# skyepurchase/MeatModeler

Hardware: AMD Instinct MI355X
Metric: descriptor-match pairs/sec + BA residuals/sec, 500×1080p frames, 1/2/4/8 GPU (higher is better)
Workload: dtype u8/int32 (match), f64 (BA); 1 GPU; 500 frames 1920x1080, 4000 ORB kpts/frame, BF Hamming 2-NN + ratio, track linking, 2-view DLT, full BA (TRF, Schur, f64 MFMA Cholesky); frames=500, height=1080, width=1920, nfeatures=4000, parallelism=pairs/points x1

## Files before the change

meatmodeler_amd/_lib.py:

```python
import ctypes as C
import os

_HERE = os.path.dirname(os.path.abspath(__file__))
LIB_PATH = os.path.join(_HERE, "libmeatmodeler_hip.so")

c_i32p = C.POINTER(C.c_int32)
c_i64p = C.POINTER(C.c_int64)
c_f32p = C.POINTER(C.c_float)
c_f64p = C.POINTER(C.c_double)
c_u8p = C.POINTER(C.c_uint8)
c_i8p = C.POINTER(C.c_int8)
vp = C.c_void_p


class MMError(RuntimeError):
    pass


class OrbParams(C.Structure):
    _fields_ = [("nfeatures", C.c_int32), ("nlevels", C.c_int32), ("edge_threshold", C.c_int32),
                ("fast_threshold", C.c_int32), ("scale_factor", C.c_float), ("reserved", C.c_int32)]


class BAProblem(C.Structure):
    _fields_ = [("F", C.c_int32), ("P", C.c_int32), ("O", C.c_int64), ("K", vp), ("fi", vp), ("pi", vp),
                ("obs", vp), ("pt_ptr", vp), ("pt_obs", vp), ("cam_ptr", vp), ("cam_obs", vp),
                ("cam_span", C.c_int32), ("reserved", C.c_int32), ("n_seg", C.c_int64), ("seg_ids", vp),
                ("seg_chunk_ptr", vp), ("n_chunks", C.c_int64), ("chunk_seg", vp), ("chunk_begin", vp),
                ("chunk_end", vp), ("pair_o", vp), ("pair_o2", vp), ("pair_p", vp)]


class BAIndex(C.Structure):
    _fields_ = [("F", C.c_int32), ("P", C.c_int32), ("O", C.c_int64), ("fi", vp), ("pi", vp),
                ("pt_ptr", vp), ("pt_obs", vp), ("cam_ptr", vp), ("cam_obs", vp), ("head", vp),
                ("cam_span", C.c_int32), ("chunk", C.c_int32), ("n_pairs", C.c_int64),
                ("pair_o", vp), ("pair_o2", vp), ("pair_p", vp), ("seg_ids", vp), ("seg_chunk_ptr", vp),
                ("chunk_seg", vp), ("chunk_begin", vp), ("chunk_end", vp)]


class BAFixed(C.Structure):
    _fields_ = [("F_fixed", C.c_int32), ("reserved", C.c_int32), ("cams", vp)]


class TrfParams(C.Structure):
    _fields_ = [("ftol", C.c_double), ("xtol", C.c_double), ("gtol", C.c_double), ("min_damping", C.c_double),
                ("max_nfev", C.c_int64)]


class TrfRow(C.Structure):
    _fields_ = [("iteration", C.c_int32), ("nfev", C.c_int32), ("cost", C.c_double), ("reduction", C.c_double),
                ("step_norm", C.c_double), ("optimality", C.c_double)]


class TriParams(C.Structure):
    _fields_ = [("refine_iters", C.c_int32), ("reserved", C.c_int32), ("max_reproj_px", C.c_double),
                ("max_cos_parallax", C.c_double), ("min_depth", C.c_double)]


class VerifyParams(C.Structure):
    _fields_ = [("n_hyp", C.c_int32), ("min_matches", C.c_int32), ("min_inliers", C.c_int32), ("refit_iters", C.c_int32),
                ("seed", C.c_uint32), ("pair_base", C.c_uint32), ("on_fail", C.c_int32), ("reserved", C.c_int32),
                ("threshold_px", C.c_double)]


class PoseParams(C.Structure):
    _fields_ = [("min_matches", C.c_int32), ("reserved", C.c_int32), ("min_front_frac", C.c_double),
                ("ambiguous_frac", C.c_double)]


class HomographyParams(C.Structure):
    _fields_ = [("n_hyp", C.c_int32), ("min_matches", C.c_int32), ("min_inliers", C.c_int32), ("refit_iters", C.c_int32),
                ("seed", C.c_uint32), ("pair_base", C.c_uint32), ("threshold_px", C.c_double), ("collinear_tol", C.c_double),
                ("degenerate_frac", C.c_double)]


class HPoseParams(C.Structure):
    _fields_ = [("min_matches", C.c_int32), ("reserved", C.c_int32), ("min_front_frac", C.c_double),
                ("ambiguous_frac", C.c_double), ("rotation_tol", C.c_double)]


class GuidedParams(C.Structure):
    _fields_ = [("threshold_px", C.c_double), ("ratio", C.c_double), ("max_dist", C.c_int32), ("cross_check", C.c_int32)]


class ResectParams(C.Structure):
    _fields_ = [("n_hyp", C.c_int32), ("min_rows", C.c_int32), ("min_inliers", C.c_int32), ("refit_iters", C.c_int32),
                ("polish_iters", C.c_int32), ("reserved", C.c_int32), ("seed", C.c_uint32), ("cam_base", C.c_uint32),
                ("threshold_px", C.c_double)]


class ResectPlanarParams(C.Structure):
    _fields_ = ResectParams._fields_ + [("planar_tol", C.c_double), ("collinear_tol", C.c_double)]


class AlignParams(C.Structure):
    _fields_ = [("n_hyp", C.c_int32), ("min_points", C.c_int32), ("min_inliers", C.c_int32), ("refit_iters", C.c_int32),
                ("with_scale", C.c_int32), ("reserved", C.c_int32), ("seed", C.c_uint32), ("prob_base", C.c_uint32),
                ("tau", C.c_double), ("collinear_tol", C.c_double)]


ALLREDUCE_FN =C.CFUNCTYPE(C.c_int, vp, vp, C.c_int64)


class Dist(C.Structure):
    _fields_ = [("rank", C.c_int32), ("world", C.c_int32), ("half_bandwidth", C.c_int32), ("band_exchange", C.c_int32),
                ("allreduce", ALLREDUCE_FN), ("user", vp)]


class TrfReport(C.Structure):
    _fields_ = [("cost0", C.c_double), ("cost", C.c_double), ("optimality", C.c_double), ("min_damping", C.c_double),
                ("nfev", C.c_int32), ("njev", C.c_int32), ("status", C.c_int32), ("iterations", C.c_int32),
                ("log_rows", C.c_int32), ("chol_fallbacks", C.c_int32), ("collectives", C.c_int32), ("reserved", C.c_int32)]


SIGNATURES = {
    "mm_abi_version": (C.c_int, []),
    "mm_ctx_create": (C.c_int, [C.c_int, vp, C.POINTER(vp)]),
    "mm_ctx_destroy": (None, [vp]),
    "mm_ctx_control": (C.c_longlong, [vp, C.c_int, C.c_longlong]),
    "mm_last_error": (C.c_char_p, [vp]),
    "mm_ctx_sync": (C.c_int, [vp]),
    "mm_timer_create": (C.c_int, [vp, C.POINTER(vp)]),
    "mm_timer_start": (C.c_int, [vp, vp]),
    "mm_timer_stop": (C.c_int, [vp, vp]),
    "mm_timer_elapsed_ms": (C.c_int, [vp, vp, C.POINTER(C.c_float)]),
    "mm_timer_destroy": (None, [vp, vp]),
    "mm_profile_enable": (C.c_int, [vp, C.c_int]),
    "mm_profile_report": (C.c_int, [vp, C.c_char_p, C.c_size_t]),
    "mm_profile_select": (C.c_int, [vp, C.c_char_p]),
    "mm_bf_workspace_bytes": (C.c_size_t, [C.c_int, C.c_int, C.c_int]),
    "mm_bf_knn2_batched": (C.c_int, [vp, vp, vp, C.c_int, C.c_size_t, vp, vp, C.c_int, C.c_size_t, C.c_int, vp, vp,
                                     vp, C.c_size_t]),
    "mm_bf_knn2_hamming": (C.c_int, [vp, vp, C.c_int, vp, C.c_int, vp, vp, vp, C.c_size_t]),
    "mm_ratio_filter_batched": (C.c_int, [vp, vp, vp, vp, C.c_int, C.c_int, C.c_double, vp, vp]),
    "mm_bf_match_ratio_workspace_bytes": (C.c_size_t, [C.c_int, C.c_int, C.c_int]),
    "mm_bf_match_ratio_batched": (C.c_int, [vp, vp, vp, C.c_int, C.c_size_t, vp, vp, C.c_int, C.c_size_t, C.c_int,
                                            C.c_double, vp, vp, vp, C.c_size_t]),
    "mm_orb_workspace_bytes": (C.c_size_t, [C.c_int, C.c_int, C.c_int, C.POINTER(OrbParams)]),
    "mm_orb_detect_compute": (C.c_int, [vp, vp, C.c_int, C.c_int, C.c_int, C.c_int, C.POINTER(OrbParams), vp, vp,
                                        C.c_size_t, vp, vp, vp, vp, vp, vp]),
    "mm_orb_level_sizes": (C.c_int, [C.c_int, C.c_int, C.POINTER(OrbParams), c_i32p, c_i32p, c_i32p, c_f32p]),
    "mm_link_tracks_clip": (C.c_int64, [C.c_int, C.c_int, c_i32p, c_f32p, C.c_int, c_i32p, c_i32p, C.c_int64,
                                        C.c_int64, c_i64p, c_i32p, c_i32p, c_i64p]),
    "mm_link_workspace_bytes": (C.c_size_t, [C.c_int, C.c_int]),
    "mm_link_tracks_device": (C.c_int, [vp, C.c_int, C.c_int, vp, vp, vp, vp, vp, C.c_size_t, vp, vp, vp, vp]),
    "mm_flatten_offsets": (C.c_int, [vp, vp, vp, C.c_int64, vp]),
    "mm_flatten_tracks": (C.c_int, [vp, vp, vp, vp, vp, C.c_int, vp, C.c_int, C.c_int64, vp, C.c_int64, C.c_int, vp, vp, vp]),
    "mm_ba_build_pairs": (C.c_int64, [C.c_int, C.c_int, C.c_int64, c_i32p, c_i32p, c_i32p, c_i32p, c_i32p, c_i32p, C.c_int,
                                      c_i64p, c_i32p, c_i32p, C.c_int64]),
    "mm_ba_build_index": (C.c_int, [C.c_int, C.c_int, C.c_int64, c_i32p, c_i32p, c_i32p, c_i32p, c_i32p, c_i32p]),
    "mm_verify_workspace_bytes": (C.c_size_t, [C.c_int, C.c_int]),
    "mm_verify_matches": (C.c_int, [vp, vp, vp, vp, C.c_int, C.c_int, C.POINTER(VerifyParams), vp, vp, vp, vp, vp, vp, C.c_size_t]),
    "mm_recover_poses": (C.c_int, [vp, c_f64p, vp, vp, vp, vp, C.c_int, C.c_int, C.POINTER(PoseParams), vp, vp, vp, vp, vp]),
    "mm_chain_poses": (C.c_int, [vp, vp, vp, vp, vp, vp, vp, C.c_int, C.c_int, c_f64p, C.c_int, vp, vp, vp, vp]),
    "mm_homography_workspace_bytes": (C.c_size_t, [C.c_int, C.c_int]),
    "mm_verify_homography": (C.c_int, [vp, vp, vp, vp, C.c_int, C.c_int, C.POINTER(HomographyParams), vp, vp, vp, vp, vp, vp, vp,
                                       C.c_size_t]),
    "mm_recover_poses_homography": (C.c_int, [vp, c_f64p, vp, vp, vp, vp, vp, C.c_int, C.c_int, C.POINTER(HPoseParams), vp, vp, vp,
                                              vp, vp, vp]),
    "mm_guided_workspace_bytes": (C.c_size_t, [C.c_int, C.c_int]),
    "mm_guided_match": (C.c_int, [vp, vp, vp, vp, vp, vp, vp, vp, C.c_int, C.c_int, C.POINTER(GuidedParams), vp, vp, vp, vp, vp,
                                  C.c_size_t]),
    "mm_resect_workspace_bytes": (C.c_size_t, [C.c_int, C.c_int, C.c_int64]),
    "mm_resect_cameras": (C.c_int, [vp, c_f64p, vp, C.c_int64, vp, vp, C.c_int64, vp, vp, C.c_int64, C.c_int, vp, vp,
                                    C.POINTER(ResectParams), vp, vp, vp, vp, vp, C.c_size_t]),
    "mm_resect_planar_workspace_bytes": (C.c_size_t, [C.c_int, C.c_int, C.c_int64]),
    "mm_resect_planar": (C.c_int, [vp, c_f64p, vp, C.c_int64, vp, vp, C.c_int64, vp, vp, C.c_int64, C.c_int, vp, vp,
                                   C.POINTER(ResectPlanarParams), vp, vp, vp, vp, vp, vp, C.c_size_t]),
    "mm_align_workspace_bytes": (C.c_size_t, [C.c_int, C.c_int, C.c_int64]),
    "mm_align_similarity": (C.c_int, [vp, vp, vp, c_i64p, C.c_int, C.POINTER(AlignParams), vp, vp, vp, vp, vp, C.c_size_t]),
    "mm_apply_similarity": (C.c_int, [vp, vp, vp, C.c_int64, vp, C.c_int64]),
    "mm_camera_centres": (C.c_int, [vp, vp, C.c_int64, vp]),
    "mm_triangulate_dlt": (C.c_int, [vp, vp, vp, vp, vp, vp, C.c_int64, vp]),
    "mm_triangulate_tracks_workspace_bytes": (C.c_size_t, [C.c_int]),
    "mm_triangulate_tracks": (C.c_int, [vp, vp, C.c_int, vp, C.c_int64, vp, vp, C.POINTER(TriParams), vp, vp, vp, vp, C.c_size_t]),
    "mm_ba_residual": (C.c_int, [vp, C.POINTER(BAProblem), vp, vp, vp, vp, vp, C.c_size_t]),
    "mm_ba_jacobian": (C.c_int, [vp, C.POINTER(BAProblem), vp, vp, vp, vp]),
    "mm_ba_normal_eq": (C.c_int, [vp, C.POINTER(BAProblem), vp, vp, vp, vp, vp, vp]),
    "mm_ba_jvp": (C.c_int, [vp, C.POINTER(BAProblem), vp, vp, vp, vp, vp]),
    "mm_ba_schur": (C.c_int, [vp, C.POINTER(BAProblem), vp, vp, vp, vp, vp, vp, vp, vp, vp, vp, C.c_size_t]),
    "mm_ba_schur_workspace_bytes": (C.c_size_t, [C.POINTER(BAProblem)]),
    "mm_ba_pairs_count": (C.c_int, [vp, C.POINTER(BAProblem), vp, vp]),
    "mm_ba_pairs_emit": (C.c_int, [vp, C.POINTER(BAProblem), vp, C.c_int, vp, vp, vp]),
    "mm_ba_index_bounds": (C.c_int, [C.c_int, C.c_int, C.c_int64, C.c_int, c_i64p, c_i64p]),
    "mm_ba_index_workspace_bytes": (C.c_size_t, [vp, C.POINTER(BAIndex), C.c_int]),
    "mm_ba_index_build": (C.c_int, [vp, C.POINTER(BAIndex), C.c_int, vp, C.c_size_t, vp, C.c_size_t]),
    "mm_ba_schur_solve": (C.c_int, [vp, C.POINTER(BAProblem), vp, vp, vp, vp, vp, vp, vp, vp, vp, C.c_int, vp, vp,
                                    C.c_size_t, vp, C.c_size_t, C.c_int, C.c_int, c_i64p, c_i64p]),
    "mm_multi_dot_workspace_bytes": (C.c_size_t, []),
    "mm_multi_dot": (C.c_int, [vp, C.c_int, C.POINTER(vp), C.POINTER(vp), C.c_int64, C.c_int64, vp, vp, C.c_size_t]),
    "mm_trf_fused": (C.c_int, [vp, C.c_int, C.POINTER(vp), C.POINTER(vp), C.POINTER(vp), C.c_double, C.c_double, C.c_int64,
                               C.c_int64, vp, vp, C.c_size_t]),
    "mm_trf_damping": (C.c_int, [vp, vp, vp, C.c_double, C.c_double, vp]),
    "mm_ba_backsub": (C.c_int, [vp, C.POINTER(BAProblem), vp, vp, vp, vp, vp, vp, vp, C.c_size_t]),
    "mm_ba_backsub_workspace_bytes": (C.c_size_t, [C.POINTER(BAProblem)]),
    "mm_chol_workspace_bytes": (C.c_size_t, [C.c_int]),
    "mm_chol_solve": (C.c_int, [vp, vp, C.c_int, vp, C.c_int, C.c_int, vp, vp, C.c_size_t]),
    "mm_ba_jvp_dots_workspace_bytes": (C.c_size_t, [C.POINTER(BAProblem)]),
    "mm_ba_jvp_dots": (C.c_int, [vp, C.POINTER(BAProblem), vp, vp, vp, vp, vp, vp, vp, vp, C.c_size_t]),
    "mm_ba_scale_update": (C.c_int, [vp, C.c_int, C.c_int, vp, vp, vp, C.c_int]),
    "mm_ba_damp": (C.c_int, [vp, C.c_int, C.c_int, vp, vp, vp, vp, vp, vp]),
    "mm_trf_step2d": (C.c_int, [vp, vp, vp, vp, vp, vp, vp, vp, vp, C.c_double, vp]),
    "mm_pyr_down": (C.c_int, [vp, vp, C.c_int, C.c_int, C.c_int, vp, C.c_int]),
    "mm_lk_track": (C.c_int, [vp, vp, vp, vp, vp, vp, C.c_int, vp, C.c_int, C.c_int, C.c_int, C.c_int, C.c_double, vp, vp, vp]),
    "mm_min_eig": (C.c_int, [vp, vp, C.c_int, C.c_int, C.c_int, C.c_int, vp]),
    "mm_corner_candidates": (C.c_int, [vp, vp, C.c_int, C.c_int, C.c_double, vp, vp, vp, C.c_int, vp]),
    "mm_gftt_select": (C.c_int, [vp, C.c_int64, C.c_int, C.c_int, C.c_int, C.c_double, vp, C.c_int]),
    "mm_contrast_workspace_bytes": (C.c_size_t, [C.c_int, C.c_int, C.c_int, C.c_int, C.c_int]),
    "mm_increase_contrast": (C.c_int, [vp, vp, C.c_int, C.c_int, C.c_int, vp, vp, vp, C.c_double, C.c_int, C.c_int, vp, vp, vp,
                                       C.c_size_t]),
    "mm_bgr_to_grey": (C.c_int, [vp, vp, C.c_size_t, vp]),
    "mm_write_ply": (C.c_int, [C.c_char_p, vp, C.c_int64]),
    "mm_chol_solve_sym": (C.c_int, [vp, vp, C.c_int, vp, C.c_int, C.c_int, vp, vp, C.c_size_t]),
    "mm_ba_trf_workspace_bytes": (C.c_size_t, [C.POINTER(BAProblem)]),
    "mm_ba_trf": (C.c_int, [vp, C.POINTER(BAProblem), vp, vp, C.POINTER(TrfParams), C.POINTER(TrfReport),
                            C.POINTER(TrfRow), C.c_int, vp, C.c_size_t]),
    "mm_ba_trf_batched_workspace_bytes": (C.c_size_t, [C.POINTER(BAProblem)]),
    "mm_ba_trf_batched": (C.c_int, [vp, C.c_int, C.POINTER(C.POINTER(BAProblem)), C.POINTER(vp), C.POINTER(vp),
                                    C.POINTER(TrfParams), C.POINTER(TrfReport), C.POINTER(vp), C.POINTER(C.c_size_t), c_i32p]),
    "mm_ba_residual_fixed": (C.c_int, [vp, C.POINTER(BAProblem), C.POINTER(BAFixed), vp, vp, vp, vp, vp, C.c_size_t]),
    "mm_ba_normal_eq_fixed": (C.c_int, [vp, C.POINTER(BAProblem), C.POINTER(BAFixed), vp, vp, vp, vp, vp, vp]),
    "mm_ba_trf_fixed_workspace_bytes": (C.c_size_t, [C.POINTER(BAProblem), C.POINTER(BAFixed)]),
    "mm_ba_trf_fixed": (C.c_int, [vp, C.POINTER(BAProblem), C.POINTER(BAFixed), vp, vp, C.POINTER(TrfParams),
                                  C.POINTER(TrfReport), C.POINTER(TrfRow), C.c_int, vp, C.c_size_t]),
    "mm_ba_trf_dist_workspace_bytes": (C.c_size_t, [C.POINTER(BAProblem), C.c_int]),
    "mm_ba_trf_dist": (C.c_int, [vp, C.POINTER(BAProblem), vp, vp, C.POINTER(TrfParams), C.POINTER(TrfReport),
                                 C.POINTER(TrfRow), C.c_int, vp, C.c_size_t, C.POINTER(Dist)]),
}


def _load():
    if not os.path.exists(LIB_PATH):
        raise ImportError(
            f"{LIB_PATH} is missing: the HIP extension has not been built "
            "(make -C meatmodeler_amd/csrc).  meatmodeler_amd has no CPU fallback.")
    lib = C.CDLL(LIB_PATH)
    for name, (res, args) in SIGNATURES.items():
        fn = getattr(lib, name)
        fn.restype = res
        fn.argtypes = args
    return lib


lib = _load()


def ptr(t):
    if t is None:
        return None
    if hasattr(t, "data_ptr"):
        return t.data_ptr()
    return t.ctypes.data


class Context:

    def __init__(self, device=None, stream=None):
        import torch
        if not torch.cuda.is_available():
            raise MMError("meatmodeler_amd needs an AMD GPU (torch.cuda.is_available() is False); "
                          "there is no CPU path")
        if device is None:
            device = torch.cuda.current_device()
        self.device = torch.device("cuda", device if isinstance(device, int) else device.index or 0)
        self.stream = stream if stream is not None else torch.cuda.current_stream(self.device)
        h = vp()
        rc = lib.mm_ctx_create(self.device.index, vp(self.stream.cuda_stream), C.byref(h))
        if rc != 0:
            raise MMError(f"mm_ctx_create failed ({rc})")
        self.h = h

    def check(self, rc, what=""):
        if rc != 0:
            msg = lib.mm_last_error(self.h)
            raise MMError(f"{what} failed ({rc}): {msg.decode() if msg else ''}")

    def sync(self):
        self.check(lib.mm_ctx_sync(self.h), "mm_ctx_sync")

    CTL_CHOL_FORCE_ABANDON, CTL_CHOL_LAST_PATH, CTL_CHOL_RESERVED, CTL_CU_COUNT, CTL_CHOL_AVOID_FUSED = 1, 2, 3, 4, 5
    CTL_LINK_LAST_VARIANT = 6
    CTL_BATCH_LAST = 7

    def control(self, what, value=0):
        r = int(lib.mm_ctx_control(self.h, int(what), int(value)))
        if r < -1 or (r == -1 and what not in (self.CTL_CHOL_LAST_PATH, self.CTL_LINK_LAST_VARIANT, self.CTL_BATCH_LAST)):
            self.check(r, "mm_ctx_control")
        return r

    def profile(self, level, only=None):
        if only is not None:
            self.check(lib.mm_profile_select(self.h, only.encode()), "mm_profile_select")
        self.check(lib.mm_profile_enable(self.h, int(level)), "mm_profile_enable")

    def profile_report(self):
        buf = C.create_string_buffer(1 << 16)
        n = lib.mm_profile_report(self.h, buf, len(buf))
        if n < 0:
            self.check(n, "mm_profile_report")
        out = {}
        for line in buf.value.decode().splitlines():
            name, cnt, ms = line.split()
            out[name] = (int(cnt), float(ms))
        return out

    def __del__(self):
        try:
            if getattr(self, "h", None):
                lib.mm_ctx_destroy(self.h)
                self.h = None
        except Exception:
            pass


class Timer:

    def __init__(self, ctx):
        self.ctx = ctx
        self.t = vp()
        ctx.check(lib.mm_timer_create(ctx.h, C.byref(self.t)), "mm_timer_create")

    def start(self):
        self.ctx.check(lib.mm_timer_start(self.ctx.h, self.t), "mm_timer_start")

    def stop(self):
        self.ctx.check(lib.mm_timer_stop(self.ctx.h, self.t), "mm_timer_stop")

    def elapsed_ms(self):
        ms = C.c_float()
        self.ctx.check(lib.mm_timer_elapsed_ms(self.ctx.h, self.t, C.byref(ms)), "mm_timer_elapsed_ms")
        return ms.value

    def __del__(self):
        try:
            lib.mm_timer_destroy(self.ctx.h, self.t)
        except Exception:
            pass


_default_ctx = {}


def default_context():
    import torch
    key = (torch.cuda.current_device(), torch.cuda.current_stream().cuda_stream)
    c = _default_ctx.get(key)
    if c is None:
        c = _default_ctx[key] = Context()
    return c
```

meatmodeler_amd/csrc/mm_common.h:

```cpp
#pragma once
#include <hip/hip_runtime.h>
#include <cstdarg>
#include <cstdio>
#include <cstring>
#include <vector>
#include "../../include/meatmodeler.h"

struct mm_prof_rec {
    const char *name;
    hipEvent_t a, b;
};

struct mm_ctx {
    int device;
    hipStream_t stream;
    char err[512];
    int prof = 0;
    char prof_only[64] = {0};
    std::vector<mm_prof_rec> recs;
    std::vector<hipEvent_t> pool;
    hipStream_t aux = nullptr;
    hipEvent_t ev_fork = nullptr, ev_join = nullptr;
    bool attr_chol_fused = false, attr_chol_bwd = false, attr_chol_batch = false;
    int cu_count = 0, fused_wgs = 0, chol_last_path = -1, debug_abandon = 0;
    bool chol_avoid_fused = false;
    bool chol_strict_budget = false;
    hipEvent_t fused_ev = nullptr;
    bool fused_ev_pending = false;
    bool fused_no_event = false;
    int link_last_variant = -1;
    void *cam_tab = nullptr;
    int cam_tab_cap = 0, cam_tab_F = 0;
    const double *cam_tab_for = nullptr;
    bool cam_tab_hold = false;
    const double *fx_cams = nullptr;
    int fx_F = 0;
    bool fx_tab_ok = false;
    void *host_board = nullptr;
    unsigned long long host_board_seq = 0;
    void *batch_dev = nullptr, *batch_host = nullptr;
    size_t batch_dev_cap = 0, batch_host_cap = 0;
    bool jvp_rows_deferred = false;
    const double *jvp_partial = nullptr;
    unsigned jvp_n_wg = 0;
    const void *chol_init_done = nullptr;
    int chol_init_sides = 0;
    int batch_last = -1;
};

struct mm_stream_swap {
    mm_ctx *c;
    hipStream_t saved;
    mm_stream_swap(mm_ctx *ctx, hipStream_t s) : c(ctx), saved(ctx->stream) { ctx->stream = s; }
    ~mm_stream_swap() { c->stream = saved; }
};

struct mm_fixed_scope {
    mm_ctx *c;
    mm_fixed_scope(mm_ctx *ctx, const mm_ba_fixed *fx) : c(ctx) {
        ctx->fx_cams = fx->cams;
        ctx->fx_F = fx->F_fixed;
        ctx->fx_tab_ok = false;
    }
    ~mm_fixed_scope() {
        c->fx_cams = nullptr;
        c->fx_F = 0;
        c->fx_tab_ok = false;
    }
};

int mm_cam_coef_table(mm_ctx *ctx, const double *cams, int F, const void **tab_out);
void mm_cam_table_hold(mm_ctx *ctx, bool on);
void mm_cam_table_invalidate(mm_ctx *ctx);

int mm_ba_residual_publish(mm_ctx *ctx, const mm_ba_problem *pb, const double *cams, const double *pts, void *ws,
                           size_t ws_bytes, double *board, int cost_slot, int count, void *host_board, unsigned long long seq);

int mm_trf_fused0_scaled(mm_ctx *ctx, const double *g, double *si, const double *B, const double *C, double *gh, double *ghs, int64_t n,
                         int64_t split, double *out, void *ws, size_t ws_bytes);
int mm_trf_fused5_coef(mm_ctx *ctx, const double *x, const double *s1, const double *s2, double *x_new, const double *h01, int64_t n,
                       int64_t split, void *ctab, int F);
int mm_trf_rows_step2d(mm_ctx *ctx, const double *partial, unsigned n_wg, double *rows, const double *r0, const double *d11,
                       const double *r1, const double *r2, const double *r3, const double *reg, const int32_t *info, double Delta,
                       double *board);
int mm_cam_table_adopt(mm_ctx *ctx, const double *cams, int F, void **tab_out);
int mm_ba_damp_damping(mm_ctx *ctx, int F, int P, const double *B, const double *C, const double *scale_inv, const double *gh2,
                       const double *d11, double Delta, double min_damping, double *damp_out, double *Bd, double *Cd);
void mm_chol_release_budget(mm_ctx *ctx);
bool mm_chol_fused_eligible(int n, int half_bandwidth);
struct mm_chol_geom {
    int n, nblk, bwb;
    int a, m, b;
    int pad;
};
struct mm_chol_layout {
    double *Linv, *ytmp, *contrib, *contrib_bwd, *lpub, *spub;
    int32_t *flags;
    mm_chol_geom g;
    uint64_t nflags, nsent, nlpub;
};
struct mm_chol_plan {
    mm_chol_layout lay;
    bool fused;
    int sides;
    unsigned grid_fused, grid_bwd;
};
struct mm_chol_init_args {
    int32_t *info, *flags;
    size_t nflags;
    unsigned long long *sentinel_buf;
    size_t nsent;
    unsigned long long *lpub;
    size_t nlpub;
    unsigned long long *Linv;
    size_t nblk;
};
bool mm_chol_init_plan(mm_ctx *ctx, int n, int half_bandwidth, int32_t *info, void *ws, size_t ws_bytes, mm_chol_init_args *out, int *sides, int *bwb);
void mm_chol_init_done(mm_ctx *ctx, const void *ws, int sides);
struct mm_damp_spec {
    const double *B, *C, *si;
    const double *gh2, *d11;
    double Delta, min_damping;
    double *damp_out;
    const double *reg;
};
int mm_ba_schur_solve_damped(mm_ctx *ctx, const mm_ba_problem *pb, const double *cams, const double *pts, const mm_damp_spec *dmp,
                             double *Bd, double *Cd, const double *gc, const double *gp, double *S, double *v, double *Cinv,
                             int half_bandwidth, int32_t *info, void *ws_schur, size_t ws_schur_bytes, void *ws_chol,
                             size_t ws_chol_bytes);
int mm_chol_solve_gated(mm_ctx *ctx, double *A, int n, double *b, int nrhs, int half_bandwidth, int32_t *info, void *ws,
                        size_t ws_bytes, const int32_t *slab_ready, int cams_per_slab, int n_cams, int sym_mode);

struct mm_batch_prob {
    mm_ba_problem pb;
    int64_t n, nc;
    double *x, *x_new, *g, *si, *gh, *ghs, *gn, *q1, *w, *q2, *s1, *s2;
    double *B, *Bd, *C, *Cd, *Cinv, *u1, *Jq2, *dp, *v, *S;
    double *r0, *r1, *r2, *r3, *d11, *bs, *damp, *board;
    int32_t *info;
    void *ctab_x, *ctab_new;
    double *res_partial;
    unsigned *md_counter;
    double *md_partial;
    double *jvp_partial;
    double *backsub_T;
    double *schur_partial, *schur_camtab;
    int32_t *schur_seg_done, *schur_desc;
    mm_chol_layout chol;
    int32_t half_bw, chol_sym_mirror;
    uint32_t g_vec, g_res, g_jvp, g_pblk, g_obs, g_pts, g_scale, g_damp, g_prep, g_pairs, g_chol, g_bwd, g_coef, g_zero;
    void *mailbox;
};
struct mm_batch_dyn {
    double Delta;
    unsigned long long seq;
    double min_damping;
    double reg;
};

int mm_batch_fused(mm_ctx *ctx, int op, const mm_batch_prob *tab, const int32_t *list, int n_list, unsigned max_g);
unsigned mm_batch_fused_grid(int64_t n);
int mm_batch_scale_update(mm_ctx *ctx, const mm_batch_prob *tab, const int32_t *list, int n_list, unsigned max_g);
int mm_batch_damp(mm_ctx *ctx, const mm_batch_prob *tab, const int32_t *list, int n_list, unsigned max_g);
int mm_batch_accept(mm_ctx *ctx, const mm_batch_prob *tab, const int32_t *list, int n_list, unsigned max_g);
int mm_batch_step2d(mm_ctx *ctx, const mm_batch_prob *tab, const int32_t *list, int n_list, const mm_batch_dyn *dyn);
void mm_batch_ba_setup(mm_batch_prob *bp);
int mm_batch_cam_coef(mm_ctx *ctx, const mm_batch_prob *tab, const int32_t *list, int n_list, unsigned max_g, int which );
int mm_batch_jvp_dots(mm_ctx *ctx, const mm_batch_prob *tab, const int32_t *list, int n_list, unsigned max_g, int second);
int mm_batch_damping(mm_ctx *ctx, const mm_batch_prob *tab, const int32_t *list, int n_list, const mm_batch_dyn *dyn);
int mm_batch_set_reg(mm_ctx *ctx, const mm_batch_prob *tab, const int32_t *list, int n_list, const mm_batch_dyn *dyn);
int mm_batch_backsub(mm_ctx *ctx, const mm_batch_prob *tab, const int32_t *list, int n_list, unsigned max_g_obs, unsigned max_g_pts);
int mm_batch_residual_publish(mm_ctx *ctx, const mm_batch_prob *tab, const int32_t *list, int n_list, unsigned max_g,
                              const mm_batch_dyn *dyn);
int mm_batch_normal_eq(mm_ctx *ctx, const mm_batch_prob *tab, const int32_t *list, int n_list, unsigned max_g_pblk, unsigned max_F);
int mm_batch_publish_rows(mm_ctx *ctx, const mm_batch_prob *tab, const int32_t *list, int n_list, const mm_batch_dyn *dyn);
int mm_batch_schur_setup(mm_ctx *ctx, mm_batch_prob *bp, void *ws_schur, size_t ws_schur_bytes);
int mm_batch_schur(mm_ctx *ctx, const mm_batch_prob *tab, const int32_t *list, int n_list, unsigned max_g_zero, unsigned max_g_prep,
                   unsigned max_g_pairs);
int mm_batch_chol_setup(mm_ctx *ctx, mm_batch_prob *bp, void *ws_chol, size_t ws_chol_bytes);
int mm_batch_chol(mm_ctx *ctx, const mm_batch_prob *tab, const int32_t *list, int n_list, unsigned max_g_chol, unsigned max_g_bwd);

static inline hipEvent_t mm_prof_event(mm_ctx *c) {
    hipEvent_t e = nullptr;
    if (!c->pool.empty()) {
        e = c->pool.back();
        c->pool.pop_back();
    } else {
        (void)hipEventCreate(&e);
    }
    return e;
}

#define MM_LAUNCH(ctx, name, kernel, grid, block, shmem, ...)                                          \
    do {                                                                                               \
        hipEvent_t ea_ = nullptr, eb_ = nullptr;                                                       \
        const dim3 g_ = (grid);                                                                        \
        const bool p_ = (ctx)->prof == 1 || ((ctx)->prof == 2 && (size_t)g_.x * g_.y * g_.z >= 64) || \
                        ((ctx)->prof == 3 && strcmp(name, (ctx)->prof_only) == 0);                      \
        if (p_) {                                                                                      \
            ea_ = mm_prof_event(ctx);                                                                  \
            eb_ = mm_prof_event(ctx);                                                                  \
            (void)hipEventRecord(ea_, (ctx)->stream);                                                  \
        }                                                                                              \
        hipLaunchKernelGGL(kernel, g_, block, shmem, (ctx)->stream, __VA_ARGS__);                      \
        if (p_) {                                                                                      \
            (void)hipEventRecord(eb_, (ctx)->stream);                                                  \
            (ctx)->recs.push_back(mm_prof_rec{name, ea_, eb_});                                        \
        }                                                                                              \
        MM_LAUNCH_CHECK(ctx, name);                                                                    \
    } while (0)

static inline int mm_fail(mm_ctx *ctx, int code, const char *fmt, ...) {
    if (ctx) {
        va_list ap;
        va_start(ap, fmt);
        vsnprintf(ctx->err, sizeof(ctx->err), fmt, ap);
        va_end(ap);
    }
    return code;
}

#define MM_HIP(ctx, call)                                                                              \
    do {                                                                                               \
        hipError_t e_ = (call);                                                                        \
        if (e_ != hipSuccess)                                                                          \
            return mm_fail(ctx, MM_ERR_HIP, "%s failed: %s (%s:%d)", #call, hipGetErrorString(e_),    \
                           __FILE__, __LINE__);                                                        \
    } while (0)

#define MM_LAUNCH_CHECK(ctx, name)                                                                     \
    do {                                                                                               \
        hipError_t e_ = hipGetLastError();                                                             \
        if (e_ != hipSuccess)                                                                          \
            return mm_fail(ctx, MM_ERR_HIP, "launch of %s failed: %s", name, hipGetErrorString(e_));   \
    } while (0)

static inline size_t mm_align_up(size_t x, size_t a) { return (x + a - 1) / a * a; }
```

meatmodeler_amd/csrc/schur.hip:

```cpp
#include <type_traits>
#include "ba_eval.h"
#include "chol_init.h"

namespace {

__device__ __forceinline__ void sym3_inverse(double a, double b, double d, double e, double f, double g, double *__restrict__ o) {
    const double m00 = e * g - f * f, m01 = d * f - b * g, m02 = b * f - d * e;
    const double det = a * m00 + b * m01 + d * m02;
    const double id = 1.0 / det;
    o[0] = m00 * id;
    o[1] = m01 * id;
    o[2] = m02 * id;
    o[3] = (a * g - d * d) * id;
    o[4] = (b * d - a * f) * id;
    o[5] = (a * e - b * b) * id;
}

constexpr int SR_WIN = 256;

__global__ __launch_bounds__(256) void point_inverse_kernel(int P, const double *__restrict__ Cd,
                                                            double *__restrict__ Cinv) {
    int p = blockIdx.x * 256 + threadIdx.x;
    if (p >= P) return;
    const double *c = Cd + (size_t)p * 6;
    sym3_inverse(c[0], c[1], c[2], c[3], c[4], c[5], Cinv + (size_t)p * 6);
}

__global__ __launch_bounds__(256) void schur_rows_kernel(mm_ba_problem pb, const double *__restrict__ cams,
                                                         const double *__restrict__ pts, const double *__restrict__ Bd,
                                                         const double *__restrict__ Cinv, const double *__restrict__ gc,
                                                         const double *__restrict__ gp, double *__restrict__ S,
                                                         double *__restrict__ v) {
    __shared__ double acc[6][SR_WIN * 6];
    __shared__ double Ks[9];
    __shared__ double cs[6];
    __shared__ double sm[4];
    const int i = blockIdx.x;
    const int w0 = blockIdx.y * SR_WIN;
    const int wn = min(SR_WIN, pb.F - w0);
    const size_t n = (size_t)pb.F * 6;
    for (int e = threadIdx.x; e < 6 * SR_WIN * 6; e += 256) (&acc[0][0])[e] = 0.0;
    if (threadIdx.x < 9) Ks[threadIdx.x] = pb.K[threadIdx.x];
    if (threadIdx.x < 6) cs[threadIdx.x] = cams[(size_t)i * 6 + threadIdx.x];
    __syncthreads();
    double vg[6] = {0, 0, 0, 0, 0, 0};
    for (int e = pb.cam_ptr[i] + threadIdx.x; e < pb.cam_ptr[i + 1]; e += 256) {
        const int o = pb.cam_obs[e];
        const int p = pb.pi[o];
        const double *Xp = pts + (size_t)p * 3;
        Proj pr;
        ba_eval<true, true>(cs, Xp, Ks, pb.obs[2 * (size_t)o], pb.obs[2 * (size_t)o + 1], pr);
        const double *ci = Cinv + (size_t)p * 6;
        const double q00 = ci[0], q01 = ci[1], q02 = ci[2], q11 = ci[3], q12 = ci[4], q22 = ci[5];
        double Y[6][3];
#pragma unroll
        for (int a = 0; a < 6; ++a) {
            const double e0 = pr.Jc[0][a] * pr.Jp[0][0] + pr.Jc[1][a] * pr.Jp[1][0];
            const double e1 = pr.Jc[0][a] * pr.Jp[0][1] + pr.Jc[1][a] * pr.Jp[1][1];
            const double e2 = pr.Jc[0][a] * pr.Jp[0][2] + pr.Jc[1][a] * pr.Jp[1][2];
            Y[a][0] = e0 * q00 + e1 * q01 + e2 * q02;
            Y[a][1] = e0 * q01 + e1 * q11 + e2 * q12;
            Y[a][2] = e0 * q02 + e1 * q12 + e2 * q22;
        }
        if (blockIdx.y == 0) {
            const double g0 = gp[(size_t)p * 3], g1 = gp[(size_t)p * 3 + 1], g2 = gp[(size_t)p * 3 + 2];
#pragma unroll
            for (int a = 0; a < 6; ++a) vg[a] += Y[a][0] * g0 + Y[a][1] * g1 + Y[a][2] * g2;
        }
        for (int e2i = pb.pt_ptr[p]; e2i < pb.pt_ptr[p + 1]; ++e2i) {
            const int o2 = pb.pt_obs[e2i];
            const int f2 = pb.fi[o2];
            if (f2 < w0 || f2 >= w0 + wn) continue;
            Proj p2;
            ba_eval<true, true>(cams + (size_t)f2 * 6, Xp, Ks, pb.obs[2 * (size_t)o2], pb.obs[2 * (size_t)o2 + 1], p2);
            double *dst = &acc[0][(f2 - w0) * 6];
#pragma unroll
            for (int b = 0; b < 6; ++b) {
                const double e0 = p2.Jc[0][b] * p2.Jp[0][0] + p2.Jc[1][b] * p2.Jp[1][0];
                const double e1 = p2.Jc[0][b] * p2.Jp[0][1] + p2.Jc[1][b] * p2.Jp[1][1];
                const double e2 = p2.Jc[0][b] * p2.Jp[0][2] + p2.Jc[1][b] * p2.Jp[1][2];
#pragma unroll
                for (int a = 0; a < 6; ++a)
                    atomicAdd(dst + a * (SR_WIN * 6) + b, Y[a][0] * e0 + Y[a][1] * e1 + Y[a][2] * e2);
            }
        }
    }
    __syncthreads();
    for (int e = threadIdx.x; e < 6 * wn * 6; e += 256) {
        const int a = e / (wn * 6), c = e % (wn * 6);
        const int col = w0 * 6 + c;
        double val = -acc[a][c];
        if (col / 6 == i) val += Bd[(size_t)i * 36 + a * 6 + (col % 6)];
        S[((size_t)i * 6 + a) * n + col] = val;
    }
    if (blockIdx.y == 0) {
#pragma unroll
        for (int a = 0; a < 6; ++a) {
            const double s = block_sum<256>(vg[a], sm);
            if (threadIdx.x == 0) v[(size_t)i * 6 + a] = gc[(size_t)i * 6 + a] - s;
        }
    }
}

#ifndef MM_SP_WAVES
#define MM_SP_WAVES 1
#endif
constexpr int SP_WAVES = MM_SP_WAVES;
constexpr int MAX_SLABS = 64;
struct SlabSync {
    int32_t *ready;
    int32_t *done;
    int32_t seg_count[MAX_SLABS];
    int cams_per_slab;
};

constexpr int RED_LD = 65;
__device__ __forceinline__ void wave_lds_barrier() {
    __builtin_amdgcn_fence(__ATOMIC_RELEASE, "wavefront");
    __builtin_amdgcn_wave_barrier();
    __builtin_amdgcn_fence(__ATOMIC_ACQUIRE, "wavefront");
}
__device__ __forceinline__ void wave_reduce_42(const double (&acc)[42], double *slab , int lane, double &out0,
                                               double &out1) {
#pragma unroll
    for (int h = 0; h < 2; ++h) {
#pragma unroll
        for (int q = 0; q < 21; ++q) slab[q * RED_LD + lane] = acc[21 * h + q];
        wave_lds_barrier();
        double s = 0.0;
        if (lane < 21) {
            const double *row = slab + lane * RED_LD;
            double s0 = 0.0, s1 = 0.0, s2 = 0.0, s3 = 0.0;
#pragma unroll
            for (int j = 0; j < 64; j += 4) {
                s0 += row[j];
                s1 += row[j + 1];
                s2 += row[j + 2];
                s3 += row[j + 3];
            }
            s = (s0 + s1) + (s2 + s3);
        }
        if (h == 0)
            out0 = s;
        else
            out1 = s;
        wave_lds_barrier();
    }
}

struct CamPQ {
    double P[9], q[3];
};
__device__ __forceinline__ double fast_rcp(double x) {
    double y = __builtin_amdgcn_rcp(x);
    double e = fma(-x, y, 1.0);
    y = fma(y, e, y);
    e = fma(-x, y, 1.0);
    return fma(y, e, y);
}

struct LeanJ {
    double Jc[2][6];
    double Jp[2][3];
};
__device__ __forceinline__ void lean_eval(const CamPQ &c, const double *__restrict__ Ks, const double *__restrict__ Jr,
                                          double X0, double X1, double X2, LeanJ &o) {
    const double u0 = fma(c.P[0], X0, fma(c.P[1], X1, fma(c.P[2], X2, c.q[0])));
    const double u1 = fma(c.P[3], X0, fma(c.P[4], X1, fma(c.P[5], X2, c.q[1])));
    const double u2 = fma(c.P[6], X0, fma(c.P[7], X1, fma(c.P[8], X2, c.q[2])));
    const double iz = fast_rcp(u2);
    const double p[2] = {u0 * iz, u1 * iz};
#pragma unroll
    for (int m = 0; m < 2; ++m) {
#pragma unroll
        for (int k = 0; k < 3; ++k) {
            o.Jp[m][k] = fma(-p[m], c.P[6 + k], c.P[3 * m + k]) * iz;
            o.Jc[m][3 + k] = fma(-p[m], Ks[6 + k], Ks[3 * m + k]) * iz;
        }
        const double g0 = X1 * o.Jp[m][2] - X2 * o.Jp[m][1];
        const double g1 = X2 * o.Jp[m][0] - X0 * o.Jp[m][2];
        const double g2 = X0 * o.Jp[m][1] - X1 * o.Jp[m][0];
#pragma unroll
        for (int k = 0; k < 3; ++k) o.Jc[m][k] = fma(g0, Jr[k], fma(g1, Jr[3 + k], g2 * Jr[6 + k]));
    }
}

constexpr int SLAB2 = 32;
struct ChunkDesc {
    int32_t i, f2, e_begin, e_end, sidx, c_first, n_ch, pad;
};
template <bool FORCE>
__device__ __forceinline__ CamPQ cam_pq_scalar(const double *__restrict__ t) {
    CamPQ v;
#pragma unroll
    for (int k = 0; k < 9; ++k) v.P[k] = FORCE ? uniform_f64(t[k]) : t[k];
#pragma unroll
    for (int k = 0; k < 3; ++k) v.q[k] = FORCE ? uniform_f64(t[9 + k]) : t[9 + k];
    return v;
}
template <bool FORCE_UNIFORM>
__device__ __forceinline__ void schur_pairs_body(const mm_ba_problem pb, const double *__restrict__ camtab,
                                                                    const ChunkDesc *__restrict__ desc,
                                                                    const double *__restrict__ pts,
                                                                    const double *__restrict__ Cinv,
                                                                    const double *__restrict__ gp,
                                                                    double *partial, const double *__restrict__ Bd,
                                                                    const double *__restrict__ gc, double *S, double *v,
                                                                    int32_t *seg_done, SlabSync slabs, unsigned wg_begin,
                                                                    unsigned wg_total, const unsigned bx) {
    __shared__ double Ks[9];
    __shared__ double red[SP_WAVES][21 * RED_LD];
    __shared__ double jrs[SP_WAVES][SLAB2];
    if (threadIdx.x < 9) Ks[threadIdx.x] = pb.K[threadIdx.x];
    const int lane = threadIdx.x & 63;
    const int wv = __builtin_amdgcn_readfirstlane((int)(threadIdx.x >> 6));
    const unsigned gpos = bx + wg_begin;
    const unsigned wg = (gpos & 1) ? wg_total - 1 - (gpos >> 1) : (gpos >> 1);
    const int64_t c = (int64_t)wg * SP_WAVES + wv;
    const bool live = c < pb.n_chunks;
    ChunkDesc cd = {};
    if (live) cd = desc[c];
    if (FORCE_UNIFORM) {
        cd.i = __builtin_amdgcn_readfirstlane(cd.i);
        cd.f2 = __builtin_amdgcn_readfirstlane(cd.f2);
        cd.e_begin = __builtin_amdgcn_readfirstlane(cd.e_begin);
        cd.e_end = __builtin_amdgcn_readfirstlane(cd.e_end);
        cd.sidx = __builtin_amdgcn_readfirstlane(cd.sidx);
        cd.c_first = __builtin_amdgcn_readfirstlane(cd.c_first);
        cd.n_ch = __builtin_amdgcn_readfirstlane(cd.n_ch);
    }
    const int i = cd.i, f2 = cd.f2, d = cd.i - cd.f2, sidx = cd.sidx;
    const int e_begin = cd.e_begin, e_end = cd.e_end;
    auto point_of = [&](int e) { return pb.pair_p ? pb.pair_p[e] : pb.pi[pb.pair_o[e]]; };
    auto self_of = [&](int e) { return d == 0 && pb.pair_o[e] == pb.pair_o2[e]; };
    int e = e_begin + lane;
    int p_next = -1;
    bool self_next = false;
    if (live) {
        if (e < e_end) {
            p_next = point_of(e);
            self_next = self_of(e);
        }
        if (lane < 9) jrs[wv][lane] = camtab[(size_t)i * CAMTAB2 + 12 + lane];
        else if (lane >= 16 && lane < 25) jrs[wv][lane] = camtab[(size_t)f2 * CAMTAB2 + 12 + lane - 16];
    }
    __syncthreads();
    if (!live) return;
    const CamPQ cp_i = cam_pq_scalar<FORCE_UNIFORM>(camtab + (size_t)i * CAMTAB2), cp_2 = cam_pq_scalar<FORCE_UNIFORM>(camtab + (size_t)f2 * CAMTAB2);
    const double *Jr_i = jrs[wv], *Jr_2 = jrs[wv] + 16;
    double acc[42];
#pragma unroll
    for (int q = 0; q < 42; ++q) acc[q] = 0.0;
    auto load_xc = [&](int p, double (&x)[12]) {
        if (p >= 0) {
            const double *Xp = pts + (size_t)p * 3, *ci = Cinv + (size_t)p * 6;
            x[0] = Xp[0];
            x[1] = Xp[1];
            x[2] = Xp[2];
#pragma unroll
            for (int q = 0; q < 6; ++q) x[3 + q] = ci[q];
            if (d == 0) {
                x[9] = gp[(size_t)p * 3];
                x[10] = gp[(size_t)p * 3 + 1];
                x[11] = gp[(size_t)p * 3 + 2];
            }
        }
    };
    auto pair_body = [&](int p, bool self, const double (&x)[12]) {
        const double X0 = x[0], X1 = x[1], X2 = x[2];
        const double q00 = x[3], q01 = x[4], q02 = x[5], q11 = x[6], q12 = x[7], q22 = x[8];
        LeanJ a;
        lean_eval(cp_i, Ks, Jr_i, X0, X1, X2, a);
        double Z[2][3];
#pragma unroll
        for (int m = 0; m < 2; ++m) {
            Z[m][0] = a.Jp[m][0] * q00 + a.Jp[m][1] * q01 + a.Jp[m][2] * q02;
            Z[m][1] = a.Jp[m][0] * q01 + a.Jp[m][1] * q11 + a.Jp[m][2] * q12;
            Z[m][2] = a.Jp[m][0] * q02 + a.Jp[m][1] * q12 + a.Jp[m][2] * q22;
        }
        double M[2][2], T[2][6];
        if (d == 0) {
            if (self) {
                const double g0 = x[9], g1 = x[10], g2 = x[11];
                const double z0 = Z[0][0] * g0 + Z[0][1] * g1 + Z[0][2] * g2, z1 = Z[1][0] * g0 + Z[1][1] * g1 + Z[1][2] * g2;
#pragma unroll
                for (int q = 0; q < 6; ++q) acc[36 + q] += a.Jc[0][q] * z0 + a.Jc[1][q] * z1;
            }
#pragma unroll
            for (int m = 0; m < 2; ++m)
#pragma unroll
                for (int n_ = 0; n_ < 2; ++n_) M[m][n_] = Z[m][0] * a.Jp[n_][0] + Z[m][1] * a.Jp[n_][1] + Z[m][2] * a.Jp[n_][2];
#pragma unroll
            for (int b = 0; b < 6; ++b) {
                T[0][b] = M[0][0] * a.Jc[0][b] + M[0][1] * a.Jc[1][b];
                T[1][b] = M[1][0] * a.Jc[0][b] + M[1][1] * a.Jc[1][b];
            }
        } else {
            LeanJ b2;
            lean_eval(cp_2, Ks, Jr_2, X0, X1, X2, b2);
#pragma unroll
            for (int m = 0; m < 2; ++m)
#pragma unroll
                for (int n_ = 0; n_ < 2; ++n_) M[m][n_] = Z[m][0] * b2.Jp[n_][0] + Z[m][1] * b2.Jp[n_][1] + Z[m][2] * b2.Jp[n_][2];
#pragma unroll
            for (int b = 0; b < 6; ++b) {
                T[0][b] = M[0][0] * b2.Jc[0][b] + M[0][1] * b2.Jc[1][b];
                T[1][b] = M[1][0] * b2.Jc[0][b] + M[1][1] * b2.Jc[1][b];
            }
        }
#pragma unroll
        for (int q = 0; q < 6; ++q)
#pragma unroll
            for (int b = 0; b < 6; ++b) acc[q * 6 + b] += a.Jc[0][q] * T[0][b] + a.Jc[1][q] * T[1][b];
    };
    double xc[12];
    load_xc(p_next, xc);
    int p_cur = p_next;
    bool self_cur = self_next;
    {
        const int en = e + 64;
        p_next = en < e_end ? point_of(en) : -1;
        self_next = en < e_end && self_of(en);
    }
#pragma clang loop unroll(disable)
    for (; e - lane < e_end; e += 64) {
        double xn[12];
        load_xc(p_next, xn);
        const int p_nn_e = e + 128;
        const int p_nn = p_nn_e < e_end ? point_of(p_nn_e) : -1;
        const bool self_nn = p_nn_e < e_end && self_of(p_nn_e);
        if (p_cur >= 0) pair_body(p_cur, self_cur, xc);
#pragma unroll
        for (int q = 0; q < 12; ++q) xc[q] = xn[q];
        p_cur = p_next;
        self_cur = self_next;
        p_next = p_nn;
        self_next = self_nn;
    }
    double tot0, tot1;
    wave_reduce_42(acc, red[wv], lane, tot0, tot1);
    const int c_first = cd.c_first, n_ch = cd.n_ch;
    const size_t n = (size_t)pb.F * 6;
    bool writer = true;
    if (n_ch > 1) {
        if (lane < 21) {
            __hip_atomic_store(partial + (size_t)c * 42 + lane, tot0, __ATOMIC_RELAXED, __HIP_MEMORY_SCOPE_AGENT);
            __hip_atomic_store(partial + (size_t)c * 42 + 21 + lane, tot1, __ATOMIC_RELAXED, __HIP_MEMORY_SCOPE_AGENT);
        }
        asm volatile("s_waitcnt vmcnt(0)" ::: "memory");
        __builtin_amdgcn_wave_barrier();
        int last = 0;
        if (lane == 0) last = atomicAdd(seg_done + sidx, 1) == n_ch - 1;
        writer = __shfl(last, 0, 64) != 0;
        if (writer && lane < 21) {
            tot0 = 0.0;
            tot1 = 0.0;
            for (int cc = 0; cc < n_ch; ++cc) {
                tot0 += __hip_atomic_load(partial + (size_t)(c_first + cc) * 42 + lane, __ATOMIC_RELAXED, __HIP_MEMORY_SCOPE_AGENT);
                tot1 += __hip_atomic_load(partial + (size_t)(c_first + cc) * 42 + 21 + lane, __ATOMIC_RELAXED, __HIP_MEMORY_SCOPE_AGENT);
            }
        }
    }
    if (!writer) return;
    const bool through = slabs.ready != nullptr;
    if (lane < 21) {
#pragma unroll
        for (int h = 0; h < 2; ++h) {
            const int q = 21 * h + lane;
            const double sum = h == 0 ? tot0 : tot1;
            if (q < 36) {
                double val = -sum;
                if (d == 0) val += Bd[(size_t)i * 36 + q];
                double *dst = S + ((size_t)i * 6 + q / 6) * n + (size_t)f2 * 6 + q % 6;
                double *mir = S + ((size_t)f2 * 6 + q % 6) * n + (size_t)i * 6 + q / 6;
                if (through) {
                    __hip_atomic_store(dst, val, __ATOMIC_RELAXED, __HIP_MEMORY_SCOPE_AGENT);
                    if (d != 0) __hip_atomic_store(mir, val, __ATOMIC_RELAXED, __HIP_MEMORY_SCOPE_AGENT);
                } else {
                    *dst = val;
                    if (d != 0) *mir = val;
                }
            } else if (d == 0) {
                double *dst = v + (size_t)i * 6 + (q - 36);
                const double val = gc[(size_t)i * 6 + (q - 36)] - sum;
                if (through) __hip_atomic_store(dst, val, __ATOMIC_RELAXED, __HIP_MEMORY_SCOPE_AGENT);
                else *dst = val;
            }
        }
    }
    if (slabs.ready) {
        asm volatile("s_waitcnt vmcnt(0)" ::: "memory");
        __builtin_amdgcn_wave_barrier();
        if (lane == 0) {
            const int sl = i / slabs.cams_per_slab;
            if (atomicAdd(slabs.done + sl, 1) == slabs.seg_count[sl] - 1)
                __hip_atomic_store(slabs.ready + sl, 1, __ATOMIC_RELEASE, __HIP_MEMORY_SCOPE_AGENT);
        }
    }
}
__global__ __launch_bounds__(64 * SP_WAVES, 2) void schur_pairs_kernel(mm_ba_problem pb, const double *__restrict__ camtab,
                                                                    const ChunkDesc *__restrict__ desc,
                                                                    const double *__restrict__ pts,
                                                                    const double *__restrict__ Cinv,
                                                                    const double *__restrict__ gp,
                                                                    double *partial, const double *__restrict__ Bd,
                                                                    const double *__restrict__ gc, double *S, double *v,
                                                                    int32_t *seg_done, SlabSync slabs, unsigned wg_begin,
                                                                    unsigned wg_total) {
    schur_pairs_body<false>(pb, camtab, desc, pts, Cinv, gp, partial, Bd, gc, S, v, seg_done, slabs, wg_begin, wg_total, blockIdx.x);
}
__global__ __launch_bounds__(64 * SP_WAVES, 2) void schur_pairs_batch_kernel(const mm_batch_prob *__restrict__ tab, const int32_t *__restrict__ list) {
    const mm_batch_prob &bp = tab[list[blockIdx.y]];
    if (blockIdx.x >= bp.g_pairs) return;
    SlabSync none = {};
    schur_pairs_body<true>(bp.pb, bp.schur_camtab, (const ChunkDesc *)bp.schur_desc, bp.x + bp.nc, bp.Cinv, bp.g + bp.nc, bp.schur_partial, bp.Bd,
                     bp.g, bp.S, bp.v, bp.schur_seg_done, none, 0u, bp.g_pairs, blockIdx.x);
}


__device__ __forceinline__ void write_chunk_desc(const mm_ba_problem &pb, int32_t *__restrict__ desc, int64_t first, int64_t stride) {
    for (int64_t k = first; k < pb.n_chunks; k += stride) {
        const int sidx = pb.chunk_seg[k], seg = pb.seg_ids[sidx];
        const int ci = seg / (pb.cam_span + 1), cdd = seg % (pb.cam_span + 1);
        const int c_first = pb.seg_chunk_ptr[sidx];
        int32_t *o = desc + 8 * k;
        o[0] = ci;
        o[1] = ci - cdd;
        o[2] = pb.chunk_begin[k];
        o[3] = pb.chunk_end[k];
        o[4] = sidx;
        o[5] = c_first;
        o[6] = pb.seg_chunk_ptr[sidx + 1] - c_first;
        o[7] = 0;
    }
}
struct PrepExtra {
    mm_damp_spec dmp;
    int zero_bwb;
    int chol_init;
    mm_chol_init_args init;
};
__device__ __forceinline__ void schur_prepare_body(mm_ba_problem pb, const double *__restrict__ cams,
                                                            double *__restrict__ Bd, const double *__restrict__ Cd,
                                                            const double *__restrict__ gc, double *__restrict__ Cinv,
                                                            double *__restrict__ S, double *__restrict__ v,
                                                            double *__restrict__ tab, int32_t *__restrict__ seg_done,
                                                            int32_t *__restrict__ desc , const unsigned bx, const unsigned gx,
                                                            const PrepExtra *ex = nullptr) {
    const int b = (int)bx, tid = threadIdx.x;
    for (int64_t k = (int64_t)b * 256 + tid; k < pb.n_seg; k += (int64_t)gx * 256) seg_done[k] = 0;
    if (desc) write_chunk_desc(pb, desc, (int64_t)b * 256 + tid, (int64_t)gx * 256);
    const bool fold = ex && ex->dmp.B;
    double reg = 0.0;
    if (fold) {
        if (ex->dmp.gh2) {
            const double r = trf_damping_value(ex->dmp.gh2[0], ex->dmp.d11[0], ex->dmp.Delta);
            reg = fmax(r, ex->dmp.min_damping);
            if (b == 0 && tid == 0) {
                ex->dmp.damp_out[0] = r;
                ex->dmp.damp_out[1] = reg;
            }
        } else {
            reg = ex->dmp.reg[0];
        }
    }
    if (ex && ex->chol_init) mm_chol_init_body(ex->init, bx, gx);
    const size_t n = (size_t)pb.F * 6;
    if (ex && ex->zero_bwb >= 0) {
        const int nblk = (int)((n + 63) / 64);
        for (size_t r = bx; r < n; r += gx) {
            const int bi = (int)(r >> 6);
            const int lo = bi - ex->zero_bwb < 0 ? 0 : bi - ex->zero_bwb, hi = bi + ex->zero_bwb >= nblk ? nblk - 1 : bi + ex->zero_bwb;
            const size_t c0 = (size_t)lo * 64, c1 = (size_t)(hi + 1) * 64 < n ? (size_t)(hi + 1) * 64 : n;
            const size_t d0 = r / 6 * 6;
            for (size_t c = c0 + 2 * (size_t)tid; c < c1; c += 512)
                if (c < d0 || c >= d0 + 6) *reinterpret_cast<double2 *>(S + r * n + c) = double2{0.0, 0.0};
        }
    }
    const int f = b * 256 + tid;
    if (f < pb.F) cam_table2_row(cams + (size_t)f * 6, pb.K, tab + (size_t)f * CAMTAB2);
    if (b < pb.F) {
        const bool empty = pb.cam_ptr[b + 1] == pb.cam_ptr[b];
        if (tid < 36) {
            double bd;
            if (fold) {
                bd = ex->dmp.B[(size_t)b * 36 + tid];
                if (tid % 7 == 0) {
                    const double s = ex->dmp.si[(size_t)b * 6 + tid / 7];
                    bd = fma(s * s, reg, bd);
                }
                Bd[(size_t)b * 36 + tid] = bd;
            } else {
                bd = Bd[(size_t)b * 36 + tid];
            }
            if (empty)
                S[((size_t)b * 6 + tid / 6) * n + (size_t)b * 6 + tid % 6] = bd;
            else if (ex && ex->zero_bwb >= 0)
                S[((size_t)b * 6 + tid / 6) * n + (size_t)b * 6 + tid % 6] = 0.0;
        }
        if (empty && tid < 6) v[(size_t)b * 6 + tid] = gc[(size_t)b * 6 + tid];
    }
    const int p = b * 256 + tid;
    if (p < pb.P) {
        double a, bq, d, e, ff, g;
        if (fold) {
            const double *c = ex->dmp.C + (size_t)p * 6;
            const double *sp = ex->dmp.si + n + (size_t)p * 3;
            a = fma(sp[0] * sp[0], reg, c[0]);
            bq = c[1];
            d = c[2];
            e = fma(sp[1] * sp[1], reg, c[3]);
            ff = c[4];
            g = fma(sp[2] * sp[2], reg, c[5]);
        } else {
            const double *c = Cd + (size_t)p * 6;
            a = c[0], bq = c[1], d = c[2], e = c[3], ff = c[4], g = c[5];
        }
        sym3_inverse(a, bq, d, e, ff, g, Cinv + (size_t)p * 6);
    }
}
__global__ __launch_bounds__(256) void schur_prepare_kernel(mm_ba_problem pb, const double *__restrict__ cams,
                                                            double *__restrict__ Bd, const double *__restrict__ Cd,
                                                            const double *__restrict__ gc, double *__restrict__ Cinv,
                                                            double *__restrict__ S, double *__restrict__ v,
                                                            double *__restrict__ tab, int32_t *__restrict__ seg_done,
                                                            int32_t *__restrict__ desc) {
    schur_prepare_body(pb, cams, Bd, Cd, gc, Cinv, S, v, tab, seg_done, desc, blockIdx.x, gridDim.x);
}
__global__ __launch_bounds__(256) void schur_prepare_damped_kernel(mm_ba_problem pb, const double *__restrict__ cams,
                                                                   double *__restrict__ Bd, const double *__restrict__ gc,
                                                                   double *__restrict__ Cinv, double *__restrict__ S,
                                                                   double *__restrict__ v, double *__restrict__ tab,
                                                                   int32_t *__restrict__ seg_done, int32_t *__restrict__ desc,
                                                                   PrepExtra ex) {
    schur_prepare_body(pb, cams, Bd, nullptr, gc, Cinv, S, v, tab, seg_done, desc, blockIdx.x, gridDim.x, &ex);
}
__global__ __launch_bounds__(256) void zero_batch_kernel(const mm_batch_prob *__restrict__ tab, const int32_t *__restrict__ list) {
    const mm_batch_prob &bp = tab[list[blockIdx.y]];
    if (blockIdx.x >= bp.g_zero) return;
    double2 *S2 = reinterpret_cast<double2 *>(bp.S);
    const int64_t n2 = bp.nc * bp.nc / 2;
    for (int64_t i = (int64_t)blockIdx.x * 256 + threadIdx.x; i < n2; i += (int64_t)bp.g_zero * 256) S2[i] = make_double2(0.0, 0.0);
}
__global__ __launch_bounds__(256) void schur_prepare_batch_kernel(const mm_batch_prob *__restrict__ tab, const int32_t *__restrict__ list) {
    const mm_batch_prob &bp = tab[list[blockIdx.y]];
    if (blockIdx.x >= bp.g_prep) return;
    schur_prepare_body(bp.pb, bp.x, bp.Bd, bp.Cd, bp.g, bp.Cinv, bp.S, bp.v, bp.schur_camtab, bp.schur_seg_done, bp.schur_desc,
                       blockIdx.x, bp.g_prep);
}

__global__ void slab_flag_kernel(int32_t *flags, int s) {
    __hip_atomic_store(flags + s, 1, __ATOMIC_RELEASE, __HIP_MEMORY_SCOPE_AGENT);
}

__global__ __launch_bounds__(256) void pairs_count_kernel(mm_ba_problem pb, int32_t *__restrict__ cnt,
                                                          int32_t *__restrict__ span_out) {
    const int64_t o = (int64_t)blockIdx.x * 256 + threadIdx.x;
    int dmax = 0;
    if (o < pb.O) {
        const int f = pb.fi[o], p = pb.pi[o];
        int c = 0;
        for (int e = pb.pt_ptr[p]; e < pb.pt_ptr[p + 1]; ++e) {
            const int d = f - pb.fi[pb.pt_obs[e]];
            c += d >= 0;
            dmax = max(dmax, d);
        }
        cnt[o] = c;
    }
    for (int off = 32; off > 0; off >>= 1) dmax = max(dmax, __shfl_down(dmax, off, 64));
    if ((threadIdx.x & 63) == 0 && dmax > __hip_atomic_load(span_out, __ATOMIC_RELAXED, __HIP_MEMORY_SCOPE_AGENT)) atomicMax(span_out, dmax);
}

__global__ __launch_bounds__(256) void pairs_emit_kernel(mm_ba_problem pb, const int64_t *__restrict__ offsets, int span,
                                                         int32_t *__restrict__ key, int32_t *__restrict__ po,
                                                         int32_t *__restrict__ po2) {
    const int64_t o = (int64_t)blockIdx.x * 256 + threadIdx.x;
    if (o >= pb.O) return;
    const int f = pb.fi[o], p = pb.pi[o];
    int64_t w = offsets[o];
    for (int e = pb.pt_ptr[p]; e < pb.pt_ptr[p + 1]; ++e) {
        const int o2 = pb.pt_obs[e];
        const int d = f - pb.fi[o2];
        if (d < 0) continue;
        key[w] = f * (span + 1) + d;
        po[w] = (int32_t)o;
        po2[w] = o2;
        ++w;
    }
}

}

extern "C" int mm_ba_pairs_count(mm_ctx *ctx, const mm_ba_problem *pb, int32_t *cnt, int32_t *span_out) {
    if (!ctx) return MM_ERR_ARG;
    if (!pb || !cnt || !span_out || (pb->O > 0 && (!pb->fi || !pb->pi || !pb->pt_ptr || !pb->pt_obs)))
        return mm_fail(ctx, MM_ERR_ARG, "mm_ba_pairs_count: bad argument");
    MM_HIP(ctx, hipMemsetAsync(span_out, 0, sizeof(int32_t), ctx->stream));
    if (pb->O == 0) return MM_OK;
    MM_LAUNCH(ctx, "pairs_count_kernel", pairs_count_kernel, dim3((unsigned)((pb->O + 255) / 256)), dim3(256), 0, *pb, cnt,
              span_out);
    return MM_OK;
}

extern "C" int mm_ba_pairs_emit(mm_ctx *ctx, const mm_ba_problem *pb, const int64_t *offsets, int span, int32_t *key,
                                int32_t *pair_o, int32_t *pair_o2) {
    if (!ctx) return MM_ERR_ARG;
    if (!pb || !offsets || !key || !pair_o || !pair_o2 || span < 0) return mm_fail(ctx, MM_ERR_ARG, "mm_ba_pairs_emit: bad argument");
    if (pb->O == 0) return MM_OK;
    if ((int64_t)pb->F * (span + 1) > 0x7fffffffLL) return mm_fail(ctx, MM_ERR_ARG, "mm_ba_pairs_emit: F * (span + 1) overflows the key");
    MM_LAUNCH(ctx, "pairs_emit_kernel", pairs_emit_kernel, dim3((unsigned)((pb->O + 255) / 256)), dim3(256), 0, *pb, offsets,
              span, key, pair_o, pair_o2);
    return MM_OK;
}

namespace {
struct SchurWs {
    double *partial;
    int32_t *seg_done;
    int32_t *slab_ready;
    int32_t *slab_done;
    double *camtab;
    int32_t *desc;
};
size_t carve_schur_ws(SchurWs &w, char *base, const mm_ba_problem *pb) {
    size_t off = 0;
    auto take = [&](auto *&p, size_t n) {
        using T = std::remove_reference_t<decltype(*p)>;
        p = reinterpret_cast<T *>(base + off);
        off += mm_align_up(n * sizeof(T), 256);
    };
    take(w.partial, (size_t)pb->n_chunks * 42);
    take(w.seg_done, (size_t)pb->n_seg);
    take(w.slab_ready, 2 * MAX_SLABS);
    w.slab_done = w.slab_ready + MAX_SLABS;
    take(w.camtab, (size_t)pb->F * CAMTAB2);
    take(w.desc, (size_t)pb->n_chunks * 8);
    return off;
}
struct SchurPlan {
    bool pairs;
    unsigned g_prep;
    unsigned g_pairs;
    size_t ws_bytes;
    SchurWs ws;
};
SchurPlan schur_plan(const mm_ba_problem *pb, void *ws) {
    SchurPlan pl;
    pl.pairs = pb->n_seg > 0 && pb->n_chunks > 0 && pb->seg_ids && pb->seg_chunk_ptr && pb->chunk_seg && pb->chunk_begin &&
               pb->chunk_end && pb->pair_o && pb->pair_o2;
    pl.g_prep = (unsigned)((pb->P + 255) / 256 > pb->F ? (pb->P + 255) / 256 : pb->F);
    pl.g_pairs = (unsigned)((pb->n_chunks + SP_WAVES - 1) / SP_WAVES);
    pl.ws_bytes = carve_schur_ws(pl.ws, (char *)ws, pb);
    return pl;
}
int launch_prepare(mm_ctx *ctx, const mm_ba_problem *pb, const SchurPlan &pl, const double *cams, const double *Bd, const double *Cd,
                   const double *gc, double *Cinv, double *S, double *v) {
    MM_LAUNCH(ctx, "schur_prepare_kernel", schur_prepare_kernel, dim3(pl.g_prep), dim3(256), 0, *pb, cams, const_cast<double *>(Bd), Cd, gc,
              Cinv, S, v, pl.ws.camtab, pl.ws.seg_done, pl.ws.desc);
    return MM_OK;
}
int launch_pairs(mm_ctx *ctx, const mm_ba_problem *pb, const SchurPlan &pl, const double *pts, const double *Cinv, const double *gp,
                 const double *Bd, const double *gc, double *S, double *v, const SlabSync &slabs, unsigned wg_begin, unsigned wg_count) {
    MM_LAUNCH(ctx, "schur_pairs_kernel", schur_pairs_kernel, dim3(wg_count), dim3(64 * SP_WAVES), 0, *pb, (const double *)pl.ws.camtab,
              (const ChunkDesc *)pl.ws.desc, pts, Cinv, gp, pl.ws.partial, Bd, gc, S, v, pl.ws.seg_done, slabs, wg_begin, pl.g_pairs);
    return MM_OK;
}
}

extern "C" size_t mm_ba_schur_workspace_bytes(const mm_ba_problem *pb) {
    if (!pb || pb->n_chunks <= 0) return 0;
    return schur_plan(pb, nullptr).ws_bytes;
}

extern "C" int mm_ba_schur(mm_ctx *ctx, const mm_ba_problem *pb, const double *cams, const double *pts,
                           const double *Bd, const double *Cd, const double *gc, const double *gp, double *S, double *v,
                           double *Cinv, void *ws, size_t ws_bytes) {
    if (!ctx) return MM_ERR_ARG;
    if (!pb || pb->F < 0 || pb->P < 0 || pb->O < 0 || !pb->K) return mm_fail(ctx, MM_ERR_ARG, "mm_ba_schur: bad problem");
    if (!cams || !pts || !Bd || !Cd || !gc || !gp || !S || !v || !Cinv || !pb->pt_ptr || !pb->cam_ptr ||
        (pb->O > 0 && (!pb->pt_obs || !pb->cam_obs || !pb->fi || !pb->pi || !pb->obs)))
        return mm_fail(ctx, MM_ERR_ARG, "mm_ba_schur: null pointer");
    if (pb->F == 0) return MM_OK;
    const SchurPlan pl = schur_plan(pb, ws);
    if (pl.pairs) {
        if (!ws || ws_bytes < pl.ws_bytes) return mm_fail(ctx, MM_ERR_WORKSPACE, "mm_ba_schur: workspace too small");
        MM_HIP(ctx, hipMemsetAsync(S, 0, (size_t)pb->F * 6 * pb->F * 6 * sizeof(double), ctx->stream));
        if (int rc = launch_prepare(ctx, pb, pl, cams, Bd, Cd, gc, Cinv, S, v)) return rc;
        return launch_pairs(ctx, pb, pl, pts, Cinv, gp, Bd, gc, S, v, SlabSync{}, 0u, pl.g_pairs);
    }
    if (pb->P > 0)
        MM_LAUNCH(ctx, "point_inverse_kernel", point_inverse_kernel, dim3((pb->P + 255) / 256), dim3(256), 0, pb->P, Cd,
                  Cinv);
    const int nwin = (pb->F + SR_WIN - 1) / SR_WIN;
    MM_LAUNCH(ctx, "schur_rows_kernel", schur_rows_kernel, dim3(pb->F, nwin), dim3(256), 0, *pb, cams, pts, Bd, Cinv, gc,
              gp, S, v);
    return MM_OK;
}

extern "C" int mm_ba_schur_solve(mm_ctx *ctx, const mm_ba_problem *pb, const double *cams, const double *pts,
                                 const double *Bd, const double *Cd, const double *gc, const double *gp, double *S,
                                 double *v, double *Cinv, int half_bandwidth, int32_t *info, void *ws_schur,
                                 size_t ws_schur_bytes, void *ws_chol, size_t ws_chol_bytes, int n_slabs,
                                 int cams_per_slab, const int64_t *slab_seg_ptr, const int64_t *slab_chunk_ptr) {
    if (!ctx) return MM_ERR_ARG;
    if (!pb || !info) return mm_fail(ctx, MM_ERR_ARG, "mm_ba_schur_solve: bad argument");
    const int n = pb->F * 6;
    const SchurPlan pl = schur_plan(pb, ws_schur);
    const bool overlap = pl.pairs && n_slabs >= 2 && n_slabs <= MAX_SLABS && cams_per_slab >= 16 && slab_seg_ptr &&
                         slab_chunk_ptr && mm_chol_fused_eligible(n, half_bandwidth) && pb->P > 0;
    if (!overlap) {
        int rc = mm_ba_schur(ctx, pb, cams, pts, Bd, Cd, gc, gp, S, v, Cinv, ws_schur, ws_schur_bytes);
        if (rc) return rc;
        return mm_chol_solve_sym(ctx, S, n, v, half_bandwidth, 1, info, ws_chol, ws_chol_bytes);
    }
    if (!cams || !pts || !Bd || !Cd || !gc || !gp || !S || !v || !Cinv) return mm_fail(ctx, MM_ERR_ARG, "mm_ba_schur_solve: null pointer");
    if (!ws_schur || ws_schur_bytes < pl.ws_bytes) return mm_fail(ctx, MM_ERR_WORKSPACE, "mm_ba_schur_solve: workspace too small");
    if (slab_seg_ptr[0] != 0 || slab_seg_ptr[n_slabs] != pb->n_seg || slab_chunk_ptr[0] != 0 || slab_chunk_ptr[n_slabs] != pb->n_chunks ||
        (int64_t)n_slabs * cams_per_slab < pb->F)
        return mm_fail(ctx, MM_ERR_ARG, "mm_ba_schur_solve: slab tables do not cover the problem");
    if (!ctx->aux) {
        int lo = 0, hi = 0;
        (void)hipDeviceGetStreamPriorityRange(&lo, &hi);
        MM_HIP(ctx, hipStreamCreateWithPriority(&ctx->aux, hipStreamNonBlocking, hi));
        MM_HIP(ctx, hipEventCreateWithFlags(&ctx->ev_fork, hipEventDisableTiming));
        MM_HIP(ctx, hipEventCreateWithFlags(&ctx->ev_join, hipEventDisableTiming));
    }
    SlabSync slabs = {};
    slabs.ready = pl.ws.slab_ready;
    slabs.done = pl.ws.slab_done;
    slabs.cams_per_slab = cams_per_slab;
    for (int sl = 0; sl < n_slabs; ++sl) slabs.seg_count[sl] = (int32_t)(slab_seg_ptr[sl + 1] - slab_seg_ptr[sl]);
    MM_HIP(ctx, hipMemsetAsync(S, 0, (size_t)n * n * sizeof(double), ctx->stream));
    MM_HIP(ctx, hipMemsetAsync(pl.ws.slab_ready, 0, 2 * MAX_SLABS * sizeof(int32_t), ctx->stream));
    if (int rc = launch_prepare(ctx, pb, pl, cams, Bd, Cd, gc, Cinv, S, v)) return rc;
    for (int sl = 0; sl < n_slabs; ++sl)
        if (slabs.seg_count[sl] == 0) MM_LAUNCH(ctx, "slab_flag_kernel", slab_flag_kernel, dim3(1), dim3(1), 0, pl.ws.slab_ready, sl);
    const unsigned wg_first = pl.g_pairs / 2;
    if (wg_first > 0)
        if (int rc = launch_pairs(ctx, pb, pl, pts, Cinv, gp, Bd, gc, S, v, slabs, 0u, wg_first)) return rc;
    MM_HIP(ctx, hipEventRecord(ctx->ev_fork, ctx->stream));
    MM_HIP(ctx, hipStreamWaitEvent(ctx->aux, ctx->ev_fork, 0));
    {
        mm_stream_swap sw(ctx, ctx->aux);
        int rc = mm_chol_solve_gated(ctx, S, n, v, 1, half_bandwidth, info, ws_chol, ws_chol_bytes, pl.ws.slab_ready, cams_per_slab, pb->F, 2);
        if (rc) {
            (void)hipEventRecord(ctx->ev_join, ctx->aux);
            (void)hipStreamWaitEvent(sw.saved, ctx->ev_join, 0);
            return rc;
        }
        MM_HIP(ctx, hipEventRecord(ctx->ev_join, ctx->aux));
    }
    if (int rc = launch_pairs(ctx, pb, pl, pts, Cinv, gp, Bd, gc, S, v, slabs, wg_first, pl.g_pairs - wg_first)) return rc;
    MM_HIP(ctx, hipStreamWaitEvent(ctx->stream, ctx->ev_join, 0));
    return MM_OK;
}

int mm_ba_schur_solve_damped(mm_ctx *ctx, const mm_ba_problem *pb, const double *cams, const double *pts, const mm_damp_spec *dmp,
                             double *Bd, double *Cd, const double *gc, const double *gp, double *S, double *v, double *Cinv,
                             int half_bandwidth, int32_t *info, void *ws_schur, size_t ws_schur_bytes, void *ws_chol,
                             size_t ws_chol_bytes) {
    if (!ctx) return MM_ERR_ARG;
    if (!pb || !dmp || !info || !cams || !pts || !Bd || !gc || !gp || !S || !v || !Cinv || !dmp->B || !dmp->C || !dmp->si ||
        (!dmp->gh2 && !dmp->reg) || (dmp->gh2 && (!dmp->d11 || !dmp->damp_out)))
        return mm_fail(ctx, MM_ERR_ARG, "mm_ba_schur_solve_damped: bad argument");
    const int n = pb->F * 6;
    static const bool off = [] { const char *e = getenv("MM_SCHUR_FOLD"); return e && atoi(e) == 0; }();
    mm_chol_init_args ia = {};
    int sides = 0, bwb = 0;
    const SchurPlan pl = schur_plan(pb, ws_schur);
    const bool fold = !off && pl.pairs && pb->P > 0 && ws_schur && ws_schur_bytes >= pl.ws_bytes &&
                      mm_chol_init_plan(ctx, n, half_bandwidth, info, ws_chol, ws_chol_bytes, &ia, &sides, &bwb);
    if (!fold) {
        if (!Cd) return mm_fail(ctx, MM_ERR_ARG, "mm_ba_schur_solve_damped: the separate calls need Cd");
        int rc = dmp->gh2 ? mm_ba_damp_damping(ctx, pb->F, pb->P, dmp->B, dmp->C, dmp->si, dmp->gh2, dmp->d11, dmp->Delta, dmp->min_damping,
                                                dmp->damp_out, Bd, Cd)
                          : mm_ba_damp(ctx, pb->F, pb->P, dmp->B, dmp->C, dmp->si, dmp->reg, Bd, Cd);
        if (rc) return rc;
        return mm_ba_schur_solve(ctx, pb, cams, pts, Bd, Cd, gc, gp, S, v, Cinv, half_bandwidth, info, ws_schur, ws_schur_bytes, ws_chol,
                                 ws_chol_bytes, 0, 0, nullptr, nullptr);
    }
    PrepExtra ex = {};
    ex.dmp = *dmp;
    ex.zero_bwb = bwb;
    ex.chol_init = 1;
    ex.init = ia;
    MM_LAUNCH(ctx, "schur_prepare_kernel", schur_prepare_damped_kernel, dim3(pl.g_prep), dim3(256), 0, *pb, cams, Bd, gc, Cinv, S, v,
              pl.ws.camtab, pl.ws.seg_done, pl.ws.desc, ex);
    if (int rc = launch_pairs(ctx, pb, pl, pts, Cinv, gp, Bd, gc, S, v, SlabSync{}, 0u, pl.g_pairs)) return rc;
    mm_chol_init_done(ctx, ws_chol, sides);
    const int rc = mm_chol_solve_sym(ctx, S, n, v, half_bandwidth, 1, info, ws_chol, ws_chol_bytes);
    mm_chol_init_done(ctx, nullptr, 0);
    return rc;
}

int mm_batch_schur_setup(mm_ctx *ctx, mm_batch_prob *bp, void *ws_schur, size_t ws_schur_bytes) {
    const mm_ba_problem *pb = &bp->pb;
    const SchurPlan pl = schur_plan(pb, ws_schur);
    if (!(pl.pairs && pb->pair_p) || pb->P <= 0)
        return mm_fail(ctx, MM_ERR_ARG, "mm_ba_trf_batched: a problem without a co-observation pair list");
    if (!ws_schur || ws_schur_bytes < pl.ws_bytes) return mm_fail(ctx, MM_ERR_WORKSPACE, "mm_ba_trf_batched: Schur workspace");
    bp->schur_partial = pl.ws.partial;
    bp->schur_camtab = pl.ws.camtab;
    bp->schur_seg_done = pl.ws.seg_done;
    bp->schur_desc = pl.ws.desc;
    bp->g_prep = pl.g_prep;
    bp->g_pairs = pl.g_pairs;
    const int64_t n2 = bp->nc * bp->nc / 2;
    const int64_t gz = (n2 + 2047) / 2048;
    bp->g_zero = (uint32_t)(gz < 1 ? 1 : (gz > 1024 ? 1024 : gz));
    return MM_OK;
}
int mm_batch_schur(mm_ctx *ctx, const mm_batch_prob *tab, const int32_t *list, int n_list, unsigned max_g_zero, unsigned max_g_prep,
                   unsigned max_g_pairs) {
    if (n_list <= 0) return MM_OK;
    MM_LAUNCH(ctx, "schur_zero_kernel", zero_batch_kernel, dim3(max_g_zero, (unsigned)n_list), dim3(256), 0, tab, list);
    MM_LAUNCH(ctx, "schur_prepare_kernel", schur_prepare_batch_kernel, dim3(max_g_prep, (unsigned)n_list), dim3(256), 0, tab, list);
    MM_LAUNCH(ctx, "schur_pairs_kernel", schur_pairs_batch_kernel, dim3(max_g_pairs, (unsigned)n_list), dim3(64 * SP_WAVES), 0, tab, list);
    return MM_OK;
}
```

meatmodeler_amd/csrc/trf.hip:

```cpp
#include "mm_common.h"
#include "trf_decide.h"
#include <chrono>
#include <vector>
#include <algorithm>
#include <initializer_list>
#include <utility>
#include <cmath>
#include <cstdlib>

namespace {

__global__ __launch_bounds__(256) void vec_mul_kernel(const double *__restrict__ a, const double *__restrict__ b,
                                                      double *__restrict__ out, int64_t n) {
    const int64_t i = (int64_t)blockIdx.x * 256 + threadIdx.x;
    if (i < n) out[i] = a[i] * b[i];
}

struct HostBoard {
    double v[16];
    unsigned long long seq;
    unsigned long long pad[7];
};

__global__ __launch_bounds__(64) void board_publish_kernel(const double *__restrict__ dev, int count, HostBoard *hb,
                                                          unsigned long long seq) {
    if ((int)threadIdx.x < count) hb->v[threadIdx.x] = dev[threadIdx.x];
    __threadfence_system();
    __builtin_amdgcn_wave_barrier();
    if (threadIdx.x == 0) __hip_atomic_store(&hb->seq, seq, __ATOMIC_RELEASE, __HIP_MEMORY_SCOPE_SYSTEM);
}

constexpr int EX_MAX_ITEMS = 12, EX_SCALARS = 64, EX_MAX_WORLD = 16;
struct ExItems {
    double *p[EX_MAX_ITEMS];
    int kind[EX_MAX_ITEMS];
    int n, rank, world;
    const int32_t *info;
};
__global__ __launch_bounds__(64) void ex_pack_kernel(ExItems it, double *__restrict__ ex) {
    const int t = threadIdx.x;
    double v = 0.0;
    if (t < it.n) {
        const double *r = it.p[t];
        const int k = it.kind[t];
        if (k == 0) v = it.rank == 0 ? r[0] + r[1] : r[1];
        else if (k == 1) v = r[2];
        else if (k == 3) v = r[0];
    }
    ex[t] = v;
    __syncthreads();
    if (t == 0) {
        int slot = 16;
        for (int i = 0; i < it.n; ++i) {
            if (it.kind[i] == 2) { ex[slot + it.rank] = it.p[i][1]; slot += EX_MAX_WORLD; }
            if (it.kind[i] == 4) { ex[slot + it.rank] = it.info[0] < 0 ? 1.0 : 0.0; slot += EX_MAX_WORLD; }
        }
    }
}
__global__ __launch_bounds__(64) void ex_unpack_kernel(ExItems it, const double *__restrict__ ex) {
    const int t = threadIdx.x;
    if (t < it.n) {
        double *r = it.p[t];
        const int k = it.kind[t];
        if (k == 0 || k == 1) r[2] = ex[t];
        else if (k == 3) r[0] = ex[t];
    }
    if (t == 0) {
        int slot = 16;
        for (int i = 0; i < it.n; ++i) {
            if (it.kind[i] == 2) {
                double m = it.p[i][0];
                for (int q = 0; q < it.world; ++q) m = fmax(m, ex[slot + q]);
                it.p[i][2] = m;
                slot += EX_MAX_WORLD;
            }
            if (it.kind[i] == 4) {
                double sum = 0.0;
                for (int q = 0; q < it.world; ++q) sum += ex[slot + q];
                it.p[i][0] = sum;
                slot += EX_MAX_WORLD;
            }
        }
    }
}
__global__ __launch_bounds__(256) void band_pack_kernel(const double *__restrict__ S, int64_t n, int hb, double *__restrict__ band) {
    const int64_t i = (int64_t)blockIdx.x * 256 + threadIdx.x, total = n * (hb + 1);
    if (i >= total) return;
    const int64_t j = i / (hb + 1), k = i % (hb + 1);
    band[i] = j + k < n ? S[(j + k) * n + j] : 0.0;
}
__global__ __launch_bounds__(256) void band_unpack_kernel(double *__restrict__ S, int64_t n, int hb, const double *__restrict__ band,
                                                          const double *__restrict__ Bd, double dup) {
    const int64_t i = (int64_t)blockIdx.x * 256 + threadIdx.x, total = n * (hb + 1);
    if (i >= total) return;
    const int64_t j = i / (hb + 1), k = i % (hb + 1), row = j + k;
    if (row >= n) return;
    double v = band[i];
    if (row / 6 == j / 6) v -= dup * Bd[(j / 6) * 36 + (row % 6) * 6 + j % 6];
    S[row * n + j] = v;
}
__global__ __launch_bounds__(256) void dedup_dense_kernel(double *__restrict__ S, int64_t n, const double *__restrict__ Bd, double dup) {
    const int64_t i = (int64_t)blockIdx.x * 256 + threadIdx.x;
    if (i >= n * 6) return;
    const int64_t f = i / 36, a = (i % 36) / 6, b = i % 6;
    S[(6 * f + a) * n + 6 * f + b] -= dup * Bd[i];
}
__global__ __launch_bounds__(256) void axpy_kernel(double *__restrict__ y, const double *__restrict__ x, double a, int64_t n) {
    const int64_t i = (int64_t)blockIdx.x * 256 + threadIdx.x;
    if (i < n) y[i] += a * x[i];
}

struct Carve {
    char *p;
    size_t used = 0;
    explicit Carve(void *base) : p((char *)base) {}
    template <class T>
    T *take(size_t count) {
        T *r = p ? (T *)(p + used) : nullptr;
        used += mm_align_up(count * sizeof(T), 256);
        return r;
    }
};

struct TrfWs {
    double *x, *x_new, *g, *si, *gh, *ghs, *gn, *q1, *w, *q2, *s1, *s2;
    double *B, *Bd, *C, *Cd, *Cinv, *u1, *Jq2, *dp, *v, *S;
    double *r0, *r1, *r2, *r3, *d11, *bs, *damp, *board, *cost2, *rowsx;
    int32_t *info;
    void *ws_res, *ws_md, *ws_jvp, *ws_schur, *ws_chol, *ws_back;
    size_t ws_res_b, ws_md_b, ws_jvp_b, ws_schur_b, ws_chol_b, ws_back_b;
    double *exs, *ex;
    size_t ex_count;
    size_t total;
};

TrfWs carve_trf(const mm_ba_problem *pb, void *base, int64_t ex_half_bw = -1) {
    TrfWs t;
    Carve c(base);
    const size_t F = pb->F, P = pb->P, O = (size_t)pb->O, n = 6 * F + 3 * P, nc = 6 * F;
    double **vecs[12] = {&t.x, &t.x_new, &t.g, &t.si, &t.gh, &t.ghs, &t.gn, &t.q1, &t.w, &t.q2, &t.s1, &t.s2};
    for (auto v : vecs) *v = c.take<double>(n + 2);
    t.B = c.take<double>(F * 36);
    t.Bd = c.take<double>(F * 36);
    t.C = c.take<double>(P * 6 + 2);
    t.Cd = c.take<double>(P * 6 + 2);
    t.Cinv = c.take<double>(P * 6 + 2);
    t.u1 = c.take<double>(O * 2 + 2);
    t.Jq2 = c.take<double>(O * 2 + 2);
    t.dp = c.take<double>(P * 3 + 2);
    t.v = c.take<double>(nc + 2);
    t.S = c.take<double>(2 * nc * nc + 2);
    t.r0 = c.take<double>(6);
    t.r1 = c.take<double>(9);
    t.r2 = c.take<double>(6);
    t.r3 = c.take<double>(18);
    t.d11 = c.take<double>(6);
    t.bs = c.take<double>(6);
    t.damp = c.take<double>(2);
    t.board = c.take<double>(16);
    t.cost2 = c.take<double>(1);
    t.rowsx = c.take<double>(3);
    t.info = c.take<int32_t>(1);
    t.ws_res_b = 2048 * 8;
    t.ws_res = c.take<char>(t.ws_res_b);
    t.ws_md_b = mm_multi_dot_workspace_bytes();
    t.ws_md = c.take<char>(t.ws_md_b);
    t.ws_jvp_b = mm_ba_jvp_dots_workspace_bytes(pb);
    t.ws_jvp = c.take<char>(t.ws_jvp_b);
    t.ws_schur_b = mm_ba_schur_workspace_bytes(pb);
    if (t.ws_schur_b < 256) t.ws_schur_b = 256;
    t.ws_schur = c.take<char>(t.ws_schur_b);
    t.ws_chol_b = mm_chol_workspace_bytes((int)nc);
    t.ws_chol = c.take<char>(t.ws_chol_b);
    t.ws_back_b = mm_ba_backsub_workspace_bytes(pb);
    t.ws_back = c.take<char>(t.ws_back_b);
    t.exs = nullptr;
    t.ex = nullptr;
    t.ex_count = 0;
    if (ex_half_bw >= 0) {
        const size_t hb = (size_t)(ex_half_bw < (int64_t)nc - 1 ? ex_half_bw : (nc ? nc - 1 : 0));
        t.ex_count = nc * (hb + 1) + nc;
        if (t.ex_count < F * 42) t.ex_count = F * 42;
        t.exs = c.take<double>(EX_SCALARS);
        t.ex = c.take<double>(t.ex_count + 2);
    }
    t.total = c.used;
    return t;
}

int wait_seq(mm_ctx *ctx, const unsigned long long *word, unsigned long long seq, const char *what, int problem = -1) {
    const auto t0 = std::chrono::steady_clock::now();
    unsigned long spins = 0;
    while (__atomic_load_n(word, __ATOMIC_ACQUIRE) != seq) {
        __builtin_ia32_pause();
        if ((++spins & 0xFFFFF) == 0 && std::chrono::steady_clock::now() - t0 > std::chrono::seconds(20)) {
            MM_HIP(ctx, hipStreamSynchronize(ctx->stream));
            if (__atomic_load_n(word, __ATOMIC_ACQUIRE) == seq) break;
            if (problem < 0) return mm_fail(ctx, MM_ERR_HIP, "%s never arrived", what);
            return mm_fail(ctx, MM_ERR_HIP, "%s %d never arrived", what, problem);
        }
    }
    return MM_OK;
}

using namespace mm_trf;

}

extern "C" size_t mm_ba_trf_workspace_bytes(const mm_ba_problem *pb) {
    if (!pb || pb->F < 0 || pb->P < 0 || pb->O < 0) return 0;
    return carve_trf(pb, nullptr).total;
}

#define TRF_CALL(expr)        \
    do {                      \
        int rc_ = (expr);     \
        if (rc_) return rc_;  \
    } while (0)

extern "C" size_t mm_ba_trf_dist_workspace_bytes(const mm_ba_problem *pb, int half_bandwidth) {
    if (!pb || pb->F < 0 || pb->P < 0 || pb->O < 0 || half_bandwidth < 0) return 0;
    return carve_trf(pb, nullptr, half_bandwidth).total;
}

static int trf_run(mm_ctx *ctx, const mm_ba_problem *pb, double *cams, double *pts, const mm_trf_params *prm, mm_trf_report *rep,
                   mm_trf_row *log, int log_cap, void *ws, size_t ws_bytes, const mm_dist *dist) {
    const auto t_enter = std::chrono::steady_clock::now();
    if (!ctx) return MM_ERR_ARG;
    if (!pb || !cams || !pts || !prm || !rep || pb->F <= 0 || pb->P < 0 || pb->O < 0 || !pb->K || log_cap < 0 || (log_cap > 0 && !log))
        return mm_fail(ctx, MM_ERR_ARG, "mm_ba_trf: bad argument");
    if (dist && (dist->world < 1 || dist->world > EX_MAX_WORLD || dist->rank < 0 || dist->rank >= dist->world || !dist->allreduce ||
                 dist->half_bandwidth < 0))
        return mm_fail(ctx, MM_ERR_ARG, "mm_ba_trf_dist: bad communicator description (1 <= world <= %d)", EX_MAX_WORLD);
    const size_t need = dist ? mm_ba_trf_dist_workspace_bytes(pb, dist->half_bandwidth) : mm_ba_trf_workspace_bytes(pb);
    if (!ws || ws_bytes < need || ((uintptr_t)ws & 255))
        return mm_fail(ctx, MM_ERR_WORKSPACE, "mm_ba_trf: workspace too small or misaligned");
    const TrfWs t = carve_trf(pb, ws, dist ? dist->half_bandwidth : -1);
    struct TableHold {
        mm_ctx *c;
        explicit TableHold(mm_ctx *ctx) : c(ctx) { mm_cam_table_hold(c, true); }
        ~TableHold() { mm_cam_table_hold(c, false); }
    } table_hold(ctx);
    struct FusedGuard {
        mm_ctx *c;
        bool saved, saved_strict, saved_no_event;
        FusedGuard(mm_ctx *ctx, bool sharded)
            : c(ctx), saved(ctx->chol_avoid_fused), saved_strict(ctx->chol_strict_budget), saved_no_event(ctx->fused_no_event) {
            c->fused_no_event = true;
            if (sharded) c->chol_strict_budget = true;
        }
        ~FusedGuard() {
            c->chol_avoid_fused = saved;
            c->chol_strict_budget = saved_strict;
            c->fused_no_event = saved_no_event;
            mm_chol_release_budget(c);
        }
    } fused_guard(ctx, dist != nullptr);
    const int F = pb->F, P = pb->P;
    const int64_t nc = 6 * (int64_t)F, n = nc + 3 * (int64_t)P;
    hipStream_t st = ctx->stream;
    auto pts_of = [&](double *v) { return v + nc; };
    MM_HIP(ctx, hipMemsetAsync(t.ws_md, 0, t.ws_md_b, st));
    MM_HIP(ctx, hipMemsetAsync(t.ws_jvp, 0, t.ws_jvp_b, st));
    MM_HIP(ctx, hipMemsetAsync(t.S, 0, (size_t)(2 * nc * nc) * sizeof(double), st));
    double *x = t.x, *x_new = t.x_new;
    MM_HIP(ctx, hipMemcpyAsync(x, cams, (size_t)nc * sizeof(double), hipMemcpyDeviceToDevice, st));
    if (P) MM_HIP(ctx, hipMemcpyAsync(x + nc, pts, (size_t)3 * P * sizeof(double), hipMemcpyDeviceToDevice, st));
    double host[16];
    rep->chol_fallbacks = 0;
    rep->collectives = 0;
    auto ar = [&](double *buf, int64_t count) -> int {
        ++rep->collectives;
        const int rc = dist->allreduce(dist->user, buf, count);
        return rc ? mm_fail(ctx, MM_ERR_HIP, "mm_ba_trf_dist: the all-reduce callback failed (%d)", rc) : MM_OK;
    };
    auto exchange = [&](std::initializer_list<std::pair<double *, int>> items) -> int {
        if (!dist) return MM_OK;
        ExItems it = {};
        it.rank = dist->rank;
        it.world = dist->world;
        it.info = t.info;
        for (auto &pr : items) {
            it.p[it.n] = pr.first;
            it.kind[it.n] = pr.second;
            ++it.n;
        }
        hipLaunchKernelGGL(ex_pack_kernel, dim3(1), dim3(64), 0, st, it, t.exs);
        TRF_CALL(ar(t.exs, EX_SCALARS));
        hipLaunchKernelGGL(ex_unpack_kernel, dim3(1), dim3(64), 0, st, it, (const double *)t.exs);
        MM_LAUNCH_CHECK(ctx, "ex_unpack_kernel");
        return MM_OK;
    };
    auto normal_eq = [&](double *v) -> int {
        TRF_CALL(mm_ba_normal_eq(ctx, pb, v, pts_of(v), t.B, t.g, t.C, pts_of(t.g)));
        if (!dist) return MM_OK;
        MM_HIP(ctx, hipMemcpyAsync(t.ex, t.B, (size_t)F * 36 * sizeof(double), hipMemcpyDeviceToDevice, st));
        MM_HIP(ctx, hipMemcpyAsync(t.ex + (size_t)F * 36, t.g, (size_t)nc * sizeof(double), hipMemcpyDeviceToDevice, st));
        TRF_CALL(ar(t.ex, (int64_t)F * 42));
        MM_HIP(ctx, hipMemcpyAsync(t.B, t.ex, (size_t)F * 36 * sizeof(double), hipMemcpyDeviceToDevice, st));
        MM_HIP(ctx, hipMemcpyAsync(t.g, t.ex + (size_t)F * 36, (size_t)nc * sizeof(double), hipMemcpyDeviceToDevice, st));
        return MM_OK;
    };
    if (!ctx->host_board) {
        MM_HIP(ctx, hipHostMalloc(&ctx->host_board, sizeof(HostBoard), hipHostMallocDefault));
        memset(ctx->host_board, 0, sizeof(HostBoard));
        ctx->host_board_seq = 0;
    }
    HostBoard *hb = (HostBoard *)ctx->host_board;
    auto take_board = [&](unsigned long long seq, int count) -> int {
        TRF_CALL(wait_seq(ctx, &hb->seq, seq, "mm_ba_trf: the trial-step scalars"));
        for (int i = 0; i < count; ++i) host[i] = ((volatile double *)hb->v)[i];
        mm_chol_release_budget(ctx);
        return MM_OK;
    };
    auto read_board = [&](const double *dev, int count) -> int {
        const unsigned long long seq = ++ctx->host_board_seq;
        hipLaunchKernelGGL(board_publish_kernel, dim3(1), dim3(64), 0, st, dev, count, hb, seq);
        MM_LAUNCH_CHECK(ctx, "board_publish_kernel");
        return take_board(seq, count);
    };
    TRF_CALL(mm_ba_residual(ctx, pb, x, pts_of(x), nullptr, t.cost2, t.ws_res, t.ws_res_b));
    if (dist) {
        const double av = ctx->chol_avoid_fused ? 1.0 : 0.0;
        MM_HIP(ctx, hipMemcpyAsync(t.board + 15, &av, sizeof(double), hipMemcpyHostToDevice, st));
        MM_HIP(ctx, hipStreamSynchronize(st));
        TRF_CALL(exchange({{t.cost2, 3}, {t.board + 15, 3}}));
        TRF_CALL(read_board(t.board + 15, 1));
        if (host[0] > 0) ctx->chol_avoid_fused = true;
    }
    TRF_CALL(read_board(t.cost2, 1));
    const double cost0 = 0.5 * host[0];
    rep->cost0 = cost0;
    if (!std::isfinite(cost0)) {
        rep->status = -2;
        return mm_fail(ctx, MM_ERR_NUMERIC, "mm_ba_trf: residuals are not finite in the initial point");
    }
    const int half_bw = dist ? dist->half_bandwidth : 6 * pb->cam_span + 5;
    TRF_CALL(normal_eq(x));
    TRF_CALL(mm_ba_scale_update(ctx, F, P, t.B, t.C, t.si, 1));
    {
        hipLaunchKernelGGL(vec_mul_kernel, dim3((unsigned)((n + 255) / 256)), dim3(256), 0, st, (const double *)x, (const double *)t.si, t.w, n);
        const double *pa[1] = {t.w}, *pbv[1] = {t.w};
        TRF_CALL(mm_multi_dot(ctx, 1, pa, pbv, n, nc, t.rowsx, t.ws_md, t.ws_md_b));
        TRF_CALL(exchange({{t.rowsx, 0}}));
        TRF_CALL(read_board(t.rowsx, 3));
    }
    TrfDecide d(cost0, host[2], n, *prm, log, log_cap);
    Outcome next = d.begin();
    static const bool timing = getenv("MM_TRF_TIMING") && atoi(getenv("MM_TRF_TIMING")) > 0;
    const auto t_loop = std::chrono::steady_clock::now();
    auto t_iter = t_loop;
    if (timing) fprintf(stderr, "mm_ba_trf timing: prologue %.1f us\n", std::chrono::duration<double, std::micro>(t_loop - t_enter).count());
    for (;;) {
        if (timing && d.iteration > 0) {
            const auto now = std::chrono::steady_clock::now();
            fprintf(stderr, "mm_ba_trf timing: iteration %d %.1f us (nfev %d)\n", d.iteration - 1,
                    std::chrono::duration<double, std::micro>(now - t_iter).count(), d.nfev);
            t_iter = now;
        }
        if (!dist && d.iteration > 0) {
            TRF_CALL(mm_trf_fused0_scaled(ctx, t.g, t.si, t.B, t.C, t.gh, t.ghs, n, nc, t.r0, t.ws_md, t.ws_md_b));
        } else {
            const double *in[2] = {t.g, t.si};
            double *outv[2] = {t.gh, t.ghs};
            TRF_CALL(mm_trf_fused(ctx, 0, in, outv, nullptr, 0, 0, n, nc, t.r0, t.ws_md, t.ws_md_b));
        }
        TRF_CALL(mm_ba_jvp_dots(ctx, pb, x, pts_of(x), t.ghs, pts_of(t.ghs), t.u1, nullptr, t.d11, t.ws_jvp, t.ws_jvp_b));
        TRF_CALL(exchange({{t.r0, 0}, {t.r0 + 3, 2}, {t.d11, 1}, {t.d11 + 3, 1}}));
        if (next == FINAL) {
            TRF_CALL(read_board(t.r0, 6));
            d.on_final(host[5]);
            break;
        }
        double *reg_eff = t.damp + 1;
        bool rows_pending = false;
        auto trial = [&](double Delta_) -> int {
            if (rows_pending) {
                rows_pending = false;
                TRF_CALL(mm_trf_rows_step2d(ctx, ctx->jvp_partial, ctx->jvp_n_wg, t.bs, t.r0, t.d11, t.r1, t.r2, t.r3, reg_eff, t.info, Delta_,
                                            t.board));
            } else {
                TRF_CALL(mm_trf_step2d(ctx, t.r0, t.d11, t.r1, t.r2, t.r3, t.bs, reg_eff, t.info, Delta_, t.board));
            }
            if (F > 0 && !dist) {
                void *ctab = nullptr;
                TRF_CALL(mm_cam_table_adopt(ctx, x_new, (int)F, &ctab));
                TRF_CALL(mm_trf_fused5_coef(ctx, x, t.s1, t.s2, x_new, t.board, n, nc, ctab, (int)F));
            } else {
                const double *in[3] = {x, t.s1, t.s2};
                double *outv[1] = {x_new};
                const double *sc[1] = {t.board};
                TRF_CALL(mm_trf_fused(ctx, 5, in, outv, sc, 0, 0, n, nc, nullptr, t.ws_md, t.ws_md_b));
                mm_cam_table_invalidate(ctx);
            }
            if (!dist) {
                const unsigned long long seq = ++ctx->host_board_seq;
                TRF_CALL(mm_ba_residual_publish(ctx, pb, x_new, pts_of(x_new), t.ws_res, t.ws_res_b, t.board, 14, 16,
                                                ctx->host_board, seq));
                return take_board(seq, 16);
            }
            TRF_CALL(mm_ba_residual(ctx, pb, x_new, pts_of(x_new), nullptr, t.board + 14, t.ws_res, t.ws_res_b));
            TRF_CALL(exchange({{t.board + 14, 3}, {t.board + 15, 4}}));
            return read_board(t.board, 16);
        };
        bool damping_known = false;
        Outcome solve;
        do {
            if (!dist) {
                mm_damp_spec dmp = {t.B, t.C, t.si, nullptr, nullptr, d.Delta, d.min_damping, t.damp, reg_eff};
                if (!damping_known) {
                    dmp.gh2 = t.r0 + 2;
                    dmp.d11 = t.d11 + 2;
                    damping_known = true;
                }
                TRF_CALL(mm_ba_schur_solve_damped(ctx, pb, x, pts_of(x), &dmp, t.Bd, t.Cd, t.g, pts_of(t.g), t.S, t.v, t.Cinv,
                                                  half_bw, t.info, t.ws_schur, t.ws_schur_b, t.ws_chol, t.ws_chol_b));
            } else {
                if (!damping_known) {
                    TRF_CALL(mm_ba_damp_damping(ctx, F, P, t.B, t.C, t.si, t.r0 + 2, t.d11 + 2, d.Delta, d.min_damping, t.damp, t.Bd, t.Cd));
                    damping_known = true;
                } else {
                    TRF_CALL(mm_ba_damp(ctx, F, P, t.B, t.C, t.si, reg_eff, t.Bd, t.Cd));
                }
                TRF_CALL(mm_ba_schur(ctx, pb, x, pts_of(x), t.Bd, t.Cd, t.g, pts_of(t.g), t.S, t.v, t.Cinv, t.ws_schur,
                                     t.ws_schur_b));
                const double dup = (double)(dist->world - 1);
                if (dist->band_exchange) {
                    const int hb = (int)(half_bw < nc - 1 ? half_bw : nc - 1);
                    const int64_t cnt = nc * (hb + 1);
                    hipLaunchKernelGGL(band_pack_kernel, dim3((unsigned)((cnt + 255) / 256)), dim3(256), 0, st, (const double *)t.S, nc, hb, t.ex);
                    MM_HIP(ctx, hipMemcpyAsync(t.ex + cnt, t.v, (size_t)nc * sizeof(double), hipMemcpyDeviceToDevice, st));
                    TRF_CALL(ar(t.ex, cnt + nc));
                    hipLaunchKernelGGL(band_unpack_kernel, dim3((unsigned)((cnt + 255) / 256)), dim3(256), 0, st, t.S, nc, hb,
                                       (const double *)t.ex, (const double *)t.Bd, dup);
                    MM_HIP(ctx, hipMemcpyAsync(t.v, t.ex + cnt, (size_t)nc * sizeof(double), hipMemcpyDeviceToDevice, st));
                } else {
                    MM_HIP(ctx, hipMemcpyAsync(t.S + nc * nc, t.v, (size_t)nc * sizeof(double), hipMemcpyDeviceToDevice, st));
                    TRF_CALL(ar(t.S, nc * nc + nc));
                    MM_HIP(ctx, hipMemcpyAsync(t.v, t.S + nc * nc, (size_t)nc * sizeof(double), hipMemcpyDeviceToDevice, st));
                    hipLaunchKernelGGL(dedup_dense_kernel, dim3((unsigned)((nc * 6 + 255) / 256)), dim3(256), 0, st, t.S, nc,
                                       (const double *)t.Bd, dup);
                }
                hipLaunchKernelGGL(axpy_kernel, dim3((unsigned)((nc + 255) / 256)), dim3(256), 0, st, t.v, (const double *)t.g, -dup, nc);
                MM_LAUNCH_CHECK(ctx, "axpy_kernel");
                TRF_CALL(mm_chol_solve_sym(ctx, t.S, (int)nc, t.v, half_bw, dist->band_exchange ? 0 : 1, t.info, t.ws_chol, t.ws_chol_b));
            }
            TRF_CALL(mm_ba_backsub(ctx, pb, x, pts_of(x), t.Cinv, pts_of(t.g), t.v, t.dp, t.ws_back, t.ws_back_b));
            {
                const double *in[4] = {t.v, t.dp, t.si, t.gh};
                double *outv[2] = {t.gn, t.q1};
                const double *sc[1] = {t.r0 + 2};
                TRF_CALL(mm_trf_fused(ctx, 1, in, outv, sc, 0, 0, n, nc, t.r1, t.ws_md, t.ws_md_b));
                TRF_CALL(exchange({{t.r1, 0}, {t.r1 + 3, 0}}));
            }
            {
                const double *in[2] = {t.gn, t.q1};
                double *outv[1] = {t.w};
                const double *sc[1] = {t.r1 + 2};
                TRF_CALL(mm_trf_fused(ctx, 2, in, outv, sc, 0, 0, n, nc, t.r2, t.ws_md, t.ws_md_b));
                TRF_CALL(exchange({{t.r2, 0}}));
            }
            {
                const double *in[5] = {t.w, t.q1, t.si, t.gh, x};
                double *outv[3] = {t.q2, t.s1, t.s2};
                const double *sc[1] = {t.r2 + 2};
                TRF_CALL(mm_trf_fused(ctx, 3, in, outv, sc, 0, 0, n, nc, t.r3, t.ws_md, t.ws_md_b));
            }
            ctx->jvp_rows_deferred = !dist && P > 0 && pb->O > 0;
            {
                const int rc_ = mm_ba_jvp_dots(ctx, pb, x, pts_of(x), t.s2, pts_of(t.s2), t.Jq2, t.u1, t.bs, t.ws_jvp, t.ws_jvp_b);
                rows_pending = ctx->jvp_rows_deferred;
                ctx->jvp_rows_deferred = false;
                if (rc_) return rc_;
            }
            TRF_CALL(exchange({{t.r3, 0}, {t.r3 + 3, 0}, {t.r3 + 6, 0}, {t.r3 + 9, 0}, {t.r3 + 12, 0}, {t.bs, 1}, {t.bs + 3, 1}}));
            TRF_CALL(trial(d.Delta));
            solve = d.on_solve(dist && host[15] > 0 ? -1 : (int)host[6], host[13], host[10], host[9]);
            if (solve == ABANDONED) {
                if (ctx->chol_avoid_fused) return mm_fail(ctx, MM_ERR_HIP, "mm_ba_trf: the banded factorisation reported info = -1");
                ctx->chol_avoid_fused = true;
                ++rep->chol_fallbacks;
            } else if (solve == RETRY) {
                MM_HIP(ctx, hipMemcpyAsync(t.damp + 1, &d.reg, sizeof(double), hipMemcpyHostToDevice, st));
                MM_HIP(ctx, hipStreamSynchronize(st));
            }
        } while (solve == ABANDONED || solve == RETRY);
        if (solve == INDEFINITE)
            return mm_fail(ctx, MM_ERR_NUMERIC, "mm_ba_trf: reduced camera system is not positive definite (pivot %d)", (int)host[6]);
        if (solve == DONE) break;
        while ((next = d.on_trial(host[2], host[3], host[4], host[14])) == TRIAL) TRF_CALL(trial(d.Delta));
        if (d.accepted) {
            std::swap(x, x_new);
            TRF_CALL(normal_eq(x));
            if (dist) TRF_CALL(mm_ba_scale_update(ctx, F, P, t.B, t.C, t.si, 0));
        }
    }
    MM_HIP(ctx, hipMemcpyAsync(cams, x, (size_t)nc * sizeof(double), hipMemcpyDeviceToDevice, st));
    if (P) MM_HIP(ctx, hipMemcpyAsync(pts, x + nc, (size_t)3 * P * sizeof(double), hipMemcpyDeviceToDevice, st));
    MM_HIP(ctx, hipStreamSynchronize(st));
    if (timing) fprintf(stderr, "mm_ba_trf timing: total %.1f us, %d iterations\n",
                        std::chrono::duration<double, std::micro>(std::chrono::steady_clock::now() - t_enter).count(), d.iteration);
    d.fill(*rep);
    return MM_OK;
}

extern "C" int mm_ba_trf(mm_ctx *ctx, const mm_ba_problem *pb, double *cams, double *pts, const mm_trf_params *prm,
                         mm_trf_report *rep, mm_trf_row *log, int log_cap, void *ws, size_t ws_bytes) {
    return trf_run(ctx, pb, cams, pts, prm, rep, log, log_cap, ws, ws_bytes, nullptr);
}

extern "C" int mm_ba_trf_dist(mm_ctx *ctx, const mm_ba_problem *pb, double *cams, double *pts, const mm_trf_params *prm,
                              mm_trf_report *rep, mm_trf_row *log, int log_cap, void *ws, size_t ws_bytes, const mm_dist *dist) {
    if (!dist) return mm_fail(ctx, MM_ERR_ARG, "mm_ba_trf_dist: null communicator description");
    return trf_run(ctx, pb, cams, pts, prm, rep, log, log_cap, ws, ws_bytes, dist);
}

extern "C" size_t mm_ba_trf_fixed_workspace_bytes(const mm_ba_problem *pb, const mm_ba_fixed *fx) {
    (void)fx;
    return mm_ba_trf_workspace_bytes(pb);
}

extern "C" int mm_ba_trf_fixed(mm_ctx *ctx, const mm_ba_problem *pb, const mm_ba_fixed *fx, double *cams, double *pts,
                               const mm_trf_params *prm, mm_trf_report *rep, mm_trf_row *log, int log_cap, void *ws, size_t ws_bytes) {
    if (!ctx) return MM_ERR_ARG;
    if (!fx || fx->F_fixed == 0) return trf_run(ctx, pb, cams, pts, prm, rep, log, log_cap, ws, ws_bytes, nullptr);
    if (fx->F_fixed < 0 || !fx->cams) return mm_fail(ctx, MM_ERR_ARG, "mm_ba_trf_fixed: bad fixed-camera descriptor");
    if (pb && pb->O > 0 && pb->n_chunks <= 0) return mm_fail(ctx, MM_ERR_ARG, "mm_ba_trf_fixed: the problem needs its co-observation pair list");
    mm_fixed_scope scope(ctx, fx);
    return trf_run(ctx, pb, cams, pts, prm, rep, log, log_cap, ws, ws_bytes, nullptr);
}

namespace {
size_t batch_tables_bytes(const mm_ba_problem *pb) { return 2 * mm_align_up((size_t)pb->F * 5 * sizeof(double), 256); }
}

extern "C" size_t mm_ba_trf_batched_workspace_bytes(const mm_ba_problem *pb) {
    if (!pb || pb->F < 0 || pb->P < 0 || pb->O < 0) return 0;
    return carve_trf(pb, nullptr).total + batch_tables_bytes(pb);
}

extern "C" int mm_ba_trf_batched(mm_ctx *ctx, int n_prob, const mm_ba_problem *const *pbs, double *const *cams, double *const *pts,
                                 const mm_trf_params *prm, mm_trf_report *reports, void *const *ws, const size_t *ws_bytes,
                                 int32_t *solved_alone) {
    if (!ctx) return MM_ERR_ARG;
    if (n_prob < 0 || (n_prob > 0 && (!pbs || !cams || !pts || !prm || !reports || !ws || !ws_bytes)))
        return mm_fail(ctx, MM_ERR_ARG, "mm_ba_trf_batched: bad argument");
    if (n_prob == 0) return MM_OK;
    hipStream_t st = ctx->stream;
    for (int p = 0; p < n_prob; ++p) {
        const mm_ba_problem *pb = pbs[p];
        if (!pb || !cams[p] || !pts[p] || pb->F <= 0 || pb->P < 0 || pb->O < 0 || !pb->K)
            return mm_fail(ctx, MM_ERR_ARG, "mm_ba_trf_batched: bad problem %d", p);
        if (!ws[p] || ws_bytes[p] < mm_ba_trf_batched_workspace_bytes(pb) || ((uintptr_t)ws[p] & 255))
            return mm_fail(ctx, MM_ERR_WORKSPACE, "mm_ba_trf_batched: workspace of problem %d too small or misaligned", p);
        if (solved_alone) solved_alone[p] = 0;
    }
    auto solve_alone = [&](int p) -> int {
        if (solved_alone) solved_alone[p] = 1;
        return trf_run(ctx, pbs[p], cams[p], pts[p], prm, &reports[p], nullptr, 0, ws[p], ws_bytes[p], nullptr);
    };
    std::vector<mm_batch_prob> tab((size_t)n_prob);
    std::vector<TrfWs> tws((size_t)n_prob);
    bool batchable = n_prob > 1;
    for (int p = 0; p < n_prob && batchable; ++p) {
        const mm_ba_problem *pb = pbs[p];
        const TrfWs t = carve_trf(pb, ws[p]);
        tws[p] = t;
        mm_batch_prob &b = tab[p];
        memset(&b, 0, sizeof(b));
        b.pb = *pb;
        b.nc = 6 * (int64_t)pb->F;
        b.n = b.nc + 3 * (int64_t)pb->P;
        b.x = t.x; b.x_new = t.x_new; b.g = t.g; b.si = t.si; b.gh = t.gh; b.ghs = t.ghs; b.gn = t.gn; b.q1 = t.q1; b.w = t.w;
        b.q2 = t.q2; b.s1 = t.s1; b.s2 = t.s2;
        b.B = t.B; b.Bd = t.Bd; b.C = t.C; b.Cd = t.Cd; b.Cinv = t.Cinv; b.u1 = t.u1; b.Jq2 = t.Jq2; b.dp = t.dp; b.v = t.v; b.S = t.S;
        b.r0 = t.r0; b.r1 = t.r1; b.r2 = t.r2; b.r3 = t.r3; b.d11 = t.d11; b.bs = t.bs; b.damp = t.damp; b.board = t.board;
        b.info = t.info;
        char *extra = (char *)ws[p] + t.total;
        b.ctab_x = extra;
        b.ctab_new = extra + mm_align_up((size_t)pb->F * 5 * sizeof(double), 256);
        b.res_partial = (double *)t.ws_res;
        b.md_counter = (unsigned *)t.ws_md;
        b.md_partial = (double *)((char *)t.ws_md + 256);
        b.jvp_partial = (double *)((char *)t.ws_jvp + 256);
        b.backsub_T = (double *)t.ws_back;
        b.half_bw = 6 * pb->cam_span + 5;
        b.g_vec = mm_batch_fused_grid(b.n);
        b.g_scale = (uint32_t)((b.n + 255) / 256);
        b.g_damp = (uint32_t)(((int64_t)pb->F * 36 + (int64_t)pb->P * 6 + 255) / 256);
        mm_batch_ba_setup(&b);
        if (pb->O <= 0 || pb->P <= 0 || mm_batch_schur_setup(ctx, &b, t.ws_schur, t.ws_schur_b) != MM_OK ||
            mm_batch_chol_setup(ctx, &b, t.ws_chol, t.ws_chol_b) != MM_OK)
            batchable = false;
    }
    ctx->batch_last = batchable ? n_prob : 0;
    if (!batchable) {
        if (getenv("MM_BATCH_DEBUG")) fprintf(stderr, "mm_ba_trf_batched: %d problems one by one (%s)\n", n_prob, n_prob > 1 ? ctx->err : "a single problem");
        for (int p = 0; p < n_prob; ++p) TRF_CALL(solve_alone(p));
        return MM_OK;
    }
    const size_t tab_b = mm_align_up((size_t)n_prob * sizeof(mm_batch_prob), 256), dyn_b = mm_align_up((size_t)n_prob * sizeof(mm_batch_dyn), 256);
    const size_t list_b = mm_align_up((size_t)n_prob * sizeof(int32_t), 256);
    constexpr int N_LISTS = 7;
    const size_t dev_need = tab_b + dyn_b + N_LISTS * list_b;
    const size_t host_need = dyn_b + N_LISTS * list_b + (size_t)n_prob * sizeof(HostBoard) + (size_t)n_prob * 4 * sizeof(double);
    if (ctx->batch_dev_cap < dev_need) {
        if (ctx->batch_dev) (void)hipFree(ctx->batch_dev);
        ctx->batch_dev = nullptr;
        ctx->batch_dev_cap = 0;
        MM_HIP(ctx, hipMalloc(&ctx->batch_dev, dev_need));
        ctx->batch_dev_cap = dev_need;
    }
    if (ctx->batch_host_cap < host_need) {
        if (ctx->batch_host) (void)hipHostFree(ctx->batch_host);
        ctx->batch_host = nullptr;
        ctx->batch_host_cap = 0;
        MM_HIP(ctx, hipHostMalloc(&ctx->batch_host, host_need, hipHostMallocDefault));
        ctx->batch_host_cap = host_need;
    }
    char *dbase = (char *)ctx->batch_dev, *hbase = (char *)ctx->batch_host;
    mm_batch_prob *d_tab = (mm_batch_prob *)dbase;
    mm_batch_dyn *d_dyn = (mm_batch_dyn *)(dbase + tab_b);
    int32_t *d_list[N_LISTS];
    for (int q = 0; q < N_LISTS; ++q) d_list[q] = (int32_t *)(dbase + tab_b + dyn_b + q * list_b);
    mm_batch_dyn *h_dyn = (mm_batch_dyn *)hbase;
    int32_t *h_list[N_LISTS];
    for (int q = 0; q < N_LISTS; ++q) h_list[q] = (int32_t *)(hbase + dyn_b + q * list_b);
    HostBoard *mail = (HostBoard *)(hbase + dyn_b + N_LISTS * list_b);
    double *h_init = (double *)(mail + n_prob);
    memset(mail, 0, (size_t)n_prob * sizeof(HostBoard));
    for (int p = 0; p < n_prob; ++p) tab[p].mailbox = &mail[p];
    MM_HIP(ctx, hipMemcpyAsync(d_tab, tab.data(), (size_t)n_prob * sizeof(mm_batch_prob), hipMemcpyHostToDevice, st));
    for (int p = 0; p < n_prob; ++p) {
        const mm_ba_problem *pb = pbs[p];
        const TrfWs &t = tws[p];
        const int64_t nc = tab[p].nc, n = tab[p].n;
        MM_HIP(ctx, hipMemsetAsync(t.ws_md, 0, t.ws_md_b, st));
        MM_HIP(ctx, hipMemsetAsync(t.ws_jvp, 0, t.ws_jvp_b, st));
// ... 133 lines not shown
```

meatmodeler_amd/ops.py:

```python
import ctypes as C
import math
import os

import numpy as np
import torch

from . import _lib
from ._lib import lib, ptr, vp, OrbParams, BAProblem, default_context

ptr_ = ptr


def _i32(t):
    assert t.dtype == torch.int32 and t.is_contiguous()
    return t



def bf_knn2_batched(q, t, nq=None, nt=None, ctx=None):
    ctx = ctx or default_context()
    assert q.dtype == torch.uint8 and t.dtype == torch.uint8 and q.shape[-1] == 32 and t.shape[-1] == 32
    assert q.stride(-1) == 1 and q.stride(-2) == 32 and t.stride(-1) == 1 and t.stride(-2) == 32
    n_pairs, nq_cap, nt_cap = q.shape[0], q.shape[1], t.shape[1]
    assert t.shape[0] == n_pairs
# ... 605 lines not shown
                                        ptr(sel_t) if sel_t is not None else None, int(t_lo), n_sel,
                                        ptr(out_ptr) if out_ptr is not None else None, n_obs, int(frame_offset), ptr(coords),
                                        ptr(fi), ptr(pi)), "mm_flatten_tracks")
    return coords, fi, pi



def ba_build_index(F, P, fi, pi):
    fi = np.ascontiguousarray(fi, np.int32)
    pi = np.ascontiguousarray(pi, np.int32)
    O = fi.size
    pt_ptr = np.zeros(P + 1, np.int32)
    cam_ptr = np.zeros(F + 1, np.int32)
    pt_obs = np.zeros(max(O, 1), np.int32)
    cam_obs = np.zeros(max(O, 1), np.int32)
    i32p = _lib.c_i32p
    rc = lib.mm_ba_build_index(F, P, O, fi.ctypes.data_as(i32p), pi.ctypes.data_as(i32p), pt_ptr.ctypes.data_as(i32p),
                               pt_obs.ctypes.data_as(i32p), cam_ptr.ctypes.data_as(i32p), cam_obs.ctypes.data_as(i32p))
    if rc != 0:
        raise ValueError(f"mm_ba_build_index failed ({rc}): frame/point index out of range")
    return pt_ptr, pt_obs[:O], cam_ptr, cam_obs[:O]


class BADevice:

    def __init__(self, K, fi, pi, obs, F, P, device, ctx=None, pairs=True, max_band_span=192, fixed_cams=None,
                 native_index=True):
        self.ctx = ctx or default_context()
        self._mdot = None
        dev = device
        self.device = dev
        self.F, self.P, self.O = int(F), int(P), int(len(fi))
        F, P, O = self.F, self.P, self.O

        def to_dev(a, dtype):
            if isinstance(a, torch.Tensor):
                return a.to(device=dev, dtype=dtype).contiguous()
            return torch.as_tensor(np.ascontiguousarray(a)).to(device=dev, dtype=dtype).contiguous()

        self.K = to_dev(np.asarray(K, np.float64).reshape(9), torch.float64)
        self.fi = to_dev(fi, torch.int32).reshape(-1)
        self.pi = to_dev(pi, torch.int32).reshape(-1)
        self.obs = to_dev(obs, torch.float64).reshape(-1, 2)
        self.fixed_cams, self.F_fixed, self.fx = None, 0, None
        if fixed_cams is not None:
            assert (isinstance(fixed_cams, torch.Tensor) and fixed_cams.dtype == torch.float64 and fixed_cams.device == dev
                    and fixed_cams.dim() == 2 and fixed_cams.shape[1] == 6), "fixed_cams: [F_fixed, 6] f64 device tensor"
            self.F_fixed = int(fixed_cams.shape[0])
            if self.F_fixed:
                self.fixed_cams = fixed_cams.contiguous()
                self.fx = _lib.BAFixed(self.F_fixed, 0, ptr(self.fixed_cams))
        F_all = F + self.F_fixed
        self.cam_span = 0
        self.max_band_span = int(max_band_span)
        self._slabs, self._slab_src = None, None
        self.n_pairs = 0
        self.overlap = os.environ.get("MM_SCHUR_OVERLAP", "0") != "0"
        self.index_build = "torch"
        if native_index and O and F > 0 and P > 0 and not self.F_fixed and self._build_index_native(pairs):
            self.index_build = "native"
        else:
            self._build_index_torch(pairs, F_all)
        self._ws = torch.empty(2048 * 8, dtype=torch.uint8, device=dev)
        self._cost2 = torch.zeros(1, dtype=torch.float64, device=dev)
        self._S = None
        self._schur_ws = None
        self._chol_ws = None

    @staticmethod
    def _chunk_pairs():
        return max(64, int(os.environ.get("MM_SCHUR_CHUNK", "512")) // 64 * 64)

    @property
    def slabs(self):
        if self._slabs is None and self._slab_src is not None:
            seg_ids, seg_chunk_ptr = self._slab_src
            self._slab_src = None
            self._set_slabs(seg_ids.to(torch.int64), seg_chunk_ptr.to(torch.int64))
        return self._slabs

    def _set_slabs(self, seg_ids, seg_chunk_ptr):
        n_slabs = 8
        cps = -(-self.F // n_slabs)
        if cps >= 16:
            seg_cam = seg_ids // (self.cam_span + 1)
            bounds = torch.arange(n_slabs + 1, dtype=torch.int64, device=self.device) * cps
            sseg = torch.searchsorted(seg_cam, bounds)
            schunk = seg_chunk_ptr[sseg]
            self._slabs = (n_slabs, cps, np.ascontiguousarray(sseg.cpu().numpy(), np.int64),
                           np.ascontiguousarray(schunk.cpu().numpy(), np.int64))

    def _set_pair_list(self, pair_o, pair_o2, pair_p, seg_ids, seg_chunk_ptr, chunk_seg, chunk_begin, chunk_end):
        self.pair_o, self.pair_o2, self.pair_p = pair_o, pair_o2, pair_p
        self.seg_ids, self.seg_chunk_ptr = seg_ids, seg_chunk_ptr
        self.chunk_seg, self.chunk_begin, self.chunk_end = chunk_seg, chunk_begin, chunk_end
        self.n_pairs = int(pair_o.numel())
        self.pb.n_seg = int(seg_ids.numel())
        self.pb.n_chunks = int(chunk_seg.numel())
        self.pb.seg_ids, self.pb.seg_chunk_ptr = ptr(seg_ids), ptr(seg_chunk_ptr)
        self.pb.chunk_seg, self.pb.chunk_begin, self.pb.chunk_end = ptr(chunk_seg), ptr(chunk_begin), ptr(chunk_end)
        self.pb.pair_o, self.pb.pair_o2, self.pb.pair_p = ptr(pair_o), ptr(pair_o2), ptr(pair_p)

    def _build_index_native(self, pairs):
        F, P, O, dev = self.F, self.P, self.O, self.device
        i32 = dict(dtype=torch.int32, device=dev)
        pt_ptr, pt_obs = torch.empty(P + 1, **i32), torch.empty(O, **i32)
        cam_ptr, cam_obs = torch.empty(F + 1, **i32), torch.empty(O, **i32)
        head = torch.empty(8, dtype=torch.int64, device=dev)
        ix = _lib.BAIndex(F, P, O, ptr(self.fi), ptr(self.pi), ptr(pt_ptr), ptr(pt_obs), ptr(cam_ptr), ptr(cam_obs), ptr(head),
                          0, self._chunk_pairs(), 0, None, None, None, None, None, None, None, None)
        ws0b = lib.mm_ba_index_workspace_bytes(self.ctx.h, C.byref(ix), 0)
        if not ws0b:
            raise _lib.MMError("mm_ba_index_workspace_bytes: no workspace size for stage 0")
        ws0 = torch.empty(ws0b, dtype=torch.uint8, device=dev)
        self.ctx.check(lib.mm_ba_index_build(self.ctx.h, C.byref(ix), 0, ptr(ws0), ws0b, None, 0), "mm_ba_index_build")
        span, n, bad_range, not_point_major = head[:4].tolist()
        if bad_range:
            raise ValueError("frame / point index out of range")
        if not_point_major:
            return False
        self.pt_ptr, self.pt_obs, self.cam_ptr, self.cam_obs = pt_ptr, pt_obs, cam_ptr, cam_obs
        self.cam_span = int(span)
        self.pb = BAProblem(F, P, O, ptr(self.K), ptr(self.fi), ptr(self.pi), ptr(self.obs),
                            ptr(self.pt_ptr), ptr(self.pt_obs), ptr(self.cam_ptr), ptr(self.cam_obs),
                            self.cam_span, 0, 0, None, None, 0, None, None, None, None, None, None)
        if pairs and self.cam_span <= self.max_band_span and self.cam_span < F and F * (self.cam_span + 1) < 2 ** 31:
            n = int(n)
            seg_cap, chunk_cap = C.c_int64(0), C.c_int64(0)
            lib.mm_ba_index_bounds(F, self.cam_span, n, ix.chunk, C.byref(seg_cap), C.byref(chunk_cap))
            seg_cap, chunk_cap = seg_cap.value, chunk_cap.value
            pair_o, pair_o2, pair_p = torch.empty(n, **i32), torch.empty(n, **i32), torch.empty(n, **i32)
            seg_ids, seg_chunk_ptr = torch.empty(seg_cap, **i32), torch.empty(seg_cap + 1, **i32)
            chunk_seg, chunk_begin, chunk_end = (torch.empty(chunk_cap, **i32) for _ in range(3))
            ix.cam_span, ix.n_pairs = self.cam_span, n
            ix.pair_o, ix.pair_o2, ix.pair_p = ptr(pair_o), ptr(pair_o2), ptr(pair_p)
            ix.seg_ids, ix.seg_chunk_ptr = ptr(seg_ids), ptr(seg_chunk_ptr)
            ix.chunk_seg, ix.chunk_begin, ix.chunk_end = ptr(chunk_seg), ptr(chunk_begin), ptr(chunk_end)
            ws1b = lib.mm_ba_index_workspace_bytes(self.ctx.h, C.byref(ix), 1)
            if not ws1b:
                raise _lib.MMError("mm_ba_index_workspace_bytes: no workspace size for stage 1")
            ws1 = torch.empty(ws1b, dtype=torch.uint8, device=dev)
            self.ctx.check(lib.mm_ba_index_build(self.ctx.h, C.byref(ix), 1, ptr(ws0), ws0b, ptr(ws1), ws1b), "mm_ba_index_build")
            n_seg, n_chunks = head[4:6].tolist()
            self._set_pair_list(pair_o, pair_o2, pair_p, seg_ids[:n_seg], seg_chunk_ptr[:n_seg + 1], chunk_seg[:n_chunks],
                                chunk_begin[:n_chunks], chunk_end[:n_chunks])
            self._slab_src = (self.seg_ids, self.seg_chunk_ptr)
        return True

    def _build_index_torch(self, pairs, F_all):
        F, P, O, dev = self.F, self.P, self.O, self.device
        max_band_span = self.max_band_span
        i64 = dict(dtype=torch.int64, device=dev)
        if O:
            lim = torch.stack([self.fi.min(), self.fi.max(), self.pi.min(), self.pi.max(),
                               (self.pi[1:] >= self.pi[:-1]).all().to(torch.int32)]).tolist()
            if lim[0] < 0 or lim[1] >= F_all or lim[2] < 0 or lim[3] >= P:
                raise ValueError("frame / point index out of range")
            point_major = bool(lim[4])
        else:
            point_major = True
        if point_major:
            self.pt_obs = torch.arange(O, dtype=torch.int32, device=dev)
        else:
            self.pt_obs = torch.sort(self.pi, stable=True)[1].to(torch.int32)
        self.pt_ptr = torch.zeros(P + 1, dtype=torch.int32, device=dev)
        self.cam_ptr = torch.zeros(F + 1, dtype=torch.int32, device=dev)
        if O and self.F_fixed:
            self.pt_ptr[1:] = torch.cumsum(torch.bincount(self.pi, minlength=P), 0).to(torch.int32)
            self.cam_ptr[1:] = torch.cumsum(torch.bincount(self.fi, minlength=F_all)[:F], 0).to(torch.int32)
            n_free = int(self.cam_ptr[-1].item())
            self.cam_obs = torch.sort(self.fi, stable=True)[1][:n_free].to(torch.int32).contiguous()
        elif O:
            self.pt_ptr[1:] = torch.cumsum(torch.bincount(self.pi, minlength=P), 0).to(torch.int32)
            self.cam_ptr[1:] = torch.cumsum(torch.bincount(self.fi, minlength=F), 0).to(torch.int32)
            self.cam_obs = torch.sort(self.fi, stable=True)[1].to(torch.int32)
        else:
            self.cam_obs = torch.zeros(0, dtype=torch.int32, device=dev)
        self.pb = BAProblem(F, P, O, ptr(self.K), ptr(self.fi), ptr(self.pi), ptr(self.obs),
                            ptr(self.pt_ptr), ptr(self.pt_obs), ptr(self.cam_ptr), ptr(self.cam_obs),
                            0, 0, 0, None, None, 0, None, None, None, None, None, None)
        pair_pb, free_idx, O_pairs = self.pb, None, O
        if O and self.F_fixed:
            free_idx = torch.nonzero(self.fi < F).reshape(-1)
            O_pairs = int(free_idx.numel())
            fi_f, pi_f = self.fi[free_idx].contiguous(), self.pi[free_idx].contiguous()
            pt_ptr_f = torch.zeros(P + 1, dtype=torch.int32, device=dev)
            pt_ptr_f[1:] = torch.cumsum(torch.bincount(pi_f, minlength=P), 0).to(torch.int32)
            pt_obs_f = (torch.arange(O_pairs, dtype=torch.int32, device=dev) if point_major
                        else torch.sort(pi_f, stable=True)[1].to(torch.int32))
            self._pair_src = (fi_f, pi_f, pt_ptr_f, pt_obs_f)
            pair_pb = BAProblem(F, P, O_pairs, ptr(self.K), ptr(fi_f), ptr(pi_f), ptr(self.obs), ptr(pt_ptr_f),
                                ptr(pt_obs_f), ptr(self.cam_ptr), ptr(self.cam_obs),
                                0, 0, 0, None, None, 0, None, None, None, None, None, None)
        if O_pairs:
            cnt = torch.empty(O_pairs, dtype=torch.int32, device=dev)
            span_t = torch.zeros(1, dtype=torch.int32, device=dev)
            self.ctx.check(lib.mm_ba_pairs_count(self.ctx.h, C.byref(pair_pb), ptr(cnt), ptr(span_t)),
                           "mm_ba_pairs_count")
            offs = torch.cumsum(cnt, 0, dtype=torch.int64)
            span, n = torch.stack([span_t[0].to(torch.int64), offs[-1]]).tolist()
            self.cam_span = int(span)
            self.pb.cam_span = self.cam_span
            if pairs and self.cam_span <= max_band_span and self.cam_span < F and F * (self.cam_span + 1) < 2 ** 31:
                key = torch.empty(n, dtype=torch.int32, device=dev)
                po = torch.empty(n, dtype=torch.int32, device=dev)
                po2 = torch.empty(n, dtype=torch.int32, device=dev)
                offs_ex = (offs - cnt).contiguous()
                self.ctx.check(lib.mm_ba_pairs_emit(self.ctx.h, C.byref(pair_pb), ptr(offs_ex), self.cam_span, ptr(key),
                                                    ptr(po), ptr(po2)), "mm_ba_pairs_emit")
                key_s, perm = torch.sort(key, stable=True)
                pair_o, pair_o2 = po[perm].contiguous(), po2[perm].contiguous()
                if free_idx is not None:
                    pair_o = free_idx[pair_o.long()].to(torch.int32).contiguous()
                    pair_o2 = free_idx[pair_o2.long()].to(torch.int32).contiguous()
                seg_ids, counts = torch.unique_consecutive(key_s, return_counts=True)
                seg_hi = torch.cumsum(counts, 0)
                seg_lo = seg_hi - counts
                CH = self._chunk_pairs()
                cntc = (counts + (CH - 1)) // CH
                first_hi = torch.cumsum(cntc, 0)
                first = first_hi - cntc
                nchunks = int(first_hi[-1].item())
                chunk_seg = torch.repeat_interleave(torch.arange(len(seg_ids), **i64), cntc, output_size=nchunks)
                chunk_begin = seg_lo[chunk_seg] + CH * (torch.arange(nchunks, **i64) - first[chunk_seg])
                chunk_end = torch.minimum(chunk_begin + CH, seg_hi[chunk_seg])
                i32 = lambda t: t.to(torch.int32).contiguous()
                pair_p = self.pi[pair_o.long()].contiguous()
                self._set_pair_list(pair_o, pair_o2, pair_p, i32(seg_ids), i32(torch.cat([first, first_hi[-1:]])), i32(chunk_seg),
                                    i32(chunk_begin), i32(chunk_end))
                self._set_slabs(seg_ids.to(torch.int64), torch.cat([first, first_hi[-1:]]))

    def residual(self, cams, pts, want_res=False, cost_out=None):
        res = torch.empty((self.O, 2), dtype=torch.float64, device=self.device) if want_res else None
        cost2 = cost_out if cost_out is not None else torch.empty(1, dtype=torch.float64, device=self.device)
        if self.fx is not None:
            self.ctx.check(lib.mm_ba_residual_fixed(self.ctx.h, C.byref(self.pb), C.byref(self.fx), ptr(cams), ptr(pts),
                                                    ptr(res), ptr(cost2), ptr(self._ws), self._ws.numel()),
                           "mm_ba_residual_fixed")
            return cost2, res
        self.ctx.check(lib.mm_ba_residual(self.ctx.h, C.byref(self.pb), ptr(cams), ptr(pts), ptr(res), ptr(cost2),
                                          ptr(self._ws), self._ws.numel()), "mm_ba_residual")
        return cost2, res

    def _no_fixed(self, what):
        if self.fx is not None:
            raise NotImplementedError(f"BADevice.{what}: no fixed-camera form (residual, normal_eq and trf_solve have one)")

    def jacobian(self, cams, pts):
        self._no_fixed("jacobian")
        Jc = torch.empty((self.O, 2, 6), dtype=torch.float64, device=self.device)
        Jp = torch.empty((self.O, 2, 3), dtype=torch.float64, device=self.device)
        self.ctx.check(lib.mm_ba_jacobian(self.ctx.h, C.byref(self.pb), ptr(cams), ptr(pts), ptr(Jc), ptr(Jp)),
                       "mm_ba_jacobian")
        return Jc, Jp

    def normal_eq(self, cams, pts, want_cams=True, want_pts=True, out=None):
        d = self.device
        if out is not None:
            B, gc, Cb, gp = out
            for t_ in out:
                assert t_ is None or (t_.dtype == torch.float64 and t_.is_contiguous())
        else:
            B = torch.empty((self.F, 6, 6), dtype=torch.float64, device=d) if want_cams else None
            gc = torch.empty((self.F, 6), dtype=torch.float64, device=d) if want_cams else None
            Cb = torch.empty((self.P, 6), dtype=torch.float64, device=d) if want_pts else None
            gp = torch.empty((self.P, 3), dtype=torch.float64, device=d) if want_pts else None
        if self.fx is not None:
            self.ctx.check(lib.mm_ba_normal_eq_fixed(self.ctx.h, C.byref(self.pb), C.byref(self.fx), ptr(cams), ptr(pts),
                                                     ptr(B), ptr(gc), ptr(Cb), ptr(gp)), "mm_ba_normal_eq_fixed")
            return B, gc, Cb, gp
        self.ctx.check(lib.mm_ba_normal_eq(self.ctx.h, C.byref(self.pb), ptr(cams), ptr(pts), ptr(B), ptr(gc), ptr(Cb),
                                           ptr(gp)), "mm_ba_normal_eq")
        return B, gc, Cb, gp

    def jvp(self, cams, pts, wc, wp):
        self._no_fixed("jvp")
        out = torch.empty((self.O, 2), dtype=torch.float64, device=self.device)
        self.ctx.check(lib.mm_ba_jvp(self.ctx.h, C.byref(self.pb), ptr(cams), ptr(pts), ptr(wc), ptr(wp), ptr(out)),
                       "mm_ba_jvp")
        return out

    def jvp_dots(self, cams, pts, wc, wp, other=None):
        self._no_fixed("jvp_dots")
        out = torch.empty((self.O, 2), dtype=torch.float64, device=self.device)
        rows = torch.empty((2, 3), dtype=torch.float64, device=self.device)
        if getattr(self, "_jvp_ws", None) is None:
            self._jvp_ws = torch.zeros(lib.mm_ba_jvp_dots_workspace_bytes(C.byref(self.pb)), dtype=torch.uint8,
                                       device=self.device)
        self.ctx.check(lib.mm_ba_jvp_dots(self.ctx.h, C.byref(self.pb), ptr(cams), ptr(pts), ptr(wc), ptr(wp), ptr(out),
                                          ptr(other), ptr(rows), ptr(self._jvp_ws), self._jvp_ws.numel()), "mm_ba_jvp_dots")
        return out, rows

    def schur(self, cams, pts, Bd, Cd, gc, gp):
        self._no_fixed("schur")
        n = 6 * self.F
        S = self._schur_buffers(n)
        v = torch.empty(n, dtype=torch.float64, device=self.device)
        Cinv = torch.empty((self.P, 6), dtype=torch.float64, device=self.device)
        self.ctx.check(lib.mm_ba_schur(self.ctx.h, C.byref(self.pb), ptr(cams), ptr(pts), ptr(Bd), ptr(Cd), ptr(gc),
                                       ptr(gp), ptr(S), ptr(v), ptr(Cinv), ptr(self._schur_ws),
                                       self._schur_ws.numel()), "mm_ba_schur")
        return S, v, Cinv

    def _alloc_S(self, n):
        self._S_storage = torch.zeros(2 * n * n, dtype=torch.float64, device=self.device)
        self._S = self._S_storage[:n * n].view(n, n)

    def _schur_buffers(self, n):
        if self._S is None:
            self._alloc_S(n)
        if self._schur_ws is None:
            nb = lib.mm_ba_schur_workspace_bytes(C.byref(self.pb))
            self._schur_ws = torch.empty(max(nb, 256), dtype=torch.uint8, device=self.device)
        return self._S

    def band_view(self, half_bandwidth):
        n = 6 * self.F
        hb = int(min(half_bandwidth, n - 1))
        return torch.as_strided(self._S_storage, (n, hb + 1), (n + 1, n))

    def schur_solve(self, cams, pts, Bd, Cd, gc, gp, half_bandwidth):
        self._no_fixed("schur_solve")
        n = 6 * self.F
        self._schur_buffers(n)
        v = torch.empty(n, dtype=torch.float64, device=self.device)
        Cinv = torch.empty((self.P, 6), dtype=torch.float64, device=self.device)
        info = torch.zeros(1, dtype=torch.int32, device=self.device)
        if self._chol_ws is None:
            self._chol_ws = torch.empty(lib.mm_chol_workspace_bytes(n), dtype=torch.uint8, device=self.device)
        hb = int(min(half_bandwidth, n))
        if self.overlap and self.slabs is not None:
            ns, cps, sseg, schunk = self.slabs
            a_seg, a_chunk = sseg.ctypes.data_as(_lib.c_i64p), schunk.ctypes.data_as(_lib.c_i64p)
        else:
            ns, cps, a_seg, a_chunk = 0, 0, None, None
        self.ctx.check(lib.mm_ba_schur_solve(self.ctx.h, C.byref(self.pb), ptr(cams), ptr(pts), ptr(Bd), ptr(Cd), ptr(gc),
                                             ptr(gp), ptr(self._S), ptr(v), ptr(Cinv), hb, ptr(info), ptr(self._schur_ws),
                                             self._schur_ws.numel(), ptr(self._chol_ws), self._chol_ws.numel(), ns, cps,
                                             a_seg, a_chunk), "mm_ba_schur_solve")
        return info, v, Cinv

    def multi_dot(self, pairs, split=0):
        if self._mdot is None:
            self._mdot = MultiDot(self.device, self.ctx)
        return self._mdot(pairs, split)

    _FUSED_ROWS = (2, 3, 2, 6, 0, 0)

    def trf_fused(self, op, ins, outs, scalars=(), h0=0.0, h1=0.0, split=0):
        if self._mdot is None:
            self._mdot = MultiDot(self.device, self.ctx)
        ws = self._mdot.ws
        n = outs[0].numel()
        for t in list(ins) + list(outs) + list(scalars):
            assert t.dtype == torch.float64 and t.is_contiguous()
        pin = (C.c_void_p * len(ins))(*[t.data_ptr() for t in ins])
        pout = (C.c_void_p * len(outs))(*[t.data_ptr() for t in outs])
        psc = (C.c_void_p * max(len(scalars), 1))(*[t.data_ptr() for t in scalars]) if scalars else None
        rows = self._FUSED_ROWS[op]
        if n == 0:
            return torch.zeros((max(rows, 1), 3), dtype=torch.float64, device=self.device)
        res = torch.empty((max(rows, 1), 3), dtype=torch.float64, device=self.device)
        self.ctx.check(lib.mm_trf_fused(self.ctx.h, op, pin, pout, psc, float(h0), float(h1), n, int(split), ptr(res), ptr(ws),
                                        ws.numel()), "mm_trf_fused")
        return res

    def trf_step2d(self, r0, d11, r1, r2, r3, bs, reg, info, Delta, board):
        self.ctx.check(lib.mm_trf_step2d(self.ctx.h, ptr(r0), ptr(d11), ptr(r1), ptr(r2), ptr(r3), ptr(bs), ptr(reg),
                                         ptr(info), float(Delta), ptr(board)), "mm_trf_step2d")

    def trf_damping(self, gh2, d11, Delta, min_damping):
        return trf_damping(gh2, d11, Delta, min_damping, self.ctx)

    def chol_solve(self, S, v, half_bandwidth=None):
        return chol_solve(S, v, self.ctx, half_bandwidth=half_bandwidth)

    def scale_update(self, B, Cb, si, first):
        self.ctx.check(lib.mm_ba_scale_update(self.ctx.h, self.F, self.P, ptr(B), ptr(Cb), ptr(si), 1 if first else 0),
                       "mm_ba_scale_update")
        return si

    def damp(self, B, Cb, si, reg, Bd, Cd):
        assert reg.dtype == torch.float64 and reg.numel() == 1
        self.ctx.check(lib.mm_ba_damp(self.ctx.h, self.F, self.P, ptr(B), ptr(Cb), ptr(si), ptr(reg), ptr(Bd), ptr(Cd)),
                       "mm_ba_damp")
        return Bd, Cd

    def chol_solve_sym(self, S, v, half_bandwidth, both_triangles):
        return chol_solve_sym(S, v, self.ctx, half_bandwidth, both_triangles)

    def trf_solve(self, cams, pts, ftol, xtol, gtol, max_nfev=None, min_damping=1e-9, log_cap=0):
        for t in (cams, pts):
            assert t.dtype == torch.float64 and t.is_contiguous() and t.device == self.device
        if getattr(self, "_trf_ws", None) is None:
            nb = (lib.mm_ba_trf_fixed_workspace_bytes(C.byref(self.pb), C.byref(self.fx)) if self.fx is not None
                  else lib.mm_ba_trf_workspace_bytes(C.byref(self.pb)))
            self._trf_ws = torch.empty(nb, dtype=torch.uint8, device=self.device)
        prm = _lib.TrfParams(ftol, xtol, gtol, min_damping, int(max_nfev) if max_nfev else 0)
        rep = _lib.TrfReport()
        log = (_lib.TrfRow * max(log_cap, 1))()
        if self.fx is not None:
            name = "mm_ba_trf_fixed"
            rc = lib.mm_ba_trf_fixed(self.ctx.h, C.byref(self.pb), C.byref(self.fx), ptr(cams), ptr(pts), C.byref(prm),
                                     C.byref(rep), log, int(log_cap), ptr(self._trf_ws), self._trf_ws.numel())
        else:
            name = "mm_ba_trf"
            rc = lib.mm_ba_trf(self.ctx.h, C.byref(self.pb), ptr(cams), ptr(pts), C.byref(prm), C.byref(rep), log,
                               int(log_cap), ptr(self._trf_ws), self._trf_ws.numel())
        if rc and rep.status == -2:
            raise ValueError("Residuals are not finite in the initial point.")
        self.ctx.check(rc, name)
        rows = [(r.iteration, r.nfev, r.cost, r.reduction, r.step_norm, r.optimality)
                for r in log[:min(rep.log_rows, log_cap)]]
        return rep, rows

    def trf_solve_dist(self, cams, pts, ftol, xtol, gtol, allreduce, half_bandwidth, band_exchange, max_nfev=None,
                       min_damping=1e-9, log_cap=0):
        self._no_fixed("trf_solve_dist")
        for t in (cams, pts):
            assert t.dtype == torch.float64 and t.is_contiguous() and t.device == self.device
        need = lib.mm_ba_trf_dist_workspace_bytes(C.byref(self.pb), int(half_bandwidth))
        if getattr(self, "_trf_ws_dist", None) is None or self._trf_ws_dist.numel() < need:
            self._trf_ws_dist = torch.empty(need, dtype=torch.uint8, device=self.device)
        ws = self._trf_ws_dist
        base = ws.data_ptr()
        err = []

        def _cb(user, buf, count):
            try:
                off = int(buf) - base
                with torch.cuda.stream(self.ctx.stream):
                    allreduce(ws[off:off + 8 * int(count)].view(torch.float64))
                return 0
            except BaseException as e:
                err.append(e)
                return 1
        cb = _lib.ALLREDUCE_FN(_cb)
        d = _lib.Dist(int(getattr(allreduce, "rank", 0)), int(getattr(allreduce, "world_size", 1)), int(half_bandwidth),
                      1 if band_exchange else 0, cb, None)
        prm = _lib.TrfParams(ftol, xtol, gtol, min_damping, int(max_nfev) if max_nfev else 0)
        rep = _lib.TrfReport()
        log = (_lib.TrfRow * max(log_cap, 1))()
        rc = lib.mm_ba_trf_dist(self.ctx.h, C.byref(self.pb), ptr(cams), ptr(pts), C.byref(prm), C.byref(rep), log,
                                int(log_cap), ptr(ws), ws.numel(), C.byref(d))
        if err:
            raise err[0]
        if rc and rep.status == -2:
            raise ValueError("Residuals are not finite in the initial point.")
        self.ctx.check(rc, "mm_ba_trf_dist")
        rows = [(r.iteration, r.nfev, r.cost, r.reduction, r.step_norm, r.optimality)
                for r in log[:min(rep.log_rows, log_cap)]]
        return rep, rows

    def backsub(self, cams, pts, Cinv, gp, dc):
        self._no_fixed("backsub")
        dp = torch.empty((self.P, 3), dtype=torch.float64, device=self.device)
        if getattr(self, "_backsub_ws", None) is None:
            self._backsub_ws = torch.empty(lib.mm_ba_backsub_workspace_bytes(C.byref(self.pb)), dtype=torch.uint8,
                                           device=self.device)
        self.ctx.check(lib.mm_ba_backsub(self.ctx.h, C.byref(self.pb), ptr(cams), ptr(pts), ptr(Cinv), ptr(gp), ptr(dc),
                                         ptr(dp), ptr(self._backsub_ws), self._backsub_ws.numel()), "mm_ba_backsub")
        return dp


def trf_solve_batched(problems, cams_list, pts_list, ftol, xtol, gtol, max_nfev=None, min_damping=1e-9, ctx=None):
    n = len(problems)
    if n == 0:
        return [], []
    ctx = ctx or problems[0].ctx
    dev = problems[0].device
    pbs = (C.POINTER(_lib.BAProblem) * n)()
    cams_p, pts_p, ws_p = (C.c_void_p * n)(), (C.c_void_p * n)(), (C.c_void_p * n)()
    ws_b = (C.c_size_t * n)()
    keep = []
    for k, (pb, cm, pt) in enumerate(zip(problems, cams_list, pts_list)):
        for t in (cm, pt):
            assert t.dtype == torch.float64 and t.is_contiguous() and t.device == dev
        assert pb.device == dev
        need = lib.mm_ba_trf_batched_workspace_bytes(C.byref(pb.pb))
        if getattr(pb, "_trf_ws", None) is None or pb._trf_ws.numel() < need:
            pb._trf_ws = torch.empty(need, dtype=torch.uint8, device=dev)
        pbs[k] = C.pointer(pb.pb)
        cams_p[k], pts_p[k], ws_p[k], ws_b[k] = cm.data_ptr(), pt.data_ptr(), pb._trf_ws.data_ptr(), pb._trf_ws.numel()
        keep.append(pb._trf_ws)
    prm = _lib.TrfParams(ftol, xtol, gtol, min_damping, int(max_nfev) if max_nfev else 0)
    reps = (_lib.TrfReport * n)()
    alone = (C.c_int32 * n)()
    rc = lib.mm_ba_trf_batched(ctx.h, n, pbs, cams_p, pts_p, C.byref(prm), reps, ws_p, ws_b, alone)
    if rc and any(r.status == -2 for r in reps):
        raise ValueError("Residuals are not finite in the initial point.")
    ctx.check(rc, "mm_ba_trf_batched")
    return list(reps), [bool(a) for a in alone]


class MultiDot:

    def __init__(self, device, ctx=None):
        self.ctx = ctx or default_context()
        self.ws = torch.zeros(lib.mm_multi_dot_workspace_bytes(), dtype=torch.uint8, device=device)

    def __call__(self, pairs, split=0):
        out_all = []
        for i0 in range(0, len(pairs), 8):
            chunk = pairs[i0:i0 + 8]
            k = len(chunk)
            n = chunk[0][0].numel()
            if n == 0:
                out_all.append(torch.zeros((k, 3), dtype=torch.float64, device=self.ws.device))
                continue
            for a, b in chunk:
                assert a.dtype == torch.float64 and b.dtype == torch.float64 and a.is_contiguous() and b.is_contiguous()
                assert a.numel() == n and b.numel() == n
            pa = (C.c_void_p * k)(*[a.data_ptr() for a, _ in chunk])
            pb_ = (C.c_void_p * k)(*[b.data_ptr() for _, b in chunk])
            out = torch.empty((k, 3), dtype=torch.float64, device=self.ws.device)
            self.ctx.check(lib.mm_multi_dot(self.ctx.h, k, pa, pb_, n, int(split), ptr(out), ptr(self.ws), self.ws.numel()),
                           "mm_multi_dot")
            out_all.append(out)
        return out_all[0] if len(out_all) == 1 else torch.cat(out_all)


def trf_damping(gh2, d11, Delta, min_damping, ctx=None):
    ctx = ctx or default_context()
    out = torch.empty(2, dtype=torch.float64, device=gh2.device)
    ctx.check(lib.mm_trf_damping(ctx.h, ptr(gh2), ptr(d11), float(Delta), float(min_damping), ptr(out)), "mm_trf_damping")
    return out


def chol_solve(A, b, ctx=None, half_bandwidth=None):
    ctx = ctx or default_context()
    n = A.shape[0]
    assert A.dtype == torch.float64 and A.is_contiguous() and b.is_contiguous() and b.shape[-1] == n
    nrhs = 1 if b.dim() == 1 else b.shape[0]
    info = torch.zeros(1, dtype=torch.int32, device=A.device)
    wsb = lib.mm_chol_workspace_bytes(n)
    ws = torch.empty(wsb, dtype=torch.uint8, device=A.device)
    hb = n if half_bandwidth is None else int(min(half_bandwidth, n))
    ctx.check(lib.mm_chol_solve(ctx.h, ptr(A), n, ptr(b), nrhs, hb, ptr(info), ptr(ws), wsb), "mm_chol_solve")
    return info


def chol_solve_sym(A, b, ctx=None, half_bandwidth=None, both_triangles=True):
    ctx = ctx or default_context()
    n = A.shape[0]
    assert A.dtype == torch.float64 and A.is_contiguous() and b.is_contiguous() and b.dim() == 1 and b.shape[0] == n
    info = torch.zeros(1, dtype=torch.int32, device=A.device)
    wsb = lib.mm_chol_workspace_bytes(n)
    ws = torch.empty(wsb, dtype=torch.uint8, device=A.device)
    hb = n if half_bandwidth is None else int(min(half_bandwidth, n))
    ctx.check(lib.mm_chol_solve_sym(ctx.h, ptr(A), n, ptr(b), hb, 1 if both_triangles else 0, ptr(info), ptr(ws), wsb),
              "mm_chol_solve_sym")
    return info



def pyramid(img, max_level, ctx=None):
    ctx = ctx or default_context()
    assert img.dtype == torch.uint8 and img.dim() == 2 and img.is_contiguous()
    levels = [img]
    for _ in range(int(max_level)):
        s = levels[-1]
        h, w = s.shape
        d = torch.empty(((h + 1) // 2, (w + 1) // 2), dtype=torch.uint8, device=s.device)
        ctx.check(lib.mm_pyr_down(ctx.h, ptr(s), w, h, s.stride(0), ptr(d), d.stride(0)), "mm_pyr_down")
        levels.append(d)
    return levels


def lk_track(prev_levels, next_levels, pts, win=(21, 21), max_count=30, epsilon=0.01, ctx=None):
    ctx = ctx or default_context()
    L = len(prev_levels)
    assert len(next_levels) == L and pts.dtype == torch.float32 and pts.is_contiguous() and pts.shape[-1] == 2
    n = pts.shape[0]
    d = pts.device
    out = torch.empty((n, 2), dtype=torch.float32, device=d)
    st = torch.empty(n, dtype=torch.uint8, device=d)
    err = torch.empty(n, dtype=torch.float32, device=d)
    if n == 0:
        return out, st, err
    arr_p = (C.c_void_p * L)(*[t.data_ptr() for t in prev_levels])
    arr_n = (C.c_void_p * L)(*[t.data_ptr() for t in next_levels])
    ws = (C.c_int * L)(*[t.shape[1] for t in prev_levels])
    hs = (C.c_int * L)(*[t.shape[0] for t in prev_levels])
    ps = (C.c_int * L)(*[t.stride(0) for t in prev_levels])
    for a, b in zip(prev_levels, next_levels):
        assert a.shape == b.shape and a.stride(0) == b.stride(0)
    eps = min(max(float(epsilon), 0.0), 10.0) ** 2
    ctx.check(lib.mm_lk_track(ctx.h, arr_p, arr_n, ws, hs, ps, L, ptr(pts), n, int(win[0]), int(win[1]),
                              min(max(int(max_count), 0), 100), eps, ptr(out), ptr(st), ptr(err)), "mm_lk_track")
    return out, st, err


def min_eig(img, block_size=3, ctx=None):
    ctx = ctx or default_context()
    assert img.dtype == torch.uint8 and img.dim() == 2 and img.stride(1) == 1
    h, w = img.shape
    eig = torch.empty((h, w), dtype=torch.float64, device=img.device)
    ctx.check(lib.mm_min_eig(ctx.h, ptr(img), w, h, img.stride(0), int(block_size), ptr(eig)), "mm_min_eig")
    return eig


def good_features(img, max_corners, quality, min_distance, block_size=3, ctx=None):
    ctx = ctx or default_context()
    h, w = img.shape
    if h < 3 or w < 3:
        return np.zeros((0, 2), np.float32)
# ... 53 lines not shown
```

Before: 8875 billion descriptor pairs/s (match stage).

## Split Schur pair chunks into short/long lists with a dedicated short-chunk kernel

Adds a one-time ordering kernel at the start of the TRF solve. It classifies pair chunks into long and short ones, and the counts are held on the context. When an order is held, the Schur build dispatches short chunks to a new one-wavefront kernel that reduces through shared memory, and long chunks go through the existing pair kernel. The per-pair math is factored into shared device helpers. The aim is to cut wasted lanes and load imbalance on chunks with few pairs, at the cost of an extra launch, a host readback of the counts, and more state on the context.

```diff
diff --git a/meatmodeler_amd/_lib.py b/meatmodeler_amd/_lib.py
--- a/meatmodeler_amd/_lib.py
+++ b/meatmodeler_amd/_lib.py
@@ -113,6 +113,9 @@
                 ("log_rows", C.c_int32), ("chol_fallbacks", C.c_int32), ("collectives", C.c_int32), ("reserved", C.c_int32)]
 
 
+INTERNAL_SIGNATURES = {
+    "mm_ba_schur_held_debug": (C.c_int, [vp, C.POINTER(BAProblem), vp, vp, vp, vp, vp, vp, vp, vp, vp, vp, C.c_size_t, c_i64p]),
+}
 SIGNATURES = {
     "mm_abi_version": (C.c_int, []),
     "mm_ctx_create": (C.c_int, [C.c_int, vp, C.POINTER(vp)]),
@@ -235,7 +238,7 @@
             f"{LIB_PATH} is missing: the HIP extension has not been built "
             "(make -C meatmodeler_amd/csrc).  meatmodeler_amd has no CPU fallback.")
     lib = C.CDLL(LIB_PATH)
-    for name, (res, args) in SIGNATURES.items():
+    for name, (res, args) in list(SIGNATURES.items()) + list(INTERNAL_SIGNATURES.items()):
         fn = getattr(lib, name)
         fn.restype = res
         fn.argtypes = args
diff --git a/meatmodeler_amd/csrc/mm_common.h b/meatmodeler_amd/csrc/mm_common.h
--- a/meatmodeler_amd/csrc/mm_common.h
+++ b/meatmodeler_amd/csrc/mm_common.h
@@ -45,6 +45,8 @@
     unsigned jvp_n_wg = 0;
     const void *chol_init_done = nullptr;
     int chol_init_sides = 0;
+    const void *schur_order_ws = nullptr, *schur_order_for = nullptr;
+    int64_t schur_n_long = 0, schur_n_short = 0;
     int batch_last = -1;
 };
 
@@ -128,6 +130,11 @@
                              double *Bd, double *Cd, const double *gc, const double *gp, double *S, double *v, double *Cinv,
                              int half_bandwidth, int32_t *info, void *ws_schur, size_t ws_schur_bytes, void *ws_chol,
                              size_t ws_chol_bytes);
+int mm_ba_schur_order(mm_ctx *ctx, const mm_ba_problem *pb, void *ws_schur, size_t ws_schur_bytes, double *counts_out, bool *launched);
+void mm_ba_schur_order_hold(mm_ctx *ctx, const mm_ba_problem *pb, const void *ws_schur, int64_t n_long, int64_t n_short);
+extern "C" int mm_ba_schur_held_debug(mm_ctx *ctx, const mm_ba_problem *pb, const double *cams, const double *pts, const double *Bd,
+                                      const double *Cd, const double *gc, const double *gp, double *S, double *v, double *Cinv,
+                                      void *ws, size_t ws_bytes, int64_t *counts_host);
 int mm_chol_solve_gated(mm_ctx *ctx, double *A, int n, double *b, int nrhs, int half_bandwidth, int32_t *info, void *ws,
                         size_t ws_bytes, const int32_t *slab_ready, int cams_per_slab, int n_cams, int sym_mode);
 
diff --git a/meatmodeler_amd/csrc/schur.hip b/meatmodeler_amd/csrc/schur.hip
--- a/meatmodeler_amd/csrc/schur.hip
+++ b/meatmodeler_amd/csrc/schur.hip
@@ -199,6 +199,121 @@
     return v;
 }
 template <bool FORCE_UNIFORM>
+__device__ __forceinline__ ChunkDesc load_chunk_desc(const ChunkDesc *__restrict__ desc, int64_t c, bool live) {
+    ChunkDesc cd = {};
+    if (live) cd = desc[c];
+    if (FORCE_UNIFORM) {
+        cd.i = __builtin_amdgcn_readfirstlane(cd.i);
+        cd.f2 = __builtin_amdgcn_readfirstlane(cd.f2);
+        cd.e_begin = __builtin_amdgcn_readfirstlane(cd.e_begin);
+        cd.e_end = __builtin_amdgcn_readfirstlane(cd.e_end);
+        cd.sidx = __builtin_amdgcn_readfirstlane(cd.sidx);
+        cd.c_first = __builtin_amdgcn_readfirstlane(cd.c_first);
+        cd.n_ch = __builtin_amdgcn_readfirstlane(cd.n_ch);
+    }
+    return cd;
+}
+__device__ __forceinline__ int pair_point(const mm_ba_problem &pb, int e) { return pb.pair_p ? pb.pair_p[e] : pb.pi[pb.pair_o[e]]; }
+__device__ __forceinline__ bool pair_self(const mm_ba_problem &pb, int d, int e) { return d == 0 && pb.pair_o[e] == pb.pair_o2[e]; }
+__device__ __forceinline__ void load_jr_slab(double *slab, const double *__restrict__ camtab, int i, int f2, int lane) {
+    if (lane < 9) slab[lane] = camtab[(size_t)i * CAMTAB2 + 12 + lane];
+    else if (lane >= 16 && lane < 25) slab[lane] = camtab[(size_t)f2 * CAMTAB2 + 12 + lane - 16];
+}
+__device__ __forceinline__ void load_pair_point(const double *__restrict__ pts, const double *__restrict__ Cinv,
+                                                const double *__restrict__ gp, int d, int p, double (&x)[12]) {
+    if (p >= 0) {
+        const double *Xp = pts + (size_t)p * 3, *ci = Cinv + (size_t)p * 6;
+        x[0] = Xp[0];
+        x[1] = Xp[1];
+        x[2] = Xp[2];
+#pragma unroll
+        for (int q = 0; q < 6; ++q) x[3 + q] = ci[q];
+        if (d == 0) {
+            x[9] = gp[(size_t)p * 3];
+            x[10] = gp[(size_t)p * 3 + 1];
+            x[11] = gp[(size_t)p * 3 + 2];
+        }
+    }
+}
+__device__ __forceinline__ void pair_factors(const CamPQ &cp_i, const CamPQ &cp_2, const double *__restrict__ Ks,
+                                             const double *__restrict__ Jr_i, const double *__restrict__ Jr_2, int d, bool self,
+                                             const double (&x)[12], double (&Jc)[2][6], double (&T)[2][6], double (&z)[2]) {
+    const double X0 = x[0], X1 = x[1], X2 = x[2];
+    const double q00 = x[3], q01 = x[4], q02 = x[5], q11 = x[6], q12 = x[7], q22 = x[8];
+    LeanJ a;
+    lean_eval(cp_i, Ks, Jr_i, X0, X1, X2, a);
+    double Z[2][3];
+#pragma unroll
+    for (int m = 0; m < 2; ++m) {
+        Z[m][0] = a.Jp[m][0] * q00 + a.Jp[m][1] * q01 + a.Jp[m][2] * q02;
+        Z[m][1] = a.Jp[m][0] * q01 + a.Jp[m][1] * q11 + a.Jp[m][2] * q12;
+        Z[m][2] = a.Jp[m][0] * q02 + a.Jp[m][1] * q12 + a.Jp[m][2] * q22;
+    }
+    double M[2][2];
+    z[0] = 0.0;
+    z[1] = 0.0;
+    if (d == 0) {
+        if (self) {
+            const double g0 = x[9], g1 = x[10], g2 = x[11];
+            z[0] = fma(Z[0][2], g2, fma(Z[0][0], g0, Z[0][1] * g1));
+            z[1] = fma(Z[1][2], g2, fma(Z[1][0], g0, Z[1][1] * g1));
+        }
+#pragma unroll
+        for (int m = 0; m < 2; ++m)
+#pragma unroll
+            for (int n_ = 0; n_ < 2; ++n_) M[m][n_] = Z[m][0] * a.Jp[n_][0] + Z[m][1] * a.Jp[n_][1] + Z[m][2] * a.Jp[n_][2];
+#pragma unroll
+        for (int b = 0; b < 6; ++b) {
+            T[0][b] = M[0][0] * a.Jc[0][b] + M[0][1] * a.Jc[1][b];
+            T[1][b] = M[1][0] * a.Jc[0][b] + M[1][1] * a.Jc[1][b];
+        }
+    } else {
+        LeanJ b2;
+        lean_eval(cp_2, Ks, Jr_2, X0, X1, X2, b2);
+#pragma unroll
+        for (int m = 0; m < 2; ++m)
+#pragma unroll
+            for (int n_ = 0; n_ < 2; ++n_) M[m][n_] = Z[m][0] * b2.Jp[n_][0] + Z[m][1] * b2.Jp[n_][1] + Z[m][2] * b2.Jp[n_][2];
+#pragma unroll
+        for (int b = 0; b < 6; ++b) {
+            T[0][b] = M[0][0] * b2.Jc[0][b] + M[0][1] * b2.Jc[1][b];
+            T[1][b] = M[1][0] * b2.Jc[0][b] + M[1][1] * b2.Jc[1][b];
+        }
+    }
+#pragma unroll
+    for (int m = 0; m < 2; ++m)
+#pragma unroll
+        for (int q = 0; q < 6; ++q) Jc[m][q] = a.Jc[m][q];
+}
+__device__ __forceinline__ double pair_block_term(const double (&Jc)[2][6], const double (&T)[2][6], int q, int b) {
+    return Jc[0][q] * T[0][b] + Jc[1][q] * T[1][b];
+}
+__device__ __forceinline__ double pair_rhs_term(const double (&Jc)[2][6], const double (&z)[2], int q) {
+    return fma(Jc[0][q], z[0], Jc[1][q] * z[1]);
+}
+__device__ __forceinline__ void store_segment_total(int q, double sum, int i, int f2, int d, size_t n, const double *__restrict__ Bd,
+                                                    const double *__restrict__ gc, double *S, double *v, bool through) {
+    if (q < 36) {
+        double val = -sum;
+        if (d == 0) val += Bd[(size_t)i * 36 + q];
+        double *dst = S + ((size_t)i * 6 + q / 6) * n + (size_t)f2 * 6 + q % 6;
+        double *mir = S + ((size_t)f2 * 6 + q % 6) * n + (size_t)i * 6 + q / 6;
+        if (through) {
+            __hip_atomic_store(dst, val, __ATOMIC_RELAXED, __HIP_MEMORY_SCOPE_AGENT);
+            if (d != 0) __hip_atomic_store(mir, val, __ATOMIC_RELAXED, __HIP_MEMORY_SCOPE_AGENT);
+        } else {
+            *dst = val;
+            if (d != 0) *mir = val;
+        }
+    } else if (d == 0) {
+        double *dst = v + (size_t)i * 6 + (q - 36);
+        const double val = gc[(size_t)i * 6 + (q - 36)] - sum;
+        if (through) __hip_atomic_store(dst, val, __ATOMIC_RELAXED, __HIP_MEMORY_SCOPE_AGENT);
+        else *dst = val;
+    }
+}
+
+template <bool FORCE_UNIFORM>
 __device__ __forceinline__ void schur_pairs_body(const mm_ba_problem pb, const double *__restrict__ camtab,
                                                                     const ChunkDesc *__restrict__ desc,
                                                                     const double *__restrict__ pts,
@@ -218,21 +333,11 @@
     const unsigned wg = (gpos & 1) ? wg_total - 1 - (gpos >> 1) : (gpos >> 1);
     const int64_t c = (int64_t)wg * SP_WAVES + wv;
     const bool live = c < pb.n_chunks;
-    ChunkDesc cd = {};
-    if (live) cd = desc[c];
-    if (FORCE_UNIFORM) {
-        cd.i = __builtin_amdgcn_readfirstlane(cd.i);
-        cd.f2 = __builtin_amdgcn_readfirstlane(cd.f2);
-        cd.e_begin = __builtin_amdgcn_readfirstlane(cd.e_begin);
-        cd.e_end = __builtin_amdgcn_readfirstlane(cd.e_end);
-        cd.sidx = __builtin_amdgcn_readfirstlane(cd.sidx);
-        cd.c_first = __builtin_amdgcn_readfirstlane(cd.c_first);
-        cd.n_ch = __builtin_amdgcn_readfirstlane(cd.n_ch);
-    }
+    const ChunkDesc cd = load_chunk_desc<FORCE_UNIFORM>(desc, c, live);
     const int i = cd.i, f2 = cd.f2, d = cd.i - cd.f2, sidx = cd.sidx;
     const int e_begin = cd.e_begin, e_end = cd.e_end;
-    auto point_of = [&](int e) { return pb.pair_p ? pb.pair_p[e] : pb.pi[pb.pair_o[e]]; };
-    auto self_of = [&](int e) { return d == 0 && pb.pair_o[e] == pb.pair_o2[e]; };
+    auto point_of = [&](int e) { return pair_point(pb, e); };
+    auto self_of = [&](int e) { return pair_self(pb, d, e); };
     int e = e_begin + lane;
     int p_next = -1;
     bool self_next = false;
@@ -241,8 +346,7 @@
             p_next = point_of(e);
             self_next = self_of(e);
         }
-        if (lane < 9) jrs[wv][lane] = camtab[(size_t)i * CAMTAB2 + 12 + lane];
-        else if (lane >= 16 && lane < 25) jrs[wv][lane] = camtab[(size_t)f2 * CAMTAB2 + 12 + lane - 16];
+        load_jr_slab(jrs[wv], camtab, i, f2, lane);
     }
     __syncthreads();
     if (!live) return;
@@ -251,67 +355,18 @@
     double acc[42];
 #pragma unroll
     for (int q = 0; q < 42; ++q) acc[q] = 0.0;
-    auto load_xc = [&](int p, double (&x)[12]) {
-        if (p >= 0) {
-            const double *Xp = pts + (size_t)p * 3, *ci = Cinv + (size_t)p * 6;
-            x[0] = Xp[0];
-            x[1] = Xp[1];
-            x[2] = Xp[2];
-#pragma unroll
-            for (int q = 0; q < 6; ++q) x[3 + q] = ci[q];
-            if (d == 0) {
-                x[9] = gp[(size_t)p * 3];
-                x[10] = gp[(size_t)p * 3 + 1];
-                x[11] = gp[(size_t)p * 3 + 2];
-            }
-        }
-    };
-    auto pair_body = [&](int p, bool self, const double (&x)[12]) {
-        const double X0 = x[0], X1 = x[1], X2 = x[2];
-        const double q00 = x[3], q01 = x[4], q02 = x[5], q11 = x[6], q12 = x[7], q22 = x[8];
-        LeanJ a;
-        lean_eval(cp_i, Ks, Jr_i, X0, X1, X2, a);
-        double Z[2][3];
-#pragma unroll
-        for (int m = 0; m < 2; ++m) {
-            Z[m][0] = a.Jp[m][0] * q00 + a.Jp[m][1] * q01 + a.Jp[m][2] * q02;
-            Z[m][1] = a.Jp[m][0] * q01 + a.Jp[m][1] * q11 + a.Jp[m][2] * q12;
-            Z[m][2] = a.Jp[m][0] * q02 + a.Jp[m][1] * q12 + a.Jp[m][2] * q22;
-        }
-        double M[2][2], T[2][6];
-        if (d == 0) {
-            if (self) {
-                const double g0 = x[9], g1 = x[10], g2 = x[11];
-                const double z0 = Z[0][0] * g0 + Z[0][1] * g1 + Z[0][2] * g2, z1 = Z[1][0] * g0 + Z[1][1] * g1 + Z[1][2] * g2;
-#pragma unroll
-                for (int q = 0; q < 6; ++q) acc[36 + q] += a.Jc[0][q] * z0 + a.Jc[1][q] * z1;
-            }
-#pragma unroll
-            for (int m = 0; m < 2; ++m)
-#pragma unroll
-                for (int n_ = 0; n_ < 2; ++n_) M[m][n_] = Z[m][0] * a.Jp[n_][0] + Z[m][1] * a.Jp[n_][1] + Z[m][2] * a.Jp[n_][2];
-#pragma unroll
-            for (int b = 0; b < 6; ++b) {
-                T[0][b] = M[0][0] * a.Jc[0][b] + M[0][1] * a.Jc[1][b];
-                T[1][b] = M[1][0] * a.Jc[0][b] + M[1][1] * a.Jc[1][b];
-            }
-        } else {
-            LeanJ b2;
-            lean_eval(cp_2, Ks, Jr_2, X0, X1, X2, b2);
-#pragma unroll
-            for (int m = 0; m < 2; ++m)
-#pragma unroll
-                for (int n_ = 0; n_ < 2; ++n_) M[m][n_] = Z[m][0] * b2.Jp[n_][0] + Z[m][1] * b2.Jp[n_][1] + Z[m][2] * b2.Jp[n_][2];
-#pragma unroll
-            for (int b = 0; b < 6; ++b) {
-                T[0][b] = M[0][0] * b2.Jc[0][b] + M[0][1] * b2.Jc[1][b];
-                T[1][b] = M[1][0] * b2.Jc[0][b] + M[1][1] * b2.Jc[1][b];
-            }
+    auto load_xc = [&](int p, double (&x)[12]) { load_pair_point(pts, Cinv, gp, d, p, x); };
+    auto pair_body = [&](bool self, const double (&x)[12]) {
+        double Jc[2][6], T[2][6], z[2];
+        pair_factors(cp_i, cp_2, Ks, Jr_i, Jr_2, d, self, x, Jc, T, z);
+        if (d == 0 && self) {
+#pragma unroll
+            for (int q = 0; q < 6; ++q) acc[36 + q] += pair_rhs_term(Jc, z, q);
         }
 #pragma unroll
         for (int q = 0; q < 6; ++q)
 #pragma unroll
-            for (int b = 0; b < 6; ++b) acc[q * 6 + b] += a.Jc[0][q] * T[0][b] + a.Jc[1][q] * T[1][b];
+            for (int b = 0; b < 6; ++b) acc[q * 6 + b] += pair_block_term(Jc, T, q, b);
     };
     double xc[12];
     load_xc(p_next, xc);
@@ -329,7 +384,7 @@
         const int p_nn_e = e + 128;
         const int p_nn = p_nn_e < e_end ? point_of(p_nn_e) : -1;
         const bool self_nn = p_nn_e < e_end && self_of(p_nn_e);
-        if (p_cur >= 0) pair_body(p_cur, self_cur, xc);
+        if (p_cur >= 0) pair_body(self_cur, xc);
 #pragma unroll
         for (int q = 0; q < 12; ++q) xc[q] = xn[q];
         p_cur = p_next;
@@ -367,25 +422,7 @@
 #pragma unroll
         for (int h = 0; h < 2; ++h) {
             const int q = 21 * h + lane;
-            const double sum = h == 0 ? tot0 : tot1;
-            if (q < 36) {
-                double val = -sum;
-                if (d == 0) val += Bd[(size_t)i * 36 + q];
-                double *dst = S + ((size_t)i * 6 + q / 6) * n + (size_t)f2 * 6 + q % 6;
-                double *mir = S + ((size_t)f2 * 6 + q % 6) * n + (size_t)i * 6 + q / 6;
-                if (through) {
-                    __hip_atomic_store(dst, val, __ATOMIC_RELAXED, __HIP_MEMORY_SCOPE_AGENT);
-                    if (d != 0) __hip_atomic_store(mir, val, __ATOMIC_RELAXED, __HIP_MEMORY_SCOPE_AGENT);
-                } else {
-                    *dst = val;
-                    if (d != 0) *mir = val;
-                }
-            } else if (d == 0) {
-                double *dst = v + (size_t)i * 6 + (q - 36);
-                const double val = gc[(size_t)i * 6 + (q - 36)] - sum;
-                if (through) __hip_atomic_store(dst, val, __ATOMIC_RELAXED, __HIP_MEMORY_SCOPE_AGENT);
-                else *dst = val;
-            }
+            store_segment_total(q, h == 0 ? tot0 : tot1, i, f2, d, n, Bd, gc, S, v, through);
         }
     }
     if (slabs.ready) {
@@ -417,21 +454,117 @@
                      bp.g, bp.S, bp.v, bp.schur_seg_done, none, 0u, bp.g_pairs, blockIdx.x);
 }
 
-
+constexpr int SH_ROWS = 14;
+__global__ __launch_bounds__(64, 4) void schur_pairs_short_kernel(mm_ba_problem pb, const double *__restrict__ camtab,
+                                                                  const ChunkDesc *__restrict__ desc,
+                                                                  const double *__restrict__ pts,
+                                                                  const double *__restrict__ Cinv,
+                                                                  const double *__restrict__ gp, const double *__restrict__ Bd,
+                                                                  const double *__restrict__ gc, double *S, double *v,
+                                                                  unsigned pos_begin, unsigned pos_end) {
+    __shared__ double red[SH_ROWS * RED_LD];
+    const int lane = threadIdx.x;
+    const int64_t c = (int64_t)blockIdx.x + pos_begin;
+    if (c >= pos_end) return;
+    const ChunkDesc cd = load_chunk_desc<false>(desc, c, true);
+    const int i = cd.i, f2 = cd.f2, d = cd.i - cd.f2;
+    const int e = cd.e_begin + lane;
+    int p = -1;
+    bool self = false;
+    if (e < cd.e_end) {
+        p = pair_point(pb, e);
+        self = pair_self(pb, d, e);
+    }
+    const CamPQ cp_i = cam_pq_scalar<false>(camtab + (size_t)i * CAMTAB2), cp_2 = cam_pq_scalar<false>(camtab + (size_t)f2 * CAMTAB2);
+    double x[12] = {};
+    load_pair_point(pts, Cinv, gp, d, p, x);
+    double Jc[2][6], T[2][6], z[2];
+    pair_factors(cp_i, cp_2, pb.K, camtab + (size_t)i * CAMTAB2 + 12, camtab + (size_t)f2 * CAMTAB2 + 12, d, self, x, Jc, T, z);
+    const bool on = p >= 0;
+    double rhs[6] = {0.0, 0.0, 0.0, 0.0, 0.0, 0.0};
+    if (d == 0 && self) {
+#pragma unroll
+        for (int q = 0; q < 6; ++q) rhs[q] = pair_rhs_term(Jc, z, q);
+    }
+    const int j_end = (cd.e_end - cd.e_begin + 3) & ~3;
+    const size_t n = (size_t)pb.F * 6;
+#pragma unroll
+    for (int h = 0; h < 3; ++h) {
+#pragma unroll
+        for (int r = 0; r < SH_ROWS; ++r) {
+            const int q = SH_ROWS * h + r;
+            if (q < 36) red[r * RED_LD + lane] = on ? pair_block_term(Jc, T, q / 6, q % 6) : 0.0;
+            else if (d == 0) red[r * RED_LD + lane] = rhs[q - 36];
+        }
+        wave_lds_barrier();
+        const int rows = h < 2 || d == 0 ? SH_ROWS : 36 - 2 * SH_ROWS;
+        if (lane < rows) {
+            const double *row = red + lane * RED_LD;
+            double s0 = 0.0, s1 = 0.0, s2 = 0.0, s3 = 0.0;
+            for (int j = 0; j < j_end; j += 4) {
+                s0 += row[j];
+                s1 += row[j + 1];
+                s2 += row[j + 2];
+                s3 += row[j + 3];
+            }
+            store_segment_total(SH_ROWS * h + lane, (s0 + s1) + (s2 + s3), i, f2, d, n, Bd, gc, S, v, false);
+        }
+        if (h < 2) wave_lds_barrier();
+    }
+}
+
+
+__device__ __forceinline__ int chunk_desc_record(const mm_ba_problem &pb, int64_t k, int32_t *__restrict__ o) {
+    const int sidx = pb.chunk_seg[k], seg = pb.seg_ids[sidx];
+    const int ci = seg / (pb.cam_span + 1), cdd = seg % (pb.cam_span + 1);
+    const int c_first = pb.seg_chunk_ptr[sidx];
+    o[0] = ci;
+    o[1] = ci - cdd;
+    o[2] = pb.chunk_begin[k];
+    o[3] = pb.chunk_end[k];
+    o[4] = sidx;
+    o[5] = c_first;
+    o[6] = pb.seg_chunk_ptr[sidx + 1] - c_first;
+    o[7] = 0;
+    return c_first;
+}
 __device__ __forceinline__ void write_chunk_desc(const mm_ba_problem &pb, int32_t *__restrict__ desc, int64_t first, int64_t stride) {
-    for (int64_t k = first; k < pb.n_chunks; k += stride) {
-        const int sidx = pb.chunk_seg[k], seg = pb.seg_ids[sidx];
-        const int ci = seg / (pb.cam_span + 1), cdd = seg % (pb.cam_span + 1);
-        const int c_first = pb.seg_chunk_ptr[sidx];
-        int32_t *o = desc + 8 * k;
-        o[0] = ci;
-        o[1] = ci - cdd;
-        o[2] = pb.chunk_begin[k];
-        o[3] = pb.chunk_end[k];
-        o[4] = sidx;
-        o[5] = c_first;
-        o[6] = pb.seg_chunk_ptr[sidx + 1] - c_first;
-        o[7] = 0;
+    for (int64_t k = first; k < pb.n_chunks; k += stride) chunk_desc_record(pb, k, desc + 8 * k);
+}
+constexpr int ORDER_THREADS = 1024;
+__device__ __forceinline__ bool chunk_is_short(const mm_ba_problem &pb, int64_t k) {
+    const int sidx = pb.chunk_seg[k];
+    return pb.seg_chunk_ptr[sidx + 1] - pb.seg_chunk_ptr[sidx] == 1 && pb.chunk_end[k] - pb.chunk_begin[k] <= 64;
+}
+__global__ __launch_bounds__(ORDER_THREADS) void schur_order_kernel(mm_ba_problem pb, int32_t *__restrict__ desc,
+                                                                    double *__restrict__ counts_out) {
+    __shared__ int32_t scan[ORDER_THREADS];
+    const int tid = threadIdx.x;
+    const int64_t per = (pb.n_chunks + ORDER_THREADS - 1) / ORDER_THREADS;
+    const int64_t k0 = tid * per < pb.n_chunks ? tid * per : pb.n_chunks, k1 = k0 + per < pb.n_chunks ? k0 + per : pb.n_chunks;
+    int32_t mine = 0;
+    for (int64_t k = k0; k < k1; ++k) mine += !chunk_is_short(pb, k);
+    scan[tid] = mine;
+    __syncthreads();
+    for (int off = 1; off < ORDER_THREADS; off <<= 1) {
+        const int32_t add = tid >= off ? scan[tid - off] : 0;
+        __syncthreads();
+        scan[tid] += add;
+        __syncthreads();
+    }
+    const int64_t n_long = scan[ORDER_THREADS - 1];
+    int64_t long_before = scan[tid] - mine;
+    for (int64_t k = k0; k < k1; ++k) {
+        const bool sh = chunk_is_short(pb, k);
+        const int64_t pos = sh ? n_long + (k - long_before) : long_before;
+        int32_t *o = desc + 8 * pos;
+        const int c_first = chunk_desc_record(pb, k, o);
+        o[5] = (int32_t)(pos - (k - c_first));
+        long_before += !sh;
+    }
+    if (tid == 0) {
+        counts_out[0] = (double)n_long;
+        counts_out[1] = (double)(pb.n_chunks - n_long);
     }
 }
 struct PrepExtra {
@@ -653,18 +786,65 @@
     pl.ws_bytes = carve_schur_ws(pl.ws, (char *)ws, pb);
     return pl;
 }
-int launch_prepare(mm_ctx *ctx, const mm_ba_problem *pb, const SchurPlan &pl, const double *cams, const double *Bd, const double *Cd,
-                   const double *gc, double *Cinv, double *S, double *v) {
+struct HeldOrder {
+    bool held;
+    bool split;
+    unsigned n_long, n_short;
+};
+HeldOrder held_order(const mm_ctx *ctx, const mm_ba_problem *pb, const SchurPlan &pl, const void *ws) {
+    static const bool no_split = [] { const char *e = getenv("MM_SCHUR_SPLIT"); return e && atoi(e) == 0; }();
+    HeldOrder h = {};
+    h.held = pl.pairs && SP_WAVES == 1 && ws && ctx->schur_order_ws == ws && ctx->schur_order_for == pb->chunk_begin &&
+             (int64_t)ctx->schur_n_long + ctx->schur_n_short == pb->n_chunks;
+    if (h.held) {
+        h.split = !no_split;
+        h.n_long = (unsigned)ctx->schur_n_long;
+        h.n_short = (unsigned)ctx->schur_n_short;
+    }
+    return h;
+}
+int launch_prepare(mm_ctx *ctx, const mm_ba_problem *pb, const SchurPlan &pl, const HeldOrder &ho, const double *cams, const double *Bd,
+                   const double *Cd, const double *gc, double *Cinv, double *S, double *v) {
     MM_LAUNCH(ctx, "schur_prepare_kernel", schur_prepare_kernel, dim3(pl.g_prep), dim3(256), 0, *pb, cams, const_cast<double *>(Bd), Cd, gc,
-              Cinv, S, v, pl.ws.camtab, pl.ws.seg_done, pl.ws.desc);
+              Cinv, S, v, pl.ws.camtab, pl.ws.seg_done, ho.held ? nullptr : pl.ws.desc);
     return MM_OK;
 }
 int launch_pairs(mm_ctx *ctx, const mm_ba_problem *pb, const SchurPlan &pl, const double *pts, const double *Cinv, const double *gp,
-                 const double *Bd, const double *gc, double *S, double *v, const SlabSync &slabs, unsigned wg_begin, unsigned wg_count) {
+                 const double *Bd, const double *gc, double *S, double *v, const SlabSync &slabs, unsigned wg_begin, unsigned wg_count,
+                 unsigned wg_total) {
     MM_LAUNCH(ctx, "schur_pairs_kernel", schur_pairs_kernel, dim3(wg_count), dim3(64 * SP_WAVES), 0, *pb, (const double *)pl.ws.camtab,
-              (const ChunkDesc *)pl.ws.desc, pts, Cinv, gp, pl.ws.partial, Bd, gc, S, v, pl.ws.seg_done, slabs, wg_begin, pl.g_pairs);
+              (const ChunkDesc *)pl.ws.desc, pts, Cinv, gp, pl.ws.partial, Bd, gc, S, v, pl.ws.seg_done, slabs, wg_begin, wg_total);
     return MM_OK;
 }
+int launch_build(mm_ctx *ctx, const mm_ba_problem *pb, const SchurPlan &pl, const HeldOrder &ho, const double *pts, const double *Cinv,
+                 const double *gp, const double *Bd, const double *gc, double *S, double *v) {
+    if (!(ho.held && ho.split)) return launch_pairs(ctx, pb, pl, pts, Cinv, gp, Bd, gc, S, v, SlabSync{}, 0u, pl.g_pairs, pl.g_pairs);
+    if (ho.n_long > 0)
+        if (int rc = launch_pairs(ctx, pb, pl, pts, Cinv, gp, Bd, gc, S, v, SlabSync{}, 0u, ho.n_long, ho.n_long)) return rc;
+    if (ho.n_short > 0)
+        MM_LAUNCH(ctx, "schur_pairs_kernel", schur_pairs_short_kernel, dim3(ho.n_short), dim3(64), 0, *pb, (const double *)pl.ws.camtab,
+                  (const ChunkDesc *)pl.ws.desc, pts, Cinv, gp, Bd, gc, S, v, ho.n_long, ho.n_long + ho.n_short);
+    return MM_OK;
+}
+}
+
+int mm_ba_schur_order(mm_ctx *ctx, const mm_ba_problem *pb, void *ws_schur, size_t ws_schur_bytes, double *counts_out, bool *launched) {
+    if (!ctx) return MM_ERR_ARG;
+    if (!pb || !counts_out || !launched) return mm_fail(ctx, MM_ERR_ARG, "mm_ba_schur_order: bad argument");
+    *launched = false;
+    const SchurPlan pl = schur_plan(pb, ws_schur);
+    if (!pl.pairs || SP_WAVES != 1 || !ws_schur || ws_schur_bytes < pl.ws_bytes || pb->n_chunks > 0x7fffffffLL) return MM_OK;
+    mm_ba_schur_order_hold(ctx, nullptr, nullptr, 0, 0);
+    MM_LAUNCH(ctx, "schur_order_kernel", schur_order_kernel, dim3(1), dim3(ORDER_THREADS), 0, *pb, pl.ws.desc, counts_out);
+    *launched = true;
+    return MM_OK;
+}
+void mm_ba_schur_order_hold(mm_ctx *ctx, const mm_ba_problem *pb, const void *ws_schur, int64_t n_long, int64_t n_short) {
+    const bool on = pb && ws_schur && n_long >= 0 && n_short >= 0 && n_long + n_short == pb->n_chunks;
+    ctx->schur_order_ws = on ? ws_schur : nullptr;
+    ctx->schur_order_for = on ? pb->chunk_begin : nullptr;
+    ctx->schur_n_long = on ? n_long : 0;
+    ctx->schur_n_short = on ? n_short : 0;
 }
 
 extern "C" size_t mm_ba_schur_workspace_bytes(const mm_ba_problem *pb) {
@@ -685,8 +865,9 @@
     if (pl.pairs) {
         if (!ws || ws_bytes < pl.ws_bytes) return mm_fail(ctx, MM_ERR_WORKSPACE, "mm_ba_schur: workspace too small");
         MM_HIP(ctx, hipMemsetAsync(S, 0, (size_t)pb->F * 6 * pb->F * 6 * sizeof(double), ctx->stream));
-        if (int rc = launch_prepare(ctx, pb, pl, cams, Bd, Cd, gc, Cinv, S, v)) return rc;
-        return launch_pairs(ctx, pb, pl, pts, Cinv, gp, Bd, gc, S, v, SlabSync{}, 0u, pl.g_pairs);
+        const HeldOrder ho = held_order(ctx, pb, pl, ws);
+        if (int rc = launch_prepare(ctx, pb, pl, ho, cams, Bd, Cd, gc, Cinv, S, v)) return rc;
+        return launch_build(ctx, pb, pl, ho, pts, Cinv, gp, Bd, gc, S, v);
     }
     if (pb->P > 0)
         MM_LAUNCH(ctx, "point_inverse_kernel", point_inverse_kernel, dim3((pb->P + 255) / 256), dim3(256), 0, pb->P, Cd,
@@ -695,6 +876,27 @@
     MM_LAUNCH(ctx, "schur_rows_kernel", schur_rows_kernel, dim3(pb->F, nwin), dim3(256), 0, *pb, cams, pts, Bd, Cinv, gc,
               gp, S, v);
     return MM_OK;
+}
+
+extern "C" int mm_ba_schur_held_debug(mm_ctx *ctx, const mm_ba_problem *pb, const double *cams, const double *pts, const double *Bd,
+                                      const double *Cd, const double *gc, const double *gp, double *S, double *v, double *Cinv,
+                                      void *ws, size_t ws_bytes, int64_t *counts_host) {
+    if (!ctx) return MM_ERR_ARG;
+    if (!pb || !counts_host || !ws) return mm_fail(ctx, MM_ERR_ARG, "mm_ba_schur_held_debug: bad argument");
+    const SchurPlan pl = schur_plan(pb, ws);
+    if (!pl.pairs || ws_bytes < pl.ws_bytes) return mm_fail(ctx, MM_ERR_ARG, "mm_ba_schur_held_debug: no pair list or workspace too small");
+    bool launched = false;
+    if (int rc = mm_ba_schur_order(ctx, pb, ws, ws_bytes, pl.ws.partial, &launched)) return rc;
+    if (!launched) return mm_fail(ctx, MM_ERR_ARG, "mm_ba_schur_held_debug: no launch order for this problem");
+    double counts[2] = {0.0, 0.0};
+    MM_HIP(ctx, hipMemcpyAsync(counts, pl.ws.partial, sizeof(counts), hipMemcpyDeviceToHost, ctx->stream));
+    MM_HIP(ctx, hipStreamSynchronize(ctx->stream));
+    counts_host[0] = (int64_t)counts[0];
+    counts_host[1] = (int64_t)counts[1];
+    mm_ba_schur_order_hold(ctx, pb, ws, counts_host[0], counts_host[1]);
+    const int rc = mm_ba_schur(ctx, pb, cams, pts, Bd, Cd, gc, gp, S, v, Cinv, ws, ws_bytes);
+    mm_ba_schur_order_hold(ctx, nullptr, nullptr, 0, 0);
+    return rc;
 }
 
 extern "C" int mm_ba_schur_solve(mm_ctx *ctx, const mm_ba_problem *pb, const double *cams, const double *pts,
@@ -732,12 +934,13 @@
     for (int sl = 0; sl < n_slabs; ++sl) slabs.seg_count[sl] = (int32_t)(slab_seg_ptr[sl + 1] - slab_seg_ptr[sl]);
     MM_HIP(ctx, hipMemsetAsync(S, 0, (size_t)n * n * sizeof(double), ctx->stream));
     MM_HIP(ctx, hipMemsetAsync(pl.ws.slab_ready, 0, 2 * MAX_SLABS * sizeof(int32_t), ctx->stream));
-    if (int rc = launch_prepare(ctx, pb, pl, cams, Bd, Cd, gc, Cinv, S, v)) return rc;
+    if (ctx->schur_order_ws == ws_schur) mm_ba_schur_order_hold(ctx, nullptr, nullptr, 0, 0);
+    if (int rc = launch_prepare(ctx, pb, pl, HeldOrder{}, cams, Bd, Cd, gc, Cinv, S, v)) return rc;
     for (int sl = 0; sl < n_slabs; ++sl)
         if (slabs.seg_count[sl] == 0) MM_LAUNCH(ctx, "slab_flag_kernel", slab_flag_kernel, dim3(1), dim3(1), 0, pl.ws.slab_ready, sl);
     const unsigned wg_first = pl.g_pairs / 2;
     if (wg_first > 0)
-        if (int rc = launch_pairs(ctx, pb, pl, pts, Cinv, gp, Bd, gc, S, v, slabs, 0u, wg_first)) return rc;
+        if (int rc = launch_pairs(ctx, pb, pl, pts, Cinv, gp, Bd, gc, S, v, slabs, 0u, wg_first, pl.g_pairs)) return rc;
     MM_HIP(ctx, hipEventRecord(ctx->ev_fork, ctx->stream));
     MM_HIP(ctx, hipStreamWaitEvent(ctx->aux, ctx->ev_fork, 0));
     {
@@ -750,7 +953,7 @@
         }
         MM_HIP(ctx, hipEventRecord(ctx->ev_join, ctx->aux));
     }
-    if (int rc = launch_pairs(ctx, pb, pl, pts, Cinv, gp, Bd, gc, S, v, slabs, wg_first, pl.g_pairs - wg_first)) return rc;
+    if (int rc = launch_pairs(ctx, pb, pl, pts, Cinv, gp, Bd, gc, S, v, slabs, wg_first, pl.g_pairs - wg_first, pl.g_pairs)) return rc;
     MM_HIP(ctx, hipStreamWaitEvent(ctx->stream, ctx->ev_join, 0));
     return MM_OK;
 }
@@ -784,9 +987,10 @@
     ex.zero_bwb = bwb;
     ex.chol_init = 1;
     ex.init = ia;
+    const HeldOrder ho = held_order(ctx, pb, pl, ws_schur);
     MM_LAUNCH(ctx, "schur_prepare_kernel", schur_prepare_damped_kernel, dim3(pl.g_prep), dim3(256), 0, *pb, cams, Bd, gc, Cinv, S, v,
-              pl.ws.camtab, pl.ws.seg_done, pl.ws.desc, ex);
-    if (int rc = launch_pairs(ctx, pb, pl, pts, Cinv, gp, Bd, gc, S, v, SlabSync{}, 0u, pl.g_pairs)) return rc;
+              pl.ws.camtab, pl.ws.seg_done, ho.held ? nullptr : pl.ws.desc, ex);
+    if (int rc = launch_build(ctx, pb, pl, ho, pts, Cinv, gp, Bd, gc, S, v)) return rc;
     mm_chol_init_done(ctx, ws_chol, sides);
     const int rc = mm_chol_solve_sym(ctx, S, n, v, half_bandwidth, 1, info, ws_chol, ws_chol_bytes);
     mm_chol_init_done(ctx, nullptr, 0);
diff --git a/meatmodeler_amd/csrc/trf.hip b/meatmodeler_amd/csrc/trf.hip
--- a/meatmodeler_amd/csrc/trf.hip
+++ b/meatmodeler_amd/csrc/trf.hip
@@ -241,6 +241,10 @@
         explicit TableHold(mm_ctx *ctx) : c(ctx) { mm_cam_table_hold(c, true); }
         ~TableHold() { mm_cam_table_hold(c, false); }
     } table_hold(ctx);
+    struct OrderHold {
+        mm_ctx *c;
+        ~OrderHold() { mm_ba_schur_order_hold(c, nullptr, nullptr, 0, 0); }
+    } order_hold{ctx};
     struct FusedGuard {
         mm_ctx *c;
         bool saved, saved_strict, saved_no_event;
@@ -334,6 +338,14 @@
     if (!std::isfinite(cost0)) {
         rep->status = -2;
         return mm_fail(ctx, MM_ERR_NUMERIC, "mm_ba_trf: residuals are not finite in the initial point");
+    }
+    {
+        bool ordered = false;
+        TRF_CALL(mm_ba_schur_order(ctx, pb, t.ws_schur, t.ws_schur_b, t.board, &ordered));
+        if (ordered) {
+            TRF_CALL(read_board(t.board, 2));
+            mm_ba_schur_order_hold(ctx, pb, t.ws_schur, (int64_t)host[0], (int64_t)host[1]);
+        }
     }
     const int half_bw = dist ? dist->half_bandwidth : 6 * pb->cam_span + 5;
     TRF_CALL(normal_eq(x));
diff --git a/meatmodeler_amd/ops.py b/meatmodeler_amd/ops.py
--- a/meatmodeler_amd/ops.py
+++ b/meatmodeler_amd/ops.py
@@ -931,6 +931,18 @@
                                        self._schur_ws.numel()), "mm_ba_schur")
         return S, v, Cinv
 
+    def schur_held(self, cams, pts, Bd, Cd, gc, gp):
+        self._no_fixed("schur_held")
+        n = 6 * self.F
+        S = self._schur_buffers(n)
+        v = torch.empty(n, dtype=torch.float64, device=self.device)
+        Cinv = torch.empty((self.P, 6), dtype=torch.float64, device=self.device)
+        counts = (C.c_int64 * 2)()
+        self.ctx.check(lib.mm_ba_schur_held_debug(self.ctx.h, C.byref(self.pb), ptr(cams), ptr(pts), ptr(Bd), ptr(Cd), ptr(gc),
+                                                  ptr(gp), ptr(S), ptr(v), ptr(Cinv), ptr(self._schur_ws),
+                                                  self._schur_ws.numel(), counts), "mm_ba_schur_held_debug")
+        return S, v, Cinv, int(counts[0]), int(counts[1])
+
     def _alloc_S(self, n):
         self._S_storage = torch.zeros(2 * n * n, dtype=torch.float64, device=self.device)
         self._S = self._S_storage[:n * n].view(n, n)
```

Result: slower. 8723 billion descriptor pairs/s (match stage) (-1.7%).
